# heyblackC/DFMIR

Hardware: AMD Instinct MI355X
Metric: train-step image-pairs/sec (fwd+bwd): 2D 256x256 bs=16 and 3D 160^3 bs=1 (higher is better)
Workload: dtype f32 (fp16x2-split MFMA, fp32 accumulate)

## Files before the change

dfmir_amd/_lib.py:

```python
import ctypes
import os
from ctypes import c_double, c_float, c_int, c_longlong, c_void_p, POINTER, Structure

_HERE = os.path.dirname(os.path.abspath(__file__))
LIB_PATH = os.environ.get("DFMIR_HIP_LIB") or os.path.join(_HERE, "libdfmir_hip.so")


class DfConvGeom(Structure):
    _fields_ = [(n, c_int) for n in (
        "N", "Cin", "Cout", "Di", "Hi", "Wi", "Do", "Ho", "Wo", "KD", "KH", "KW",
        "stride", "dil", "pd", "ph", "pw", "pad_mode", "act")] + [("slope", c_float)]


P = c_void_p
_GP = POINTER(DfConvGeom)
_SIGS = {
    "dfmir_abi_version": [],
    "dfmir_set_option": [ctypes.c_char_p, ctypes.c_char_p],
    "dfmir_get_option": [ctypes.c_char_p, ctypes.c_char_p, c_int],
    "dfmir_conv_fwd": [_GP, P, P, P, P, P],
    "dfmir_conv_wgrad": [_GP, P, P, P, P],
    "dfmir_bias_grad": [P, P, c_int, c_int, c_longlong, P],
    "dfmir_weight_pack": [P, P, c_int, c_int, c_int, c_int, P],
    "dfmir_weight_pack_floats": [c_int, c_int, c_int],
    "dfmir_weight_pack_batch": [P, c_int, P, c_int, P],
    "dfmir_conv3x3_res_ok": [_GP],
    "dfmir_conv3x3_fwd_scaled_res": [_GP, P, P, c_int, P, P, P, P, c_int, P, P],
    "dfmir_conv3x3_reflect_ring_ok": [_GP],
    "dfmir_conv3x3_reflect_ring_len": [_GP],
    "dfmir_conv3x3_reflect_ring": [_GP, P, P, P, c_int, P, P, P],
    "dfmir_conv3x3_bwd_pair_ok": [_GP, _GP],
    "dfmir_conv3x3_bwd_pair": [_GP, _GP, P, P, c_int, P, P, P, P, c_int, P, P, P, c_int, P, P, POINTER(c_int), P],
    "dfmir_conv_fwd_scaled": [_GP, P, P, c_int, P, P, P, P],
    "dfmir_conv_wgrad_scaled": [_GP, P, P, c_int, P, P, c_int, P, P, P],
    "dfmir_conv_wgrad_scaled_ch": [_GP, P, P, c_int, P, P, c_int, P, P, P, P],
    "dfmir_instnorm_bwd_pmax_ok": [c_longlong],
    "dfmir_instnorm_bwd_pmax": [P, P, P, P, P, c_int, c_longlong, c_int, P, P, c_int, P, P],
    "dfmir_patch_gather_bwd_gp": [P, P, P, c_int, c_int, c_longlong, c_int, c_int, P, P, P],
    "dfmir_patch_gather_bwd_any": [P, P, P, c_int, c_int, c_longlong, c_int, c_int, P, P, P],
    "dfmir_absmax": [P, c_longlong, P, P],
    "dfmir_conv3d_split_ok": [_GP],
    "dfmir_conv3d_split_ws_floats": [c_int, c_int],
    "dfmir_conv3d_split_fwd": [_GP, P, P, c_int, P, P, P, P, P, P],
    "dfmir_conv3d_split_fwd_sub": [_GP, P, P, c_int, P, P, P, P, P, c_int, P],
    "dfmir_conv3d_split_fwd_actgrad": [_GP, P, P, c_int, P, P, P, P, P, c_int, P, c_float, P],
    "dfmir_conv3d_up_ok": [c_int] * 6,
    "dfmir_conv3d_wsplit_batch": [P, c_int, P],
    "dfmir_conv3d_split_is_pair": [c_int],
    "dfmir_conv3d_march_ok": [_GP],
    "dfmir_conv3d_march_fwd": [_GP, P, P, c_int, P, P, P, P, P, c_float, P],
    "dfmir_conv3d_tiny_ok": [_GP],
    "dfmir_conv3d_tiny_fwd": [_GP, P, P, P, P, P, P, c_float, P],
    "dfmir_conv3d_s2c2_ok": [_GP],
    "dfmir_conv3d_s2c2_fwd": [_GP, P, P, P, P, P, P],
    "dfmir_conv3d_s2c2_wgrad": [_GP, P, P, P, P],
    "dfmir_conv3d_s2_ok": [_GP],
    "dfmir_conv3d_s2_fwd": [_GP, P, P, P, P, P, P],
    "dfmir_conv3d_s2_wgrad": [_GP, P, P, P, P, P],
    "dfmir_conv3d_s2_dgrad_ok": [_GP],
    "dfmir_conv3d_s2_dgrad": [_GP, P, P, P, P],
    "dfmir_conv3d_up_ws_floats": [c_int, c_int],
    "dfmir_conv3d_up_fwd": [P, P, c_int, P, c_int, P, P] + [c_int] * 6 + [P],
    "dfmir_conv3d_up_skip2_fwd": [P, P, c_int, P, P, c_int, c_int, P, P, P, P, P] + [c_int] * 7 + [c_float, P],
    "dfmir_conv3d_up_dgrad_ws_floats": [c_int, c_int],
    "dfmir_conv3d_up_dgrad": [P, P, c_int, P, c_int, P, P, P, P, c_float] + [c_int] * 6 + [P],
    "dfmir_conv3d_split_fwd_add": [_GP, P, P, c_int, P, c_int, c_int, P, P, P, P, P],
    "dfmir_conv3d_split_wgrad_ok": [_GP],
    "dfmir_conv3d_split_wgrad": [_GP, P, P, c_int, P, P, c_int, P, P],
    "dfmir_conv3d_split_wgrad_upcat": [_GP, P, P, c_int, P, c_int, P, P, c_int, P, P, P],
    "dfmir_conv3d_upwgrad_ok": [_GP, c_int],
    "dfmir_conv3d_wgrad_is_march": [_GP],
    "dfmir_conv3d_wgrad_is_march_at": [_GP, P, P],
    "dfmir_conv3d_upwgrad_ws_floats": [],
    "dfmir_conv3d_upwgrad": [_GP, P, P, c_int, P, c_int, P, P, c_int, P, P, P, P],
    "dfmir_conv3d_split_wgrad_db": [_GP, P, P, c_int, P, P, c_int, P, P, P],
    "dfmir_probe_merge": [P, P, P, P],
    "dfmir_act_bwd_amax": [P, P, P, c_longlong, c_int, c_float, P, P],
    "dfmir_weight_unpack": [P, P, c_int, c_int, c_int, P],
    "dfmir_weight_unpack_add_batch": [P, c_int, c_longlong, P],
    "dfmir_conv7x7_c1_fwd": [P, P, P, P, c_int, c_int, c_int, c_int, c_int, P],
    "dfmir_conv7x7_c1_wgrad": [P, P, P, P, c_int, c_int, c_int, c_int, c_int, P],
    "dfmir_tapstack_fwd": [P, P] + [c_int] * 7 + [P],
    "dfmir_tapstack_bwd": [P, P] + [c_int] * 7 + [P],
    "dfmir_tapsum_fwd": [P, P, P] + [c_int] * 10 + [c_float, P],
    "dfmir_tapsum_bwd": [P, P] + [c_int] * 9 + [P],
    "dfmir_instnorm_fwd": [P, P, P, P, P, c_int, c_longlong, c_float, c_int, P, P],
    "dfmir_instnorm_stats_ok": [c_longlong],
    "dfmir_instnorm_stats": [P, P, P, c_int, c_longlong, c_float, c_int, P, P],
    "dfmir_instnorm_bwd": [P, P, P, P, P, c_int, c_longlong, c_int, P, P],
    "dfmir_instnorm_bwd_cols_ok": [c_longlong, c_int],
    "dfmir_instnorm_bwd_cols": [P, P, P, P, P, c_int, c_longlong, c_int, P, P, c_int, P],
    "dfmir_in_relu_blurdown_ok": [c_int, c_int],
    "dfmir_in_relu_blurdown_fwd": [P, P, P, P, c_int, c_int, c_int, c_float, P, P],
    "dfmir_in_relu_blurdown_bwd": [P, P, P, P, P, c_int, c_int, c_int, P, P, P],
    "dfmir_act_bwd": [P, P, P, c_longlong, c_int, c_float, P],
    "dfmir_blur_down_fwd": [P, P, c_int, c_int, c_int, P],
    "dfmir_blur_down_bwd": [P, P, c_int, c_int, c_int, P],
    "dfmir_blur_up_fwd": [P, P, c_int, c_int, c_int, P],
    "dfmir_blur_up_bwd": [P, P, c_int, c_int, c_int, P],
    "dfmir_reflect_pad2d_fwd": [P, P, c_int, c_int, c_int, c_int, P],
    "dfmir_reflect_pad2d_bwd": [P, P, c_int, c_int, c_int, c_int, P],
    "dfmir_reflect_pad2d_bwd_add": [P, P, P, c_int, c_int, c_int, c_int, P],
    "dfmir_upcat_fwd": [P, P, P] + [c_int] * 7 + [P],
    "dfmir_upcat_bwd": [P, P, P] + [c_int] * 7 + [P],
    "dfmir_cat_channels_fwd": [P, P, P, c_longlong, c_longlong, c_longlong, P],
    "dfmir_cat_channels_bwd": [P, P, P, c_longlong, c_longlong, c_longlong, P],
    "dfmir_scale": [P, P, c_longlong, c_float, P],
    "dfmir_warp2d_fwd": [P, P, P] + [c_int] * 6 + [P],
    "dfmir_warp2d_bwd": [P, P, P, P, P] + [c_int] * 6 + [P],
    "dfmir_warp3d_fwd": [P, P, P] + [c_int] * 7 + [P],
    "dfmir_warp3d_bwd": [P, P, P, P, P] + [c_int] * 7 + [P],
    "dfmir_warp_bwd_own_ws_floats": [c_int] * 6,
    "dfmir_warp_bwd_own": [c_int, P, P, P, P, P] + [c_int] * 7 + [P, P],
    "dfmir_resize_fwd": [P, P] + [c_int] * 7 + [c_float, P],
    "dfmir_resize_bwd": [P, P] + [c_int] * 7 + [c_float, P],
    "dfmir_resize_bwd_ws_floats": [c_int] * 7,
    "dfmir_resize_bwd_sep": [P, P] + [c_int] * 7 + [c_float, P, P],
    "dfmir_bspline_fwd": [c_int, P, P] + [c_int] * 7 + [P],
    "dfmir_bspline_bwd_ws_floats": [c_int] * 8,
    "dfmir_bspline_bwd": [c_int, P, P] + [c_int] * 7 + [P, P],
    "dfmir_patch_gather_fwd": [P, P, P, c_int, c_int, c_longlong, c_int, P],
    "dfmir_patch_gather_bwd": [P, P, P, c_int, c_int, c_longlong, c_int, P],
    "dfmir_patch_gather_bwd_amax": [P, P, P, c_int, c_int, c_longlong, c_int, P, P],
    "dfmir_patch_gather_fwd_g": [P, P, P, c_int, c_int, c_longlong, c_int, c_int, P],
    "dfmir_patch_gather_bwd_g": [P, P, P, c_int, c_int, c_longlong, c_int, c_int, P, P],
    "dfmir_l2norm_fwd": [P, P, P, c_int, c_longlong, c_float, P],
    "dfmir_l2norm_bwd": [P, P, P, P, c_int, c_longlong, c_float, P],
    "dfmir_patchnce_fwd": [P, P, P, P, c_longlong, c_int, c_int, c_float, P],
    "dfmir_patchnce_bwd": [P, P, P, P, c_longlong, c_int, c_int, c_float, P],
    "dfmir_masked_l1_fwd": [P, P, P, c_float, P, P, c_longlong, P],
    "dfmir_masked_l1_bwd": [P, P, P, c_float, P, P, P, P, c_longlong, P],
    "dfmir_flow_smooth_ws_floats": [],
    "dfmir_flow_smooth_fwd": [P, P, P] + [c_int] * 5 + [P],
    "dfmir_flow_smooth_bwd": [P, P, P] + [c_int] * 5 + [P],
    "dfmir_flow_smooth_fwd_p": [P, P, P] + [c_int] * 6 + [P],
    "dfmir_flow_smooth_bwd_p": [P, P, P] + [c_int] * 6 + [P],
    "dfmir_mul": [P, P, P, c_longlong, P],
    "dfmir_bend_ws_floats": [c_int] * 5,
    "dfmir_bend_fwd": [P, P, P] + [c_int] * 5 + [c_float] * 3 + [P],
    "dfmir_bend_bwd": [P, P, P] + [c_int] * 5 + [c_float] * 3 + [P],
    "dfmir_jacdet_ws_floats": [c_int] * 5,
    "dfmir_jacdet_fwd": [c_int, P, P, P] + [c_int] * 5 + [c_float, c_int, P],
    "dfmir_jacdet_bwd": [c_int, P, P, P] + [c_int] * 5 + [c_float, c_int, P],
    "dfmir_jacdet_map": [c_int, P, P] + [c_int] * 5 + [P],
    "dfmir_jacdet_stats": [c_int, P, P, P] + [c_int] * 5 + [c_double, c_double, P],
    "dfmir_invcons_ws_floats": [c_int] * 5,
    "dfmir_invcons_fwd": [c_int, P, P, P, P, P, P] + [c_int] * 4 + [P],
    "dfmir_invcons_bwd_ws_floats": [c_int] * 5,
    "dfmir_invcons_bwd": [c_int, P, P, P, P, P, P, P] + [c_int] * 4 + [P],
    "dfmir_compose_fwd": [c_int, P, P, P] + [c_int] * 4 + [P],
    "dfmir_compose_bwd_ws_floats": [c_int] * 5,
    "dfmir_compose_bwd": [c_int, P, P, P, P, P, P] + [c_int] * 4 + [P],
    "dfmir_flow_invert_ws_floats": [c_int] * 7,
    "dfmir_flow_invert": [c_int, P, P, P, P, P] + [c_int] * 5 + [c_float, c_int, P],
    "dfmir_dsearch_pool": [c_int, P, P, P] + [c_int] * 6 + [P],
    "dfmir_dsearch_cost": [c_int, P, P, P] + [c_int] * 6 + [P],
    "dfmir_dsearch_argmin": [c_int, P, P, c_float, P, P] + [c_int] * 5 + [P],
    "dfmir_dsearch_smooth": [c_int, P, P] + [c_int] * 4 + [P],
    "dfmir_warp_ssd_ws_floats": [c_int] * 6,
    "dfmir_warp_ssd_pack": [c_int, P, P] + [c_int] * 5 + [P],
    "dfmir_warp_ssd_fwd": [c_int] + [P] * 9 + [c_int] * 5 + [P],
    "dfmir_warp_ssd_fwd_grad": [c_int] + [P] * 10 + [c_int] * 5 + [P],
    "dfmir_warp_ssd_bwd": [P, P, P, P, c_longlong, P],
    "dfmir_affine_ws_floats": [c_int] * 5,
    "dfmir_affine_flow": [c_int, P, P] + [c_int] * 4 + [P],
    "dfmir_affine_flow_bwd": [c_int, P, P, P] + [c_int] * 4 + [P],
    "dfmir_affine_system": [c_int] + [P] * 6 + [c_int] * 6 + [P],
    "dfmir_affine_lm_step": [c_int] + [P] * 7 + [c_int] * 3 + [c_double] * 2 + [P],
    "dfmir_landmark_ws_floats": [c_int] * 6,
    "dfmir_landmark_fwd": [c_int] + [P] * 10 + [c_int] * 5 + [c_float] * 3 + [c_int, P],
    "dfmir_landmark_bwd": [c_int] + [P] * 8 + [c_int] * 5 + [c_float] * 3 + [c_int, P],
    "dfmir_nmi_ws_floats": [c_longlong, c_int],
    "dfmir_nmi_fwd": [P, P, P, P, c_int, c_float, c_float, c_longlong, P, P, P],
    "dfmir_nmi_bwd": [P, P, P, P, c_int, c_float, c_float, c_longlong, P, P, P, P, P],
    "dfmir_mind_ws_floats": [c_int] * 8,
    "dfmir_mind_desc": [P] + [c_int] * 7 + [P, P, P],
    "dfmir_mind_fwd": [P, P, P] + [c_int] * 7 + [P, P, P],
    "dfmir_mind_bwd": [P, P, P] + [c_int] * 7 + [P, P, P, P, P, P],
    "dfmir_gradfield_ws_floats": [c_int] * 5,
    "dfmir_gradfield_fwd": [P, P, P] + [c_int] * 5 + [c_float] * 3 + [c_int] + [c_double] * 3 + [P, P, P],
    "dfmir_gradfield_bwd": [P] * 7 + [c_int] * 5 + [c_float] * 3 + [P],
    "dfmir_gradfield_field": [P] + [c_int] * 5 + [c_float] * 3 + [c_int] + [c_double] * 2 + [P, P, P],
    "dfmir_warp_dice_ws_floats": [c_int] * 6,
    "dfmir_warp_dice_fwd": [c_int, P, P, P, P] + [c_int] * 6 + [P, P, P, P, P],
    "dfmir_warp_dice_bwd": [c_int, P, P, P, P] + [c_int] * 5 + [P, P, P, P],
    "dfmir_label_hausdorff_ws_bytes": [c_int] * 6,
    "dfmir_label_edt_sq": [c_int, P, c_int, c_int] + [c_int] * 4 + [P, P],
    "dfmir_label_hausdorff": [c_int, P, P, P] + [c_int] * 7 + [P, P, P, P, P, P],
    "dfmir_dice_ws_floats": [c_longlong, c_longlong],
    "dfmir_dice_fwd": [P, P, c_longlong, c_longlong, P, P, P],
    "dfmir_dice_bwd": [P, P, c_longlong, c_longlong, P, P, P, P, P],
    "dfmir_mse_ws_floats": [c_longlong],
    "dfmir_mse_fwd": [P, P, c_longlong, P, P, P],
    "dfmir_mse_bwd": [P, P, c_longlong, P, P, P, P],
    "dfmir_ncc_fwd_m": [P, P, P, c_int, P, P, P, P] + [c_int] * 5 + [c_float, P],
    "dfmir_ncc_bwd_m": [P, P, P, c_int, P, P, P, P, P, P] + [c_int] * 5 + [c_float, P],
    "dfmir_ncc_gauss_fwd": [P, P, P, c_int, P, P, P, P] + [c_int] * 4 + [P, c_int, c_float, c_float, P],
    "dfmir_ncc_gauss_bwd": [P, P, P, c_int, P, P, P, P, P, P] + [c_int] * 4 + [P, c_int, c_float, c_float, P],
    "dfmir_ncc_fwd": [P, P, P, P, P, P] + [c_int] * 5 + [c_float, P],
    "dfmir_ncc_bwd": [P, P, P, P, P, P, P, P] + [c_int] * 5 + [c_float, P],
    "dfmir_patch_gather_fwd_multi": [P, c_int, P, P, c_int, c_int, c_longlong, c_int, P],
    "dfmir_nce_head_fwd": [P, c_int, P, P, P, P, P, P, P, P, P, P, c_int, c_int, c_longlong, c_int, c_float, P],
    "dfmir_patch_ids_draw": [P, P, c_int, c_int, c_int, P, P],
    "dfmir_segment_means_fwd": [P, P, c_int, c_int, c_longlong, c_float, P],
    "dfmir_segment_means_bwd": [P, P, c_int, c_int, c_longlong, c_float, P],
    "dfmir_scalar_combine_fwd": [P, c_int, P, c_int, P, P],
    "dfmir_scalar_combine_bwd": [P, c_int, P, c_int, P, P],
    "dfmir_det_head_floats": [],
    "dfmir_det_begin": [P, c_longlong, P, c_longlong, P, c_int, P, c_longlong, P, c_int, ctypes.c_double, P],
    "dfmir_det_end": [P, P, c_longlong, P, c_longlong, P],
    "dfmir_fill_zero": [P, c_longlong, P],
    "dfmir_sum_scaled": [P, P, c_longlong, c_float, P],
    "dfmir_fill_from_scalar": [P, P, c_longlong, c_float, P],
    "dfmir_adam_step": [P, P, P, P, c_longlong] + [c_float] * 7 + [P],
}

_lib = None


class DfmirHipError(RuntimeError):
    pass


def lib():
    global _lib
    if _lib is None:
        import torch
        if not os.path.exists(LIB_PATH):
            raise DfmirHipError(
                "libdfmir_hip.so not found at %s -- build it with `python -c 'import __graft_entry__ as g; "
                "g.build()'` or `make -C dfmir_amd/csrc` (there is no CPU fallback)" % LIB_PATH)
        h = ctypes.CDLL(LIB_PATH)
        for name, args in _SIGS.items():
            fn = getattr(h, name)
            fn.argtypes = args
            fn.restype = c_int
        h.dfmir_weight_pack_floats.restype = c_longlong
        h.dfmir_conv3d_split_ws_floats.restype = c_longlong
        h.dfmir_conv3d_up_ws_floats.restype = c_longlong
        h.dfmir_conv3d_up_dgrad_ws_floats.restype = c_longlong
        h.dfmir_conv3d_upwgrad_ws_floats.restype = c_longlong
        h.dfmir_flow_smooth_ws_floats.restype = c_longlong
        h.dfmir_bend_ws_floats.restype = c_longlong
        h.dfmir_jacdet_ws_floats.restype = c_longlong
        h.dfmir_invcons_ws_floats.restype = c_longlong
        h.dfmir_invcons_bwd_ws_floats.restype = c_longlong
        h.dfmir_compose_bwd_ws_floats.restype = c_longlong
        h.dfmir_flow_invert_ws_floats.restype = c_longlong
        h.dfmir_warp_ssd_ws_floats.restype = c_longlong
        h.dfmir_affine_ws_floats.restype = c_longlong
        h.dfmir_landmark_ws_floats.restype = c_longlong
        h.dfmir_nmi_ws_floats.restype = c_longlong
        h.dfmir_mind_ws_floats.restype = c_longlong
        h.dfmir_gradfield_ws_floats.restype = c_longlong
        h.dfmir_warp_dice_ws_floats.restype = c_longlong
        h.dfmir_label_hausdorff_ws_bytes.restype = c_longlong
        h.dfmir_dice_ws_floats.restype = c_longlong
        h.dfmir_mse_ws_floats.restype = c_longlong
        h.dfmir_warp_bwd_own_ws_floats.restype = c_longlong
        h.dfmir_resize_bwd_ws_floats.restype = c_longlong
        h.dfmir_bspline_bwd_ws_floats.restype = c_longlong
        h.dfmir_last_error.argtypes = []
        h.dfmir_last_error.restype = ctypes.c_char_p
        _lib = h
    return _lib


def check(rc):
    if rc != 0:
        msg = lib().dfmir_last_error()
        raise DfmirHipError(msg.decode() if msg else "dfmir_hip error %d" % rc)


def set_option(name, value=None):
    check(lib().dfmir_set_option(name.encode(), None if value is None else str(value).encode()))


def get_option(name):
    buf = ctypes.create_string_buffer(256)
    n = lib().dfmir_get_option(name.encode(), buf, 256)
    return None if n < 0 else buf.value.decode()


def exported_symbols():
    return sorted(list(_SIGS.keys()) + ["dfmir_last_error"])
```

dfmir_amd/csrc/conv.hip:

```cpp
#include "conv3x3_common.h"
#include <stdlib.h>
#include <vector>

typedef float f32x16 __attribute__((ext_vector_type(16)));

struct ConvK {
  DfConvGeom g;
  int kc, nchunks;
  int Dm, Hm, Wm, ncx, ncy, ncz;
};

static inline void df_chunking(int Cin, int& kc, int& nchunks) {
  nchunks = (Cin + 15) / 16;
  int per = (Cin + nchunks - 1) / nchunks;
  kc = (per + 1) & ~1;
  if (kc < 2) kc = 2;
}

template <bool DIL2>
__device__ __forceinline__ bool conv_pixel(const ConvK& k, long long pp, long long P, int& n, int& oz, int& oy, int& ox,
                                           int& cls) {
  const DfConvGeom& g = k.g;
  cls = 0;
  if (pp >= P) { n = oz = oy = ox = 0; return false; }
// ... 282 lines not shown
    v += bias ? bias[co] : 0.f;
    if (g.act == 1) v = v > 0.f ? v : v * g.slope;
    else if (g.act == 2) v = tanhf(v);
    y[((long long)n * g.Cout + co) * DHWo + (pp - (long long)n * DHWo)] = v;
  }
}

template <int WJ, int WC, int TJ, int TC, int BP>
__global__ __launch_bounds__(256) void conv_wgrad_mfma_k(const float* __restrict__ x,
                                                         const float* __restrict__ dy,
                                                         float* __restrict__ dwt, DfConvGeom g,
                                                         long long pchunk, const float* __restrict__ fx) {
  constexpr int BJ = WJ * TJ * 32, BC = WC * TC * 32;
  constexpr int RS = 256 / BP;
  constexpr int NA = BJ / RS, NB = (BC + RS - 1) / RS;
  static_assert(WJ * WC == 4, "4 waves");
  __shared__ float As[2][BP][BJ + 1];
  __shared__ float Bs[2][BP][BC + 1];
  __shared__ int jinfo[BJ];

  const int tid = threadIdx.x, lane = tid & 63, wid = tid >> 6;
  const int wj = wid / WC, wc = wid % WC;
  const long long DHWi = (long long)g.Di * g.Hi * g.Wi;
  const long long DHWo = (long long)g.Do * g.Ho * g.Wo;
  const long long P = (long long)g.N * DHWo;
  const int J = g.KD * g.KH * g.KW * g.Cin;
  const int j0 = blockIdx.y * BJ, c0 = blockIdx.z * BC;
  const long long pbeg = (long long)blockIdx.x * pchunk;
  long long pend = pbeg + pchunk;
  if (pend > P) pend = P;

  for (int i = tid; i < BJ; i += 256) {
    const int j = j0 + i;
    int info = -1;
    if (j < J) {
      const int tap = j / g.Cin, ci = j - tap * g.Cin;
      const int kw = tap % g.KW, t2 = tap / g.KW, kh = t2 % g.KH, kd = t2 / g.KH;
      info = (ci << 12) | (kd << 8) | (kh << 4) | kw;
    }
    jinfo[i] = info;
  }
  __syncthreads();

  constexpr unsigned OOB = 0x80000000u;
  const unsigned dhwi4 = (unsigned)DHWi * 4u;
  const __amdgpu_buffer_rsrc_t x_src = __builtin_amdgcn_make_buffer_rsrc(
      const_cast<float*>(x), 0, (unsigned)((long long)g.N * g.Cin * DHWi * 4), 0x00020000);
  const __amdgpu_buffer_rsrc_t d_src = __builtin_amdgcn_make_buffer_rsrc(
      const_cast<float*>(dy), 0, (unsigned)((long long)g.N * g.Cout * DHWo * 4), 0x00020000);
  const int pl = tid % BP, r0 = tid / BP;
  float ra[NA], rb[NB];
  f32x16 acc[TJ][TC];
#pragma unroll
  for (int i = 0; i < TJ; ++i)
#pragma unroll
    for (int j = 0; j < TC; ++j)
#pragma unroll
      for (int r = 0; r < 16; ++r) acc[i][j][r] = 0.f;

#define WG_GLOAD(pb_)                                                                            \
  {                                                                                              \
    const long long pq = (pb_) + pl;                                                             \
    const bool pv = pq < pend;                                                                   \
    int ox = 0, oy = 0, oz = 0, n = 0;                                                           \
    if (pv) {                                                                                    \
      long long t = pq;                                                                          \
      ox = (int)(t % g.Wo); t /= g.Wo;                                                           \
      oy = (int)(t % g.Ho); t /= g.Ho;                                                           \
      oz = (int)(t % g.Do); n = (int)(t / g.Do);                                                 \
    }                                                                                            \
    const unsigned xb = (unsigned)n * (unsigned)g.Cin * dhwi4;                                   \
    _Pragma("unroll") for (int jj = 0; jj < NA; ++jj) {                                          \
      const int info = jinfo[r0 + RS * jj];                                                      \
      const int ci = info >> 12, kd = (info >> 8) & 15, kh = (info >> 4) & 15, kw = info & 15;   \
      int iz, iy, ix;                                                                            \
      bool v = pv && info >= 0;                                                                  \
      v &= df_in_coord(oz, kd, g.stride, g.pd, 1, g.Di, g.pad_mode, iz);                         \
      v &= df_in_coord(oy, kh, g.stride, g.ph, 1, g.Hi, g.pad_mode, iy);                         \
      v &= df_in_coord(ox, kw, g.stride, g.pw, 1, g.Wi, g.pad_mode, ix);                         \
      const unsigned o = v ? xb + (unsigned)ci * dhwi4 +                                         \
                                 (unsigned)(((long long)iz * g.Hi + iy) * g.Wi + ix) * 4u : OOB; \
      ra[jj] = __uint_as_float(__builtin_amdgcn_raw_buffer_load_b32(x_src, o, 0, 0));            \
    }                                                                                            \
    const long long so = pq - (long long)n * DHWo;                                               \
    _Pragma("unroll") for (int jj = 0; jj < NB; ++jj) {                                          \
      const int cr = r0 + RS * jj;                                                               \
      const int co = c0 + cr;                                                                    \
      const unsigned o = (pv && cr < BC && co < g.Cout)                                          \
                             ? (unsigned)(((long long)n * g.Cout + co) * DHWo + so) * 4u : OOB;  \
      rb[jj] = __uint_as_float(__builtin_amdgcn_raw_buffer_load_b32(d_src, o, 0, 0));            \
    }                                                                                            \
  }
#define WG_LSTORE(buf_)                                                                          \
  {                                                                                              \
    _Pragma("unroll") for (int jj = 0; jj < NA; ++jj) As[buf_][pl][r0 + RS * jj] = ra[jj];       \
    _Pragma("unroll") for (int jj = 0; jj < NB; ++jj) {                                          \
      const int cr = r0 + RS * jj;                                                               \
      if (cr < BC) Bs[buf_][pl][cr] = rb[jj];                                                    \
    }                                                                                            \
  }

  if (pbeg < pend) {
    WG_GLOAD(pbeg);
    WG_LSTORE(0);
  }
  __syncthreads();
  const int l31 = lane & 31, lhi = lane >> 5;
  int it = 0;
  for (long long pb = pbeg; pb < pend; pb += BP, ++it) {
    const int buf = it & 1;
    const bool more = (pb + BP) < pend;
    if (more) WG_GLOAD(pb + BP);
#pragma unroll 2
    for (int kk = 0; kk < BP / 2; ++kk) {
      const int kr = 2 * kk + lhi;
      float a[TJ], b[TC];
#pragma unroll
      for (int i = 0; i < TJ; ++i) a[i] = As[buf][kr][(wj * TJ + i) * 32 + l31];
#pragma unroll
      for (int j = 0; j < TC; ++j) b[j] = Bs[buf][kr][(wc * TC + j) * 32 + l31];
#pragma unroll
      for (int i = 0; i < TJ; ++i)
#pragma unroll
        for (int j = 0; j < TC; ++j)
          acc[i][j] = __builtin_amdgcn_mfma_f32_32x32x2f32(a[i], b[j], acc[i][j], 0, 0, 0);
    }
    if (more) WG_LSTORE(buf ^ 1);
    __syncthreads();
  }
#undef WG_GLOAD
#undef WG_LSTORE

#pragma unroll
  for (int j = 0; j < TC; ++j) {
    const int co = c0 + (wc * TC + j) * 32 + l31;
    if (co >= g.Cout) continue;
#pragma unroll
    for (int i = 0; i < TJ; ++i) {
      const int jb = j0 + (wj * TJ + i) * 32 + 4 * lhi;
#pragma unroll
      for (int r = 0; r < 16; ++r) {
        const int jr = jb + (r & 3) + 8 * (r >> 2);
        if (jr < J) df_acc(dwt, (long long)jr * g.Cout + co, acc[i][j][r], fx);
      }
    }
  }
}


__global__ __launch_bounds__(256) void conv1x1_wgrad_k(const float* __restrict__ x, const float* __restrict__ dy,
                                                       float* __restrict__ dwt, int N, int Cin, int Cout, long long S,
                                                       long long chunks_per_img, long long chunks_per_block,
                                                       const float* __restrict__ fx) {
  constexpr int BK = 64, LD = BK + 1;
  __shared__ float Xs[64 * LD];
  __shared__ float Ds[64 * LD];
  const int tid = threadIdx.x, lane = tid & 63, wid = tid >> 6;
  const int l31 = lane & 31, lhi = lane >> 5, wm = wid >> 1, wn = wid & 1;
  const int ci0 = blockIdx.y * 64, co0 = blockIdx.z * 64;
  const long long total = (long long)N * chunks_per_img;
  const long long cbeg = (long long)blockIdx.x * chunks_per_block;
  long long cend = cbeg + chunks_per_block;
  if (cend > total) cend = total;
  const int r = tid >> 2, q16 = (tid & 3) * 16;
  const bool xrow = ci0 + r < Cin, drow = co0 + r < Cout;
  float4 rx[4], rd[4];
  const float4 z4 = make_float4(0.f, 0.f, 0.f, 0.f);
#define G1_GLOAD(c_)                                                                                         \
  {                                                                                                          \
    const long long n_ = (c_) / chunks_per_img, q0_ = ((c_) - n_ * chunks_per_img) * BK + q16;               \
    const float* xp_ = x + ((long long)n_ * Cin + ci0 + r) * S + q0_;                                        \
    const float* dp_ = dy + ((long long)n_ * Cout + co0 + r) * S + q0_;                                      \
    _Pragma("unroll") for (int j = 0; j < 4; ++j) {                                                          \
      const bool in_ = q0_ + 4 * j < S;                                                                      \
      rx[j] = (xrow && in_) ? *reinterpret_cast<const float4*>(xp_ + 4 * j) : z4;                            \
      rd[j] = (drow && in_) ? *reinterpret_cast<const float4*>(dp_ + 4 * j) : z4;                            \
    }                                                                                                        \
  }
#define G1_LSTORE()                                                                                          \
  {                                                                                                          \
    float* xs_ = &Xs[r * LD + q16];                                                                          \
    float* ds_ = &Ds[r * LD + q16];                                                                          \
    _Pragma("unroll") for (int j = 0; j < 4; ++j) {                                                          \
      xs_[4 * j] = rx[j].x; xs_[4 * j + 1] = rx[j].y; xs_[4 * j + 2] = rx[j].z; xs_[4 * j + 3] = rx[j].w;    \
      ds_[4 * j] = rd[j].x; ds_[4 * j + 1] = rd[j].y; ds_[4 * j + 2] = rd[j].z; ds_[4 * j + 3] = rd[j].w;    \
    }                                                                                                        \
  }
  f32x16 acc;
#pragma unroll
  for (int i = 0; i < 16; ++i) acc[i] = 0.f;
  if (cbeg < cend) G1_GLOAD(cbeg)
  for (long long c = cbeg; c < cend; ++c) {
    __syncthreads();
    G1_LSTORE()
    __syncthreads();
    if (c + 1 < cend) G1_GLOAD(c + 1)
    const float* ap = &Xs[(wm * 32 + l31) * LD + lhi];
    const float* bp = &Ds[(wn * 32 + l31) * LD + lhi];
#pragma unroll 8
    for (int ks = 0; ks < BK / 2; ++ks)
      acc = __builtin_amdgcn_mfma_f32_32x32x2f32(ap[2 * ks], bp[2 * ks], acc, 0, 0, 0);
  }
#undef G1_GLOAD
#undef G1_LSTORE
  const int co = co0 + wn * 32 + l31;
  if (co < Cout && cbeg < cend) {
#pragma unroll
    for (int i = 0; i < 16; ++i) {
      const int ci = ci0 + wm * 32 + 4 * lhi + (i & 3) + 8 * (i >> 2);
      if (ci < Cin) df_acc(dwt, (long long)ci * Cout + co, acc[i], fx);
    }
  }
}

__global__ void bias_grad_k(const float* __restrict__ dy, float* __restrict__ db, int N, int C,
                            long long S, int nsplit, const float* __restrict__ fx) {
  __shared__ float sm[17];
  const int c = blockIdx.x, n = blockIdx.y, part = blockIdx.z;
  const long long per = (((S + nsplit - 1) / nsplit) + 3) & ~3LL;
  const long long beg = part * per;
  long long end = beg + per;
  if (end > S) end = S;
  const float* p = dy + ((long long)n * C + c) * S;
  float s = 0.f;
  if ((S & 3) == 0) {
    const float4* p4 = reinterpret_cast<const float4*>(p);
    for (long long i = (beg >> 2) + threadIdx.x; i < (end >> 2); i += blockDim.x) {
      const float4 v = p4[i];
      s += (v.x + v.y) + (v.z + v.w);
    }
  } else {
    for (long long i = beg + threadIdx.x; i < end; i += blockDim.x) s += p[i];
  }
  s = block_sum(s, sm);
  if (threadIdx.x == 0 && beg < S) df_acc(db, c, s, fx);
}

__global__ __launch_bounds__(256) void weight_pack_k(const float* __restrict__ w, float* __restrict__ o, int Cout,
                                                     int Cin, int T, int mode, float* __restrict__ part) {
  __shared__ unsigned smax;
  if (threadIdx.x == 0) smax = 0u;
  __syncthreads();
  float am = 0.f;
  const long long total = (long long)Cout * Cin * T;
  for (long long i = (long long)blockIdx.x * blockDim.x + threadIdx.x; i < total;
       i += (long long)gridDim.x * blockDim.x) {
    if (mode == 0) {
      const int co = (int)(i % Cout);
      long long r = i / Cout;
      const int ci = (int)(r % Cin);
      const int t = (int)(r / Cin);
      o[i] = w[((long long)co * Cin + ci) * T + t];
      am = fmaxf(am, fabsf(o[i]));
    } else {
      const int ci = (int)(i % Cin);
      long long r = i / Cin;
      const int co = (int)(r % Cout);
      const int t = (int)(r / Cout);
      o[i] = w[((long long)co * Cin + ci) * T + (T - 1 - t)];
      am = fmaxf(am, fabsf(o[i]));
    }
  }
  if (part) publish_block_absmax(am, &smax, part + blockIdx.x);
}
__global__ void weight_unpack_k(const float* __restrict__ gt, float* __restrict__ g, int Cout, int Cin,
                                int T) {
  const long long total = (long long)Cout * Cin * T;
  for (long long i = (long long)blockIdx.x * blockDim.x + threadIdx.x; i < total;
       i += (long long)gridDim.x * blockDim.x) {
    const int t = (int)(i % T);
    long long r = i / T;
    const int ci = (int)(r % Cin);
    const int co = (int)(r / Cin);
    g[i] = gt[((long long)t * Cin + ci) * Cout + co];
  }
}

__global__ __launch_bounds__(256) void weight_pack_batch_k(const DfPackJobDev* __restrict__ jobs) {
  const DfPackJobDev jb = jobs[blockIdx.y];
  if ((int)blockIdx.x >= jb.nblk) return;
  __shared__ unsigned smax;
  if (threadIdx.x == 0) smax = 0u;
  __syncthreads();
  float am = 0.f;
  const int Cout = jb.Cout, Cin = jb.Cin, T = jb.T;
  const long long total = (long long)Cout * Cin * T;
  for (long long i = (long long)blockIdx.x * 256 + threadIdx.x; i < total; i += (long long)jb.nblk * 256) {
    float v;
    if (jb.mode == 0) {
      const int co = (int)(i % Cout);
      long long r = i / Cout;
      const int ci = (int)(r % Cin);
      const int t = (int)(r / Cin);
      v = jb.w[((long long)co * Cin + ci) * T + t];
    } else {
      const int ci = (int)(i % Cin);
      long long r = i / Cin;
      const int co = (int)(r % Cout);
      const int t = (int)(r / Cout);
      v = jb.w[((long long)co * Cin + ci) * T + (T - 1 - t)];
    }
    jb.o[i] = v;
    am = fmaxf(am, fabsf(v));
  }
  if (jb.part) publish_block_absmax(am, &smax, jb.part + blockIdx.x);
}

__global__ __launch_bounds__(256) void weight_unpack_add_batch_k(const DfUnpackJob* __restrict__ jobs) {
  const DfUnpackJob jb = jobs[blockIdx.y];
  const int Cout = jb.Cout, Cin = jb.Cin, T = jb.T;
  if (T > 9) {
    const long long total = (long long)Cout * Cin * T;
    for (long long i = (long long)blockIdx.x * blockDim.x + threadIdx.x; i < total;
         i += (long long)gridDim.x * blockDim.x) {
      const int t = (int)(i % T);
      long long r = i / T;
      const int ci = (int)(r % Cin);
      const int co = (int)(r / Cin);
      const long long j = ((long long)t * Cin + ci) * Cout + co;
      jb.dst[i] += jb.src[j];
      jb.src[j] = 0.f;
    }
    return;
  }
  __shared__ float tile[32][32 * 9 + 1];
  const int tco = (Cout + 31) >> 5, tci = (Cin + 31) >> 5;
  const int lx = threadIdx.x & 31, ly = threadIdx.x >> 5;
  for (int tl = blockIdx.x; tl < tco * tci; tl += gridDim.x) {
    const int co0 = (tl % tco) << 5, ci0 = (tl / tco) << 5;
    for (int r = ly; r < T * 32; r += 8) {
      const int t = r >> 5, ci = ci0 + (r & 31), co = co0 + lx;
      float v = 0.f;
      if (ci < Cin && co < Cout) {
        const long long j = ((long long)t * Cin + ci) * Cout + co;
        v = jb.src[j];
        jb.src[j] = 0.f;
      }
      tile[lx][(r & 31) * T + t] = v;
    }
    __syncthreads();
    const int ncol = 32 * T;
    for (int e = threadIdx.x; e < 32 * ncol; e += 256) {
      const int c = e / ncol, q = e - c * ncol;
      const int co = co0 + c, ci = ci0 + q / T;
      if (co < Cout && ci < Cin) jb.dst[((long long)co * Cin + ci0) * T + q] += tile[c][q];
    }
    __syncthreads();
  }
}

bool df_conv3x3_fwd_try(const DfConvGeom* g, const float* x, const float* w_tcc, const float* bias,
                        float* y, hipStream_t st, int* rc);
bool df_conv3x3_wgrad_try(const DfConvGeom* g, const float* x, const float* dy, float* dw_tcc,
                          hipStream_t st, int* rc);
bool df_conv3x3_small_wgrad_try(const DfConvGeom* g, const float* x, const float* dy, float* dw_tcc, hipStream_t st,
                                int* rc);
bool df_conv3x3_split_fwd_try(const DfConvGeom* g, const float* x, const float* x_amax, int x_n, const float* w_packed,
                              const float* bias, const float* res, const float* ring, int ring_rl, float* y,
                              hipStream_t st, int* rc);
int df_conv3x3_split_res_ok(const DfConvGeom* g);
bool df_conv3x3_split_wgrad_try(const DfConvGeom* g, const float* x, const float* x_amax, int x_n, const float* dy,
                                const float* dy_amax, int dy_n, float* dw_tcc, float* db, hipStream_t st, int* rc,
                                const float* dy_pmax);
int df_weight_split_launch(const float* w_tcc, float* packed, int K, int M, int npart, hipStream_t st);
float* df_weight_probe_slots(float* packed, int K, int M);
int df_absmax_launch(const float* x, long long n, float* out, hipStream_t st, bool zero_first);
bool df_conv3d_fwd_try(const DfConvGeom* g, const float* x, const float* w_tcc, const float* bias, float* y,
                       hipStream_t st, int* rc);
bool df_conv3d_wgrad_try(const DfConvGeom* g, const float* x, const float* dy, float* dw_tcc, hipStream_t st,
                         int* rc);
static bool use_generic_only() {
  static DfOptInt o{"DFMIR_CONV_GENERIC", 0};
  return o.get() == 1;
}

static int check_geom(const DfConvGeom* g) {
  if (!g) return -1;
  if (g->N <= 0 || g->Cin <= 0 || g->Cout <= 0) return -1;
  if (g->Di <= 0 || g->Hi <= 0 || g->Wi <= 0 || g->Do <= 0 || g->Ho <= 0 || g->Wo <= 0) return -1;
  if (g->KD <= 0 || g->KH <= 0 || g->KW <= 0 || g->KD > 15 || g->KH > 15 || g->KW > 15) return -1;
  if (g->stride < 1 || g->dil < 1) return -1;
  if (g->pad_mode != 0 && g->pad_mode != 1) return -1;
  if (g->pad_mode == 1 && g->dil != 1) return -1;
  return 0;
}

static int conv_fwd_impl(const DfConvGeom* g, const float* x, const float* x_amax, int x_n, const float* w_tcc,
                         const float* bias, float* y, void* stream);
extern "C" int dfmir_conv_fwd(const DfConvGeom* g, const float* x, const float* w_tcc,
                              const float* bias, float* y, void* stream) {
  return conv_fwd_impl(g, x, nullptr, 0, w_tcc, bias, y, stream);
}
extern "C" int dfmir_conv_fwd_scaled(const DfConvGeom* g, const float* x, const float* x_amax, int x_amax_n,
                                     const float* w_tcc, const float* bias, float* y, void* stream) {
  return conv_fwd_impl(g, x, x_amax, x_amax_n, w_tcc, bias, y, stream);
}
extern "C" int dfmir_conv3x3_res_ok(const DfConvGeom* g) {
  return (g && check_geom(g) == 0 && !use_generic_only()) ? df_conv3x3_split_res_ok(g) : 0;
}
extern "C" int dfmir_conv3x3_fwd_scaled_res(const DfConvGeom* g, const float* x, const float* x_amax, int x_amax_n,
                                            const float* w_tcc, const float* bias, const float* res,
                                            const float* ring, int ring_len, float* y, void* stream) {
  DF_ARG_CHECK(g && check_geom(g) == 0 && x && x_amax && x_amax_n > 0 && w_tcc && (res || ring) && y);
  DF_ARG_CHECK(!use_generic_only() && df_conv3x3_split_res_ok(g));
  DF_ARG_CHECK(!ring || (ring_len >= (g->Ho > g->Wo ? g->Ho : g->Wo) + 2 && g->Ho >= 4 && g->Wo >= 4));
  int rc = 0;
  if (!df_conv3x3_split_fwd_try(g, x, x_amax, x_amax_n, w_tcc, bias, res, ring, ring_len, y, (hipStream_t)stream, &rc))
    return df_set_error((int)hipErrorInvalidValue, __FILE__, __LINE__);
  return rc;
}
extern "C" int dfmir_absmax(const float* x, long long n, float* out, void* stream) {
  DF_ARG_CHECK(x && out && n > 0);
  const int rc = df_absmax_launch(x, n, out, (hipStream_t)stream, false);
  if (rc) return df_set_error(rc, __FILE__, __LINE__);
  return 0;
}
static int conv_fwd_impl(const DfConvGeom* g, const float* x, const float* x_amax, int x_n, const float* w_tcc,
                         const float* bias, float* y, void* stream) {
  DF_ARG_CHECK(check_geom(g) == 0 && x && w_tcc && y);
  hipStream_t st = (hipStream_t)stream;
  const long long P = (long long)g->N * g->Do * g->Ho * g->Wo;
  static DfOptFlag tinyvol_o{"DFMIR_NO_TINYVOL"};
  const bool tinyvol = !use_generic_only() && g->Do > 1 && (long long)g->Do * g->Ho * g->Wo <= 512 && P <= 8192 && g->Cout <= 64 &&
                       g->Cout > 4 && !tinyvol_o.get();
  if (!use_generic_only()) {
    int rc = 0;
    if (df_conv3x3_split_fwd_try(g, x, x_amax, x_n, w_tcc, bias, nullptr, nullptr, 0, y, st, &rc)) return rc;
    if (df_conv3x3_fwd_try(g, x, w_tcc, bias, y, st, &rc)) return rc;
    if (!tinyvol && df_conv3d_fwd_try(g, x, w_tcc, bias, y, st, &rc)) return rc;
  }
  if (g->Cout <= 4) {
    const unsigned grid = (unsigned)((P + 255) / 256);
    if (g->Cout == 1) conv_small_k<1><<<grid, 256, 0, st>>>(x, w_tcc, bias, y, *g);
    else if (g->Cout == 2) conv_small_k<2><<<grid, 256, 0, st>>>(x, w_tcc, bias, y, *g);
    else conv_small_k<4><<<grid, 256, 0, st>>>(x, w_tcc, bias, y, *g);
    DF_LAUNCH_CHECK();
    return 0;
  }
  if (tinyvol) {
    if (g->Cout <= 8) conv_tinyvol_k<8><<<(unsigned)P, 256, 0, st>>>(x, w_tcc, bias, y, *g);
    else if (g->Cout <= 16) conv_tinyvol_k<16><<<(unsigned)P, 256, 0, st>>>(x, w_tcc, bias, y, *g);
    else if (g->Cout <= 32) conv_tinyvol_k<32><<<(unsigned)P, 256, 0, st>>>(x, w_tcc, bias, y, *g);
    else conv_tinyvol_k<64><<<(unsigned)P, 256, 0, st>>>(x, w_tcc, bias, y, *g);
    DF_LAUNCH_CHECK();
    return 0;
  }
  const long long in_img = (long long)g->Cin * g->Di * g->Hi * g->Wi * 4;
  const long long out_img = (long long)g->Cout * g->Do * g->Ho * g->Wo * 4;
  DF_ARG_CHECK(in_img < 0x7FFFFFFFLL && out_img < 0x7FFFFFFFLL);
  DF_ARG_CHECK((long long)g->KD * g->KH * g->KW * g->Cin * g->Cout * 4 < 0x7FFFFFFFLL);
  long long nb = 0x7FFFFFFFLL / (in_img > out_img ? in_img : out_img);
  if (nb > g->N) nb = g->N;
  for (int n0 = 0; n0 < g->N; n0 += (int)nb) {
    ConvK k;
    k.g = *g;
    k.g.N = (g->N - n0 < nb) ? g->N - n0 : (int)nb;
    df_chunking(g->Cin, k.kc, k.nchunks);
    const float* xs = x + (long long)n0 * (in_img / 4);
    float* ys = y + (long long)n0 * (out_img / 4);
    long long Ps = (long long)k.g.N * g->Do * g->Ho * g->Wo;
    const bool dil2 = g->dil == 2 && g->stride == 1 && g->pad_mode == 0 && g->KD * g->KH * g->KW <= 128 && g->Cout <= 64;
    k.ncx = k.ncy = k.ncz = 1;
    k.Dm = g->Do; k.Hm = g->Ho; k.Wm = g->Wo;
    if (dil2) {
      if (g->Wi > 1 || g->KW > 1) { k.ncx = 2; k.Wm = (g->Wo + 1) / 2; }
      if (g->Hi > 1 || g->KH > 1) { k.ncy = 2; k.Hm = (g->Ho + 1) / 2; }
      if (g->Di > 1 || g->KD > 1) { k.ncz = 2; k.Dm = (g->Do + 1) / 2; }
      Ps = (long long)k.ncx * k.ncy * k.ncz * k.g.N * k.Dm * k.Hm * k.Wm;
    }
    const bool small_p = (Ps + 255) / 256 < 192 && g->Cout > 8;
    if (dil2) {
      if (small_p) {
        dim3 grid((unsigned)((Ps + 63) / 64), (unsigned)((g->Cout + 63) / 64));
        conv_mfma_k<2, 2, 1, 1, true><<<grid, 256, 0, st>>>(xs, w_tcc, bias, ys, k);
      } else {
        dim3 grid((unsigned)((Ps + 255) / 256), 1);
        if (g->Cout > 32) conv_mfma_k<1, 4, 2, 2, true><<<grid, 256, 0, st>>>(xs, w_tcc, bias, ys, k);
        else conv_mfma_k<1, 4, 1, 2, true><<<grid, 256, 0, st>>>(xs, w_tcc, bias, ys, k);
      }
    } else if (small_p && g->Cout <= 64) {
      dim3 grid((unsigned)((Ps + 63) / 64), (unsigned)((g->Cout + 63) / 64));
      conv_mfma_k<2, 2, 1, 1><<<grid, 256, 0, st>>>(xs, w_tcc, bias, ys, k);
    } else if (g->Cout > 64) {
      const long long big = ((Ps + 127) / 128) * ((g->Cout + 127) / 128);
      constexpr int big_min = 256;
      if (big < big_min) {
        dim3 grid((unsigned)((Ps + 63) / 64), (unsigned)((g->Cout + 63) / 64));
        conv_mfma_k<2, 2, 1, 1><<<grid, 256, 0, st>>>(xs, w_tcc, bias, ys, k);
      } else {
        dim3 grid((unsigned)((Ps + 127) / 128), (unsigned)((g->Cout + 127) / 128));
        conv_mfma_k<2, 2, 2, 2><<<grid, 256, 0, st>>>(xs, w_tcc, bias, ys, k);
      }
    } else if (g->Cout > 32) {
      dim3 grid((unsigned)((Ps + 255) / 256), 1);
      conv_mfma_k<1, 4, 2, 2><<<grid, 256, 0, st>>>(xs, w_tcc, bias, ys, k);
    } else {
      dim3 grid((unsigned)((Ps + 255) / 256), 1);
      conv_mfma_k<1, 4, 1, 2><<<grid, 256, 0, st>>>(xs, w_tcc, bias, ys, k);
    }
    DF_LAUNCH_CHECK();
  }
  return 0;
}

static int conv_wgrad_impl(const DfConvGeom* g, const float* x, const float* x_amax, int x_n, const float* dy,
                           const float* dy_amax, int dy_n, float* dw_tcc, float* db, void* stream,
                           const float* dy_pmax = nullptr);
extern "C" int dfmir_conv_wgrad_scaled_ch(const DfConvGeom* g, const float* x, const float* x_amax, int x_amax_n,
                                          const float* dy, const float* dy_amax, int dy_amax_n, const float* dy_pmax,
                                          float* dw_tcc, float* db, void* stream) {
  return conv_wgrad_impl(g, x, x_amax, x_amax_n, dy, dy_amax, dy_amax_n, dw_tcc, db, stream, dy_pmax);
}
extern "C" int dfmir_conv_wgrad(const DfConvGeom* g, const float* x, const float* dy, float* dw_tcc,
                                void* stream) {
  return conv_wgrad_impl(g, x, nullptr, 0, dy, nullptr, 0, dw_tcc, nullptr, stream);
}
extern "C" int dfmir_conv_wgrad_scaled(const DfConvGeom* g, const float* x, const float* x_amax, int x_amax_n,
                                       const float* dy, const float* dy_amax, int dy_amax_n, float* dw_tcc,
                                       float* db, void* stream) {
  return conv_wgrad_impl(g, x, x_amax, x_amax_n, dy, dy_amax, dy_amax_n, dw_tcc, db, stream);
}
static int bias_grad_launch(const float* dy, float* db, int N, int C, long long S, hipStream_t st);
static int conv_wgrad_impl(const DfConvGeom* g, const float* x, const float* x_amax, int x_n, const float* dy,
                           const float* dy_amax, int dy_n, float* dw_tcc, float* db, void* stream, const float* dy_pmax) {
  DF_ARG_CHECK(check_geom(g) == 0 && x && dy && dw_tcc);
  DF_ARG_CHECK(g->dil == 1 && g->Cin < (1 << 19));
  hipStream_t st = (hipStream_t)stream;
  if (!use_generic_only()) {
    int rc = 0;
    if (df_conv3x3_split_wgrad_try(g, x, x_amax, x_n, dy, dy_amax, dy_n, dw_tcc, db, st, &rc, dy_pmax)) return rc;
  }
  if (db) {
    const int rcb = bias_grad_launch(dy, db, g->N, g->Cout, (long long)g->Do * g->Ho * g->Wo, st);
    if (rcb) return rcb;
  }
  if (!use_generic_only()) {
    int rc = 0;
    if (df_conv3x3_wgrad_try(g, x, dy, dw_tcc, st, &rc)) return rc;
    if (df_conv3x3_small_wgrad_try(g, x, dy, dw_tcc, st, &rc)) return rc;
    if (df_conv3d_wgrad_try(g, x, dy, dw_tcc, st, &rc)) return rc;
  }
  {
    static DfOptFlag no1x1_o{"DFMIR_NO_1X1_WGRAD"};
    const long long S1 = (long long)g->Di * g->Hi * g->Wi;
    if (!use_generic_only() && !no1x1_o.get() && g->KD == 1 && g->KH == 1 && g->KW == 1 && g->stride == 1 && g->pd == 0 &&
        g->ph == 0 && g->pw == 0 && g->Do == g->Di && g->Ho == g->Hi && g->Wo == g->Wi && (S1 & 3) == 0 && S1 >= 64 &&
        ((reinterpret_cast<uintptr_t>(x) | reinterpret_cast<uintptr_t>(dy)) & 15) == 0 && g->Cin >= 8 && g->Cout >= 8) {
      const long long cpi = (S1 + 63) / 64, total = (long long)g->N * cpi;
      const unsigned ny = (unsigned)((g->Cin + 63) / 64), nz = (unsigned)((g->Cout + 63) / 64);
      long long want = 1024 / ((long long)ny * nz);
      if (want < 1) want = 1;
      long long maxs = (total + 7) / 8;
      if (maxs < 1) maxs = 1;
      if (want > maxs) want = maxs;
      const long long cpb = (total + want - 1) / want;
      const unsigned nx = (unsigned)((total + cpb - 1) / cpb);
      conv1x1_wgrad_k<<<dim3(nx, ny, nz), 256, 0, st>>>(x, dy, dw_tcc, g->N, g->Cin, g->Cout, S1, cpi, cpb, df_det_fx());
      DF_LAUNCH_CHECK();
      return 0;
    }
  }
  long long P = (long long)g->N * g->Do * g->Ho * g->Wo;
  const int J = g->KD * g->KH * g->KW * g->Cin;
  auto plan = [&](int BJ, int BC, int BP, unsigned& nP, long long& pchunk, dim3& grid) {
    const unsigned nJ = (J + BJ - 1) / BJ, nC = (g->Cout + BC - 1) / BC;
    long long want = 2048 / ((long long)nJ * nC);
    if (want < 1) want = 1;
    long long maxp = (P + (long long)BP * 8 - 1) / ((long long)BP * 8);
    if (maxp < 1) maxp = 1;
    if (want > maxp) want = maxp;
    pchunk = (P + want - 1) / want;
    pchunk = ((pchunk + BP - 1) / BP) * BP;
    nP = (unsigned)((P + pchunk - 1) / pchunk);
    grid = dim3(nP, nJ, nC);
  };
  const long long in_img = (long long)g->Cin * g->Di * g->Hi * g->Wi * 4;
  const long long out_img = (long long)g->Cout * g->Do * g->Ho * g->Wo * 4;
  DF_ARG_CHECK(in_img < 0x7FFFFFFFLL && out_img < 0x7FFFFFFFLL);
  long long nb = 0x7FFFFFFFLL / (in_img > out_img ? in_img : out_img);
  if (nb > g->N) nb = g->N;
  const int Nfull = g->N;
  for (int n0 = 0; n0 < Nfull; n0 += (int)nb) {
    DfConvGeom gs = *g;
    gs.N = (Nfull - n0 < nb) ? Nfull - n0 : (int)nb;
    const float* xs = x + (long long)n0 * (in_img / 4);
    const float* ds = dy + (long long)n0 * (out_img / 4);
    P = (long long)gs.N * g->Do * g->Ho * g->Wo;
    unsigned nP;
    long long pchunk;
    dim3 grid;
    if (g->Cout > 64) {
      plan(128, 128, 16, nP, pchunk, grid);
      conv_wgrad_mfma_k<2, 2, 2, 2, 16><<<grid, 256, 0, st>>>(xs, ds, dw_tcc, gs, pchunk, df_det_fx());
    } else if (g->Cout > 32) {
      plan(128, 64, 16, nP, pchunk, grid);
      conv_wgrad_mfma_k<4, 1, 1, 2, 16><<<grid, 256, 0, st>>>(xs, ds, dw_tcc, gs, pchunk, df_det_fx());
    } else {
      plan(128, 32, 32, nP, pchunk, grid);
      conv_wgrad_mfma_k<4, 1, 1, 1, 32><<<grid, 256, 0, st>>>(xs, ds, dw_tcc, gs, pchunk, df_det_fx());
    }
    DF_LAUNCH_CHECK();
  }
  return 0;
}

static int bias_grad_launch(const float* dy, float* db, int N, int C, long long S, hipStream_t st) {
  int nsplit = (int)((S + 65535) / 65536);
  if (nsplit > 64) nsplit = 64;
  if (nsplit < 1) nsplit = 1;
  DF_ARG_CHECK(N <= 65535);
  bias_grad_k<<<dim3(C, N, nsplit), S >= 4096 ? 256 : 64, 0, st>>>(dy, db, N, C, S, nsplit, df_det_fx());
  DF_LAUNCH_CHECK();
  return 0;
}
extern "C" int dfmir_bias_grad(const float* dy, float* db, int N, int C, long long S, void* stream) {
  DF_ARG_CHECK(dy && db && N > 0 && C > 0 && S > 0);
  return bias_grad_launch(dy, db, N, C, S, (hipStream_t)stream);
}

extern "C" int dfmir_weight_pack(const float* w, float* w_tcc, int Cout, int Cin, int T, int mode,
                                 void* stream) {
  DF_ARG_CHECK(w && w_tcc && Cout > 0 && Cin > 0 && T > 0 && (mode == 0 || mode == 1));
  const long long total = (long long)Cout * Cin * T;
  const unsigned nblk = df_grid(total, 256, 2048);
  const int K = mode ? Cout : Cin, M = mode ? Cin : Cout;
  float* part = (T == 9) ? df_weight_probe_slots(w_tcc, K, M) : nullptr;
  weight_pack_k<<<nblk, 256, 0, (hipStream_t)stream>>>(w, w_tcc, Cout, Cin, T, mode, part);
  DF_LAUNCH_CHECK();
  if (T == 9) {
    const int rc = df_weight_split_launch(w_tcc, w_tcc, K, M, (int)nblk, (hipStream_t)stream);
    if (rc) return df_set_error(rc, __FILE__, __LINE__);
  }
  return 0;
}
int df_conv3x3_reflect_ring_ok(const DfConvGeom* g);
int df_conv3x3_reflect_ring_launch(const DfConvGeom* g, const float* dy, const float* dy_cols, const float* dy_amax,
                                   int dy_n, const float* wd_packed, float* ring, hipStream_t st);
int df_conv3x3_reflect_ring_len(const DfConvGeom* g);
extern "C" int dfmir_conv3x3_reflect_ring_ok(const DfConvGeom* g) {
  return (g && check_geom(g) == 0) ? df_conv3x3_reflect_ring_ok(g) : 0;
}
extern "C" int dfmir_conv3x3_reflect_ring_len(const DfConvGeom* g) {
  return (g && check_geom(g) == 0 && df_conv3x3_reflect_ring_ok(g)) ? df_conv3x3_reflect_ring_len(g) : 0;
}
extern "C" int dfmir_conv3x3_reflect_ring(const DfConvGeom* g, const float* dy, const float* dy_cols,
                                          const float* dy_amax, int dy_amax_n, const float* wd_packed, float* ring,
                                          void* stream) {
  DF_ARG_CHECK(g && check_geom(g) == 0 && dy && dy_amax && dy_amax_n > 0 && wd_packed && ring);
  DF_ARG_CHECK(df_conv3x3_reflect_ring_ok(g));
  const int rc = df_conv3x3_reflect_ring_launch(g, dy, dy_cols, dy_amax, dy_amax_n, wd_packed, ring, (hipStream_t)stream);
  if (rc) return df_set_error(rc, __FILE__, __LINE__);
  return 0;
}
int df_conv3x3_bwd_pair_ok(const DfConvGeom* gd, const DfConvGeom* gw);
bool df_conv3x3_bwd_pair_try(const DfConvGeom* gd, const DfConvGeom* gw, const float* dy, const float* dy_amax, int dy_n,
                             const float* dy_pmax, const float* wd_packed, const float* res, const float* ring, int ring_rl,
                             float* dx, const float* x, const float* x_amax, int x_n, float* dw_tcc, float* db,
                             hipStream_t st, int* rc);
extern "C" int dfmir_conv3x3_bwd_pair_ok(const DfConvGeom* gd, const DfConvGeom* gw) {
  return (gd && gw && check_geom(gd) == 0 && check_geom(gw) == 0 && !use_generic_only()) ? df_conv3x3_bwd_pair_ok(gd, gw) : 0;
}
extern "C" int dfmir_conv3x3_bwd_pair(const DfConvGeom* gd, const DfConvGeom* gw, const float* dy, const float* dy_amax,
                                      int dy_amax_n, const float* dy_pmax, const float* wd_packed, const float* res,
                                      const float* ring, int ring_len, float* dx, const float* x, const float* x_amax,
                                      int x_amax_n, float* dw_tcc, float* db, int* paired, void* stream) {
  DF_ARG_CHECK(gd && gw && check_geom(gd) == 0 && check_geom(gw) == 0 && dy && wd_packed && dx && x && dw_tcc && paired);
  DF_ARG_CHECK(gd->N == gw->N && gd->Cin == gw->Cout && gd->Cout == gw->Cin && gw->dil == 1 && gw->Cin < (1 << 19));
  DF_ARG_CHECK(!ring || (ring_len >= (gd->Ho > gd->Wo ? gd->Ho : gd->Wo) + 2 && gd->Ho >= 4 && gd->Wo >= 4));
  *paired = 0;
  int rc = 0;
  if (!use_generic_only() && df_conv3x3_bwd_pair_try(gd, gw, dy, dy_amax, dy_amax_n, dy_pmax, wd_packed, res, ring, ring_len,
                                                     dx, x, x_amax, x_amax_n, dw_tcc, db, (hipStream_t)stream, &rc)) {
    *paired = rc == 0 ? 1 : 0;
    return rc;
  }
  rc = (res || ring) ? dfmir_conv3x3_fwd_scaled_res(gd, dy, dy_amax, dy_amax_n, wd_packed, nullptr, res, ring, ring_len, dx, stream)
                     : conv_fwd_impl(gd, dy, dy_amax, dy_amax_n, wd_packed, nullptr, dx, stream);
  if (rc) return rc;
  return conv_wgrad_impl(gw, x, x_amax, x_amax_n, dy, dy_amax, dy_amax_n, dw_tcc, db, stream, dy_pmax);
}
extern "C" int dfmir_weight_pack_batch(const DfPackJob* jobs_host, int njobs, void* table_dev, int upload,
                                       void* stream) {
  DF_ARG_CHECK(jobs_host && table_dev && njobs > 0 && njobs <= 65535);
  static_assert(sizeof(DfPackJobDev) == 64, "job table stride");
  hipStream_t st = (hipStream_t)stream;
  int max_nblk = 0, max_nsplit = 0;
  std::vector<DfPackJobDev> tab((size_t)njobs);
  for (int i = 0; i < njobs; ++i) {
    const DfPackJob& h = jobs_host[i];
    DF_ARG_CHECK(h.w && h.packed && h.Cout > 0 && h.Cin > 0 && h.T > 0 && (h.mode == 0 || h.mode == 1));
    DfPackJobDev& d = tab[(size_t)i];
    d.w = h.w; d.o = h.packed; d.Cout = h.Cout; d.Cin = h.Cin; d.T = h.T; d.mode = h.mode;
    d.nblk = (int)df_grid((long long)h.Cout * h.Cin * h.T, 256, 2048);
    df_weight_split_fill(&d);
    max_nblk = d.nblk > max_nblk ? d.nblk : max_nblk;
    max_nsplit = d.nsplit > max_nsplit ? d.nsplit : max_nsplit;
  }
  if (upload) {
    hipError_t e = hipMemcpyAsync(table_dev, tab.data(), sizeof(DfPackJobDev) * (size_t)njobs, hipMemcpyHostToDevice, st);
    if (e != hipSuccess) return df_set_error((int)e, __FILE__, __LINE__);
  }
  weight_pack_batch_k<<<dim3((unsigned)max_nblk, (unsigned)njobs), 256, 0, st>>>(
      reinterpret_cast<const DfPackJobDev*>(table_dev));
  DF_LAUNCH_CHECK();
  const int rc = df_weight_split_batch_launch(reinterpret_cast<const DfPackJobDev*>(table_dev), njobs, max_nsplit, st);
  if (rc) return df_set_error(rc, __FILE__, __LINE__);
  return 0;
}
extern "C" long long dfmir_weight_pack_floats(int Cout, int Cin, int T) {
  if (Cout <= 0 || Cin <= 0 || T <= 0) return -1;
  const long long s0 = df_pack_split_floats(Cin, Cout, T), s1 = df_pack_split_floats(Cout, Cin, T);
  return df_pack_tcc_floats(Cin, Cout, T) + (s0 > s1 ? s0 : s1) + (T == 9 ? 4 + 2048 : 0);
}
extern "C" int dfmir_weight_unpack_add_batch(const DfUnpackJob* jobs_dev, int njobs, long long max_total,
                                             void* stream) {
  DF_ARG_CHECK(jobs_dev && njobs > 0 && njobs <= 65535 && max_total > 0);
  long long bx = (max_total + 255) / 256;
  if (bx > 64) bx = 64;
  weight_unpack_add_batch_k<<<dim3((unsigned)bx, (unsigned)njobs), 256, 0, (hipStream_t)stream>>>(jobs_dev);
  DF_LAUNCH_CHECK();
  return 0;
}
extern "C" int dfmir_weight_unpack(const float* g_tcc, float* g, int Cout, int Cin, int T,
                                   void* stream) {
  DF_ARG_CHECK(g_tcc && g && Cout > 0 && Cin > 0 && T > 0);
  const long long total = (long long)Cout * Cin * T;
  weight_unpack_k<<<df_grid(total, 256, 2048), 256, 0, (hipStream_t)stream>>>(g_tcc, g, Cout, Cin, T);
  DF_LAUNCH_CHECK();
  return 0;
}
```

dfmir_amd/csrc/nce_head.hip:

```cpp
#include "common.h"

#define DF_IDS_MAXP 1024
#define DF_IDS_MAXPERM 4096
struct DfIdSizes {
  long long S[8];
};

__device__ __forceinline__ unsigned long long df_mix64(unsigned long long z) {
  z += 0x9E3779B97F4A7C15ull;
  z = (z ^ (z >> 30)) * 0xBF58476D1CE4E5B9ull;
  z = (z ^ (z >> 27)) * 0x94D049BB133111EBull;
  return z ^ (z >> 31);
}

__global__ __launch_bounds__(256) void patch_ids_draw_k(unsigned long long* __restrict__ state, DfIdSizes sizes,
                                                        int n_layers, int n_sets, int P, int Ppad,
                                                        long long* __restrict__ out) {
  __shared__ unsigned long long el[DF_IDS_MAXPERM];
  __shared__ unsigned char lost[DF_IDS_MAXP];
  __shared__ int pending;
  const int layer = blockIdx.x / n_sets, set = blockIdx.x - layer * n_sets;
  const unsigned long long S = (unsigned long long)sizes.S[layer];
  const unsigned long long seed = state[0], counter = state[1];
  const unsigned long long stream = df_mix64(seed ^ df_mix64(counter * 0x100000001B3ull + (unsigned long long)blockIdx.x));
// ... 5 lines not shown
      el[i] = i < (int)S ? ((df_mix64(stream ^ ((unsigned long long)i * 0xD6E8FEB86659FD93ull)) >> 12) << 12) | (unsigned long long)i
                         : ~0ull;
    __syncthreads();
    for (int k = 2; k <= Spad; k <<= 1)
      for (int j = k >> 1; j > 0; j >>= 1) {
        for (int i = threadIdx.x; i < Spad; i += 256) {
          const int ixj = i ^ j;
          if (ixj > i) {
            const unsigned long long a = el[i], b = el[ixj];
            const bool up = (i & k) == 0;
            if ((a > b) == up) { el[i] = b; el[ixj] = a; }
          }
        }
        __syncthreads();
      }
    for (int i = threadIdx.x; i < P; i += 256) o[i] = (long long)(el[i] & 0xFFFull);
  } else {
  long long mine[DF_IDS_MAXP / 256];
  bool fresh[DF_IDS_MAXP / 256];
#pragma unroll
  for (int j = 0; j < DF_IDS_MAXP / 256; ++j) { mine[j] = -1; fresh[j] = true; }
  for (int round = 0; round < 64; ++round) {
#pragma unroll
    for (int j = 0; j < DF_IDS_MAXP / 256; ++j) {
      const int slot = threadIdx.x + j * 256;
      if (slot < Ppad) {
        unsigned long long e = ~0ull;
        if (slot < P) {
          if (fresh[j]) {
            const unsigned long long r = df_mix64(stream ^ ((unsigned long long)slot * 0xD6E8FEB86659FD93ull +
                                                            (unsigned long long)round * 0xA0761D6478BD642Full));
            mine[j] = (long long)(((r >> 32) * S) >> 32);
          }
          e = ((unsigned long long)mine[j] << 12) | ((unsigned long long)(fresh[j] ? 1 : 0) << 11) | (unsigned long long)slot;
        }
        el[slot] = e;
      }
    }
    if (threadIdx.x == 0) pending = 0;
    __syncthreads();
    for (int k = 2; k <= Ppad; k <<= 1)
      for (int j = k >> 1; j > 0; j >>= 1) {
        for (int i = threadIdx.x; i < Ppad; i += 256) {
          const int ixj = i ^ j;
          if (ixj > i) {
            const unsigned long long a = el[i], b = el[ixj];
            const bool up = (i & k) == 0;
            if ((a > b) == up) { el[i] = b; el[ixj] = a; }
          }
        }
        __syncthreads();
      }
    for (int i = threadIdx.x; i < Ppad; i += 256) lost[i] = 0;
    __syncthreads();
    for (int i = threadIdx.x + 1; i < Ppad; i += 256) {
      const unsigned long long e = el[i];
      if (e != ~0ull && (el[i - 1] >> 12) == (e >> 12)) lost[(int)(e & 0x7FFull)] = 1;
    }
    __syncthreads();
    bool any = false;
#pragma unroll
    for (int j = 0; j < DF_IDS_MAXP / 256; ++j) {
      const int slot = threadIdx.x + j * 256;
      if (slot < P) {
        fresh[j] = lost[slot] != 0;
        any = any || fresh[j];
      }
    }
    if (any) atomicOr(&pending, 1);
    __syncthreads();
    const int more = pending;
    __syncthreads();
    if (!more) break;
  }
#pragma unroll
  for (int j = 0; j < DF_IDS_MAXP / 256; ++j) {
    const int slot = threadIdx.x + j * 256;
    if (slot < P) o[slot] = mine[j];
  }
  }
  __syncthreads();
  if (threadIdx.x == 0) {
    __threadfence();
    const unsigned long long done = atomicAdd(&state[2], 1ull);
    if (done == (unsigned long long)gridDim.x - 1) {
      state[2] = 0ull;
      state[1] = counter + 1ull;
      __threadfence();
    }
  }
}

extern "C" int dfmir_patch_ids_draw(unsigned long long* state, const long long* sizes, int n_layers, int n_sets,
                                    int P, long long* out, void* stream) {
  DF_ARG_CHECK(state && sizes && out && n_layers > 0 && n_layers <= 8 && n_sets > 0 && P > 0 && P <= DF_IDS_MAXP);
  DfIdSizes sz{};
  for (int l = 0; l < n_layers; ++l) {
    DF_ARG_CHECK(sizes[l] >= P && sizes[l] < (1LL << 32));
    DF_ARG_CHECK(sizes[l] >= 2LL * P || sizes[l] <= DF_IDS_MAXPERM);
    sz.S[l] = sizes[l];
  }
  int Ppad = 1;
  while (Ppad < P) Ppad <<= 1;
  patch_ids_draw_k<<<(unsigned)(n_layers * n_sets), 256, 0, (hipStream_t)stream>>>(state, sz, n_layers, n_sets, P, Ppad,
                                                                               out);
  DF_LAUNCH_CHECK();
  return 0;
}

struct DfGatherSrcs {
  const float* p[8];
};
__global__ void patch_gather_multi_k(DfGatherSrcs srcs, const long long* __restrict__ ids, float* __restrict__ out,
                                     int G, int Bper, int C, long long S, int P) {
  const long long total = (long long)G * Bper * C * P;
  const long long rows = (long long)G * Bper * P;
  for (long long i = (long long)blockIdx.x * blockDim.x + threadIdx.x; i < total;
       i += (long long)gridDim.x * blockDim.x) {
    const int p = (int)(i % P);
    long long t = i / P;
    const int c = (int)(t % C);
    t /= C;
    const int b = (int)(t % Bper), g = (int)(t / Bper);
    out[(long long)c * rows + ((long long)g * Bper + b) * P + p] =
        srcs.p[g][((long long)b * C + c) * S + ids[(long long)g * P + p]];
  }
}
extern "C" int dfmir_patch_gather_fwd_multi(const float* const* srcs, int G, const long long* ids, float* out, int Bper,
                                            int C, long long S, int P, void* stream) {
  DF_ARG_CHECK(srcs && ids && out && G > 0 && G <= 8 && Bper > 0 && C > 0 && S > 0 && P > 0);
  DfGatherSrcs s{};
  for (int g = 0; g < G; ++g) {
    DF_ARG_CHECK(srcs[g] != nullptr);
    s.p[g] = srcs[g];
  }
  patch_gather_multi_k<<<df_grid((long long)G * Bper * C * P, 256, 4096), 256, 0, (hipStream_t)stream>>>(
      s, ids, out, G, Bper, C, S, P);
  DF_LAUNCH_CHECK();
  return 0;
}

typedef float nh_f32x16 __attribute__((ext_vector_type(16)));
struct NceHeadP {
  DfGatherSrcs srcs;
  const long long* ids;
  const float *w1, *b1, *w2, *b2;
  float *out, *nrm, *xs, *hs, *ypre;
  int G, Bper, C, P;
  long long S, rows;
  float eps;
};
constexpr int NH_R = 32, NH_M = 256, NH_CMAX = 256, NH_KB = 8;
__global__ __launch_bounds__(256, 2) void nce_head_fwd_k(NceHeadP k) {
  __shared__ float Xs[NH_CMAX * NH_R];
  __shared__ float Hs[NH_M * NH_R];
  __shared__ float red[4][NH_R];
  const int tid = threadIdx.x, lane = tid & 63, wid = tid >> 6;
  const int l31 = lane & 31, hi = lane >> 5;
  const long long r0 = (long long)blockIdx.x * NH_R;
  {
    const int r = tid & 31;
    const long long rr = r0 + r;
    const bool rok = rr < k.rows;
    const long long gb = rok ? rr / k.P : 0;
    const int pp = rok ? (int)(rr - gb * k.P) : 0;
    const int g = (int)(gb / k.Bper), b = (int)(gb - (long long)g * k.Bper);
    const long long id = rok ? k.ids[(long long)g * k.P + pp] : 0;
    const float* src = k.srcs.p[g] + (long long)b * k.C * k.S + id;
    const int Cp = (k.C + 2 * NH_KB - 1) / (2 * NH_KB) * (2 * NH_KB);
    for (int cb = tid >> 5; cb < Cp; cb += 64) {
      float v[8];
#pragma unroll
      for (int u = 0; u < 8; ++u) {
        const int c = cb + 8 * u;
        v[u] = (rok && c < k.C) ? src[(long long)c * k.S] : 0.f;
      }
#pragma unroll
      for (int u = 0; u < 8; ++u) {
        const int c = cb + 8 * u;
        if (c < Cp) {
          Xs[c * NH_R + r] = v[u];
          if (k.xs && rok && c < k.C) k.xs[(long long)c * k.rows + rr] = v[u];
        }
      }
    }
  }
  __syncthreads();
  const int m0 = 64 * wid;
  nh_f32x16 acc[2];
#pragma unroll
  for (int i = 0; i < 2; ++i)
#pragma unroll
    for (int e = 0; e < 16; ++e) acc[i][e] = 0.f;
#define NH_GEMM(W_, KTOT_, SRC_)                                                                  \
  {                                                                                               \
    const float* wp = (W_) + m0 + l31;                                                            \
    const int K2 = ((KTOT_) + 1) >> 1, nb = (K2 + NH_KB - 1) / NH_KB;                             \
    float ca0[NH_KB], ca1[NH_KB], na0[NH_KB], na1[NH_KB];                                         \
    _Pragma("unroll") for (int u = 0; u < NH_KB; ++u) {                                           \
      const int kr = 2 * u + hi;                                                                  \
      const bool ok = kr < (KTOT_);                                                               \
      ca0[u] = ok ? wp[(long long)kr * NH_M] : 0.f;                                               \
      ca1[u] = ok ? wp[(long long)kr * NH_M + 32] : 0.f;                                          \
    }                                                                                             \
    for (int j = 0; j < nb; ++j) {                                                                \
      if (j + 1 < nb) {                                                                           \
        _Pragma("unroll") for (int u = 0; u < NH_KB; ++u) {                                       \
          const int kr = 2 * ((j + 1) * NH_KB + u) + hi;                                          \
          const bool ok = kr < (KTOT_);                                                           \
          na0[u] = ok ? wp[(long long)kr * NH_M] : 0.f;                                           \
          na1[u] = ok ? wp[(long long)kr * NH_M + 32] : 0.f;                                      \
        }                                                                                         \
      }                                                                                           \
      _Pragma("unroll") for (int u = 0; u < NH_KB; ++u) {                                         \
        const int kr = 2 * (j * NH_KB + u) + hi;                                                  \
        const float bv = (SRC_)[kr * NH_R + l31];                                                 \
        acc[0] = __builtin_amdgcn_mfma_f32_32x32x2f32(ca0[u], bv, acc[0], 0, 0, 0);               \
        acc[1] = __builtin_amdgcn_mfma_f32_32x32x2f32(ca1[u], bv, acc[1], 0, 0, 0);               \
      }                                                                                           \
      _Pragma("unroll") for (int u = 0; u < NH_KB; ++u) { ca0[u] = na0[u]; ca1[u] = na1[u]; }     \
    }                                                                                             \
  }
  NH_GEMM(k.w1, k.C, Xs)
#pragma unroll
  for (int i = 0; i < 2; ++i)
#pragma unroll
    for (int e = 0; e < 16; ++e) {
      const int m = m0 + 32 * i + (e >> 2) * 8 + hi * 4 + (e & 3);
      float v = acc[i][e] + k.b1[m];
      v = v > 0.f ? v : 0.f;
      Hs[m * NH_R + l31] = v;
      if (k.hs && r0 + l31 < k.rows) k.hs[(long long)m * k.rows + r0 + l31] = v;
      acc[i][e] = 0.f;
    }
  __syncthreads();
  NH_GEMM(k.w2, NH_M, Hs)
#undef NH_GEMM
  float ss = 0.f;
#pragma unroll
  for (int i = 0; i < 2; ++i)
#pragma unroll
    for (int e = 0; e < 16; ++e) {
      const int m = m0 + 32 * i + (e >> 2) * 8 + hi * 4 + (e & 3);
      acc[i][e] += k.b2[m];
      ss += acc[i][e] * acc[i][e];
    }
  ss += __shfl_xor(ss, 32);
  if (hi == 0) red[wid][l31] = ss;
  __syncthreads();
  const float nr = sqrtf((red[0][l31] + red[1][l31]) + (red[2][l31] + red[3][l31]));
  const float inv = 1.f / (nr + k.eps);
  const long long rr = r0 + l31;
  if (rr < k.rows) {
    if (k.nrm && wid == 0 && hi == 0) k.nrm[rr] = nr;
#pragma unroll
    for (int i = 0; i < 2; ++i)
#pragma unroll
      for (int e = 0; e < 16; ++e) {
        const int m = m0 + 32 * i + (e >> 2) * 8 + hi * 4 + (e & 3);
        k.out[(long long)m * k.rows + rr] = acc[i][e] * inv;
        if (k.ypre) k.ypre[(long long)m * k.rows + rr] = acc[i][e];
      }
  }
}
extern "C" int dfmir_nce_head_fwd(const float* const* srcs, int G, const long long* ids, const float* w1, const float* b1,
                                  const float* w2, const float* b2, float* out, float* nrm, float* xs, float* hs,
                                  float* ypre, int Bper, int C, long long S, int P, float eps, void* stream) {
  DF_ARG_CHECK(srcs && ids && w1 && b1 && w2 && b2 && out && G > 0 && G <= 8 && Bper > 0 && C > 0 && C <= NH_CMAX && S > 0 && P > 0);
  NceHeadP k{};
  for (int g = 0; g < G; ++g) {
    DF_ARG_CHECK(srcs[g] != nullptr);
    k.srcs.p[g] = srcs[g];
  }
  k.ids = ids; k.w1 = w1; k.b1 = b1; k.w2 = w2; k.b2 = b2;
  k.out = out; k.nrm = nrm; k.xs = xs; k.hs = hs; k.ypre = ypre;
  k.G = G; k.Bper = Bper; k.C = C; k.P = P; k.S = S; k.rows = (long long)G * Bper * P; k.eps = eps;
  nce_head_fwd_k<<<(unsigned)((k.rows + NH_R - 1) / NH_R), 256, 0, (hipStream_t)stream>>>(k);
  DF_LAUNCH_CHECK();
  return 0;
}

__global__ __launch_bounds__(256) void segment_means_k(const float* __restrict__ rows, float* __restrict__ out, int L,
                                                       int T, long long seg, float scale) {
  __shared__ float sm[17];
  const int t = blockIdx.x;
  float s = 0.f;
  for (int l = 0; l < L; ++l) {
    const float* r = rows + ((long long)l * T + t) * seg;
    for (long long i = threadIdx.x; i < seg; i += 256) s += r[i];
  }
  s = block_sum(s, sm);
  if (threadIdx.x == 0) out[t] = s * (scale / (float)seg);
}
__global__ void segment_means_bwd_k(const float* __restrict__ g, float* __restrict__ drows, int L, int T, long long seg,
                                    float scale) {
  const long long total = (long long)L * T * seg;
  for (long long i = (long long)blockIdx.x * blockDim.x + threadIdx.x; i < total;
       i += (long long)gridDim.x * blockDim.x) {
    const int t = (int)((i / seg) % T);
    drows[i] = g[t] * (scale / (float)seg);
  }
}
extern "C" int dfmir_segment_means_fwd(const float* rows, float* out, int L, int T, long long seg, float scale,
                                       void* stream) {
  DF_ARG_CHECK(rows && out && L > 0 && T > 0 && seg > 0);
  segment_means_k<<<(unsigned)T, 256, 0, (hipStream_t)stream>>>(rows, out, L, T, seg, scale);
  DF_LAUNCH_CHECK();
  return 0;
}
extern "C" int dfmir_segment_means_bwd(const float* gout, float* drows, int L, int T, long long seg, float scale,
                                       void* stream) {
  DF_ARG_CHECK(gout && drows && L > 0 && T > 0 && seg > 0);
  segment_means_bwd_k<<<df_grid((long long)L * T * seg, 256, 1024), 256, 0, (hipStream_t)stream>>>(gout, drows, L, T, seg,
                                                                                                scale);
  DF_LAUNCH_CHECK();
  return 0;
}

struct DfCombine {
  const float* in[8];
  float M[8][8];
};
__global__ void scalar_combine_k(DfCombine c, int n_in, int n_out, float* __restrict__ out) {
  const int j = threadIdx.x;
  if (j < n_out) {
    float s = 0.f;
    for (int i = 0; i < n_in; ++i) s += c.M[j][i] * c.in[i][0];
    out[j] = s;
  }
}
__global__ void scalar_combine_bwd_k(DfCombine c, const float* __restrict__ g, int n_in, int n_out,
                                     float* __restrict__ din) {
  const int i = threadIdx.x;
  if (i < n_in) {
    float s = 0.f;
    for (int j = 0; j < n_out; ++j) s += c.M[j][i] * g[j];
    din[i] = s;
  }
}
extern "C" int dfmir_scalar_combine_fwd(const float* const* in, int n_in, const float* M, int n_out, float* out,
                                        void* stream) {
  DF_ARG_CHECK(in && M && out && n_in > 0 && n_in <= 8 && n_out > 0 && n_out <= 8);
  DfCombine c{};
  for (int i = 0; i < n_in; ++i) {
    DF_ARG_CHECK(in[i] != nullptr);
    c.in[i] = in[i];
  }
  for (int j = 0; j < n_out; ++j)
    for (int i = 0; i < n_in; ++i) c.M[j][i] = M[j * n_in + i];
  scalar_combine_k<<<1, 64, 0, (hipStream_t)stream>>>(c, n_in, n_out, out);
  DF_LAUNCH_CHECK();
  return 0;
}
extern "C" int dfmir_scalar_combine_bwd(const float* gout, int n_in, const float* M, int n_out, float* din,
                                        void* stream) {
  DF_ARG_CHECK(gout && M && din && n_in > 0 && n_in <= 8 && n_out > 0 && n_out <= 8);
  DfCombine c{};
  for (int j = 0; j < n_out; ++j)
    for (int i = 0; i < n_in; ++i) c.M[j][i] = M[j * n_in + i];
  scalar_combine_bwd_k<<<1, 64, 0, (hipStream_t)stream>>>(c, gout, n_in, n_out, din);
  DF_LAUNCH_CHECK();
  return 0;
}

__global__ void probe_merge_k(const float* __restrict__ a, const float* __restrict__ b, float* __restrict__ out) {
  out[threadIdx.x] = fmaxf(a[threadIdx.x], b[threadIdx.x]);
}
extern "C" int dfmir_probe_merge(const float* a, const float* b, float* out, void* stream) {
  DF_ARG_CHECK(a && b && out);
  probe_merge_k<<<1, DF_PROBE_SLOTS, 0, (hipStream_t)stream>>>(a, b, out);
  DF_LAUNCH_CHECK();
  return 0;
}
```

dfmir_amd/networks.py:

```python
import functools
import os
import math

import numpy as np
import torch
import torch.nn as nn
from torch.nn import init
from torch.optim import lr_scheduler

from . import ops


class _ConvNd(nn.Module):

    def __init__(self, nd, in_channels, out_channels, kernel_size, stride=1, padding=0, bias=True):
        super().__init__()
        self.nd = nd
        self.in_channels, self.out_channels = in_channels, out_channels
        self.kernel_size, self.stride, self.padding = kernel_size, stride, padding
        self.weight = nn.Parameter(torch.empty((out_channels, in_channels) + (kernel_size,) * nd))
        self.bias = nn.Parameter(torch.empty(out_channels)) if bias else None
        self._packs = {}
        self.reset_parameters()

# ... 239 lines not shown
            stop = encode_only and idx == last
            if idx in want:
                if shared and not stop and t is feat:
                    feat, t = ops.fork_tap(t)
                feats.append(t)
            return stop

        while i < n:
            m = mods[i]
            gb = getattr(self, 'grad_boundary', None)
            if gb is not None and i == gb[0] and feat.requires_grad and torch.is_grad_enabled():
                feat.register_hook(lambda g_, cb=gb[1]: (cb(), None)[1])
            if isinstance(m, ReflectionPad2d) and i + 1 < n and isinstance(mods[i + 1], Conv2d):
                if i in want:
                    if emit(i, m(feat), shared=False):
                        return feat, feats, True
                conv = mods[i + 1]
                tanh = i + 2 < n and isinstance(mods[i + 2], Tanh) and (i + 1) not in want
                feat = _reflect_conv(m, conv, feat, act=2 if tanh else 0)
                if emit(i + 1, feat):
                    return feat, feats, True
                i += 2
                if tanh:
                    if emit(i, feat):
                        return feat, feats, True
                    i += 1
                continue
            if isinstance(m, Conv2d):
                tanh = i + 1 < n and isinstance(mods[i + 1], Tanh) and i not in want
                feat = m(feat, act=2 if tanh else 0)
                if emit(i, feat):
                    return feat, feats, True
                i += 1
                if tanh:
                    if emit(i, feat):
                        return feat, feats, True
                    i += 1
                continue
            if (isinstance(m, InstanceNorm2d) and i + 2 < n and isinstance(mods[i + 1], ReLU)
                    and isinstance(mods[i + 2], Downsample) and not ({i, i + 1, i + 2} & want)
                    and ops.in_relu_blurdown_ok(feat)):
                feat = ops.instance_norm_relu_blur_down(feat, m.eps)
                i += 3
                continue
            if isinstance(m, InstanceNorm2d):
                relu = i + 1 < n and isinstance(mods[i + 1], ReLU)
                feat = m(feat, relu=relu)
                if emit(i, feat):
                    return feat, feats, True
                i += 1
                if relu:
                    if emit(i, feat):
                        return feat, feats, True
                    i += 1
                continue
            feat = m(feat)
            if emit(i, feat):
                return feat, feats, True
            i += 1
        return feat, feats, False

    def forward(self, input, layers=[], encode_only=False):
        if -1 in layers:
            layers.append(len(self.model))
        if len(layers) > 0:
            feat, feats, stopped = self._run(input, list(layers), encode_only)
            if stopped:
                return feats
            return feat, feats
        feat, _, _ = self._run(input, [], False)
        return feat


def define_G(input_nc, output_nc, ngf, netG, norm='batch', use_dropout=False, init_type='normal',
             init_gain=0.02, no_antialias=False, no_antialias_up=False, gpu_ids=[], opt=None):
    norm_layer = get_norm_layer(norm_type=norm)
    blocks = {'resnet_9blocks': 9, 'resnet_6blocks': 6, 'resnet_4blocks': 4}
    if netG not in blocks:
        raise NotImplementedError('Generator model name [%s] is not recognized' % netG)
    net = ResnetGenerator(input_nc, output_nc, ngf, norm_layer=norm_layer, use_dropout=use_dropout,
                          no_antialias=no_antialias, no_antialias_up=no_antialias_up, n_blocks=blocks[netG], opt=opt)
    return init_net(net, init_type, init_gain, gpu_ids, initialize_weights=True)


class Normalize(nn.Module):

    def __init__(self, power=2):
        super().__init__()
        if power != 2:
            raise NotImplementedError("only the L2 Normalize is on the path")
        self.power = power

    def forward(self, x_rows_c):
        return ops.l2norm_rows(_as_channel_major(x_rows_c)).t()


def _as_channel_major(x_rows_c):
    t = x_rows_c.t()
    return t if t.is_contiguous() else t.contiguous()


class PatchSampleF(nn.Module):

    def __init__(self, use_mlp=False, init_type='normal', init_gain=0.02, nc=256, gpu_ids=[]):
        super().__init__()
        self.l2norm = Normalize(2)
        self.use_mlp = use_mlp
        self.nc = nc
        self.mlp_init = False
        self.init_type = init_type
        self.init_gain = init_gain
        self.gpu_ids = gpu_ids

    def create_mlp(self, feats):
        for mlp_id, feat in enumerate(feats):
            input_nc = feat.shape[1]
            mlp = nn.Sequential(Linear(input_nc, self.nc), ReLU(), Linear(self.nc, self.nc))
            mlp.to(feat.device)
            setattr(self, 'mlp_%d' % mlp_id, mlp)
        init_net(self, self.init_type, self.init_gain, self.gpu_ids)
        self.mlp_init = True

    def forward(self, feats, num_patches=64, patch_ids=None):
        return_ids, return_feats = [], []
        if self.use_mlp and not self.mlp_init:
            self.create_mlp(feats)
        for feat_id, feat in enumerate(feats):
            if num_patches <= 0:
                raise NotImplementedError("num_patches=0 (dense features) is not on the path")
            S = feat.shape[2] * feat.shape[3]
            if patch_ids is not None:
                patch_id = patch_ids[feat_id]
            else:
                patch_id = torch.randperm(S, device=feats[0].device)
                patch_id = ops.mark_distinct(patch_id[:int(min(num_patches, patch_id.shape[0]))])
            groups = patch_id.shape[0] if patch_id.dim() == 2 else 1
            x = ops.patch_gather(feat, patch_id, groups)
            return_ids.append(patch_id)
            return_feats.append(self.project(feat_id, x).t())
        return return_feats, return_ids

    def sample_project(self, feat_id, feat, ids, groups=1):
        if ops.nce_head_ok(feat.shape[1], self.nc, self.use_mlp):
            mlp = getattr(self, 'mlp_%d' % feat_id)
            return ops.nce_head(feat, ids, mlp[0], mlp[2])
        return self.project(feat_id, ops.patch_gather(feat, ids, groups))

    def sample_project_multi(self, feat_id, srcs, ids):
        if ops.nce_head_ok(srcs[0].shape[1], self.nc, self.use_mlp):
            mlp = getattr(self, 'mlp_%d' % feat_id)
            return ops.nce_head_multi(srcs, ids, mlp[0], mlp[2])
        return self.project(feat_id, ops.patch_gather_multi(srcs, ids))

    def project(self, feat_id, x_cm):
        if self.use_mlp:
            mlp = getattr(self, 'mlp_%d' % feat_id)
            x_cm = mlp[2](mlp[0](x_cm, relu=True))
        return ops.l2norm_rows(x_cm)


def define_F(input_nc, netF, norm='batch', use_dropout=False, init_type='normal', init_gain=0.02,
             no_antialias=False, gpu_ids=[], opt=None):
    if netF == 'sample':
        net = PatchSampleF(use_mlp=False, init_type=init_type, init_gain=init_gain, gpu_ids=gpu_ids, nc=opt.netF_nc)
    elif netF == 'mlp_sample':
        net = PatchSampleF(use_mlp=True, init_type=init_type, init_gain=init_gain, gpu_ids=gpu_ids, nc=opt.netF_nc)
    else:
        raise NotImplementedError('projection model name [%s] is not recognized' % netF)
    return init_net(net, init_type, init_gain, gpu_ids)


class GANLoss(nn.Module):

    def __init__(self, gan_mode, target_real_label=1.0, target_fake_label=0.0):
        super().__init__()
        self.gan_mode = gan_mode

    def forward(self, *a, **k):
        raise NotImplementedError("the registration model is discriminator-free (lambda_GAN = 0)")
```

dfmir_amd/ops.py:

```python
import collections
import ctypes
import functools
import os

import numpy as np
import torch
from torch.autograd import Function
from torch.autograd.function import once_differentiable

from ._lib import DfConvGeom, DfmirHipError, check, lib

_VP = ctypes.c_void_p


def _p(t):
    return None if t is None else _VP(t.data_ptr())


def _st():
    return _VP(torch.cuda.current_stream().cuda_stream)


def _need(*ts):
    for t in ts:
# ... 1781 lines not shown

    @staticmethod
    @once_differentiable
    def backward(ctx, dout):
        (ids,) = ctx.saved_tensors
        shape, B, C, S, Pn, G, distinct = ctx.meta
        dout = _c(dout)
        if ctx.stash is not None:
            ctx.stash.append((dout, ids, ctx.meta))
            return None, None, None, None
        dfeat = zeros(shape, dout.device)
        if distinct:
            check(lib().dfmir_patch_gather_bwd_g(_p(dout), _p(ids), _p(dfeat), B, C, S, Pn, G, None, _st()))
        else:
            check(lib().dfmir_patch_gather_bwd_any(_p(dout), _p(ids), _p(dfeat), B, C, S, Pn, G, None, None, _st()))
        return dfeat, None, None, None


def mark_distinct(ids):
    ids._df_distinct = (ids._version, ids.data_ptr())
    return ids


def ids_distinct(ids, groups=1):
    tag = getattr(ids, "_df_distinct", None)
    if tag is not None and tag == (ids._version, ids.data_ptr()):
        return True
    key = (ids._version, ids.data_ptr(), int(groups))
    seen = getattr(ids, "_df_distinct_checked", None)
    if seen is not None and seen[0] == key:
        return seen[1]
    if torch.cuda.is_current_stream_capturing():
        return False
    srt = torch.sort(ids.reshape(int(groups), -1), dim=1).values
    hit = bool((srt[:, 1:] != srt[:, :-1]).all()) if srt.shape[1] > 1 else True
    ids._df_distinct_checked = (key, hit)
    return hit


def patch_gather(feat, ids, groups=1):
    distinct = ids_distinct(ids, groups) if (torch.is_grad_enabled() and feat.requires_grad) else True
    return PatchGatherFn.apply(feat, ids, groups, distinct)


class L2NormFn(Function):

    @staticmethod
    def forward(ctx, x, eps):
        _need(x)
        x = _c(x)
        C, rows = x.shape
        y = torch.empty_like(x)
        nrm = torch.empty(rows, device=x.device, dtype=torch.float32)
        check(lib().dfmir_l2norm_fwd(_p(x), _p(y), _p(nrm), C, rows, float(eps), _st()))
        ctx.save_for_backward(x, nrm)
        ctx.eps = float(eps)
        return y

    @staticmethod
    @once_differentiable
    def backward(ctx, dy):
        x, nrm = ctx.saved_tensors
        dy = _c(dy)
        dx = torch.empty_like(x)
        check(lib().dfmir_l2norm_bwd(_p(dy), _p(x), _p(nrm), _p(dx), x.shape[0], x.shape[1], ctx.eps, _st()))
        return dx, None


def l2norm_rows(x, eps=1e-7):
    return L2NormFn.apply(x, eps)


class PatchNCEFn(Function):

    @staticmethod
    def forward(ctx, q, k, groups, T):
        _need(q, k)
        q, k = _c(q), _c(k)
        C, rows = q.shape
        if rows % groups != 0:
            raise DfmirHipError("patchnce: rows %d not divisible by groups %d" % (rows, groups))
        R = rows // groups
        loss = torch.empty(rows, device=q.device, dtype=torch.float32)
        probs = torch.empty((rows, R + 1), device=q.device, dtype=torch.float32)
        check(lib().dfmir_patchnce_fwd(_p(q), _p(k), _p(loss), _p(probs), rows, C, groups, float(T), _st()))
        ctx.save_for_backward(probs, k)
        ctx.meta = (rows, C, groups, float(T))
        return loss

    @staticmethod
    @once_differentiable
    def backward(ctx, dloss):
        probs, k = ctx.saved_tensors
        rows, C, groups, T = ctx.meta
        dloss = _c(dloss)
        dq = torch.empty_like(k)
        check(lib().dfmir_patchnce_bwd(_p(dloss), _p(probs), _p(k), _p(dq), rows, C, groups, T, _st()))
        return dq, None, None, None


def patchnce_rows(q, k, groups, T):
    return PatchNCEFn.apply(q, k, groups, T)


class NCETermsFn(Function):

    @staticmethod
    def forward(ctx, groups, temp, scale, n_terms, *qk):
        L = len(qk) // 2
        qs = [_c(t) for t in qk[:L]]
        ks = [_c(t) for t in qk[L:]]
        _need(*qs)
        _need(*ks)
        rows = qs[0].shape[1]
        if rows % n_terms or rows % groups:
            raise DfmirHipError("nce_terms: %d rows, %d terms, %d groups" % (rows, n_terms, groups))
        seg = rows // n_terms
        R = rows // groups
        dev = qs[0].device
        buf = torch.empty((L, rows), device=dev, dtype=torch.float32)
        probs = []
        for l in range(L):
            C = qs[l].shape[0]
            pr = torch.empty((rows, R + 1), device=dev, dtype=torch.float32)
            check(lib().dfmir_patchnce_fwd(_p(qs[l]), _p(ks[l]), _VP(buf.data_ptr() + 4 * l * rows), _p(pr), rows, C,
                                           groups, float(temp), _st()))
            probs.append(pr)
        out = torch.empty(n_terms, device=dev, dtype=torch.float32)
        check(lib().dfmir_segment_means_fwd(_p(buf), _p(out), L, n_terms, seg, float(scale), _st()))
        ctx.save_for_backward(*(probs + ks))
        ctx.meta = (L, rows, seg, groups, float(temp), float(scale), n_terms, [q.shape[0] for q in qs])
        ctx.rows_buf = buf
        return out

    @staticmethod
    @once_differentiable
    def backward(ctx, g):
        L, rows, seg, groups, temp, scale, n_terms, Cs = ctx.meta
        saved = ctx.saved_tensors
        probs, ks = saved[:L], saved[L:]
        g = _c(g)
        drows = torch.empty((L, rows), device=g.device, dtype=torch.float32)
        check(lib().dfmir_segment_means_bwd(_p(g), _p(drows), L, n_terms, seg, scale, _st()))
        dqs = []
        for l in range(L):
            dq = torch.empty_like(ks[l])
            check(lib().dfmir_patchnce_bwd(_VP(drows.data_ptr() + 4 * l * rows), _p(probs[l]), _p(ks[l]), _p(dq), rows,
                                           Cs[l], groups, temp, _st()))
            dqs.append(dq)
        return (None, None, None, None) + tuple(dqs) + (None,) * L


def nce_terms(qs, ks, groups, temp, scale, n_terms):
    return NCETermsFn.apply(int(groups), temp, scale, int(n_terms), *(list(qs) + [k.detach() for k in ks]))


class ScalarCombineFn(Function):

    @staticmethod
    def forward(ctx, M, *ins):
        import numpy as np
        _need(*ins)
        n_in, n_out = len(ins), len(M)
        Mh = np.ascontiguousarray(np.asarray(M, dtype=np.float32).reshape(n_out, n_in))
        ptrs = (ctypes.c_void_p * n_in)(*[t.data_ptr() for t in ins])
        out = torch.empty(n_out, device=ins[0].device, dtype=torch.float32)
        check(lib().dfmir_scalar_combine_fwd(ptrs, n_in, Mh.ctypes.data, n_out, _p(out), _st()))
        ctx.M = Mh
        ctx.shapes = [tuple(t.shape) for t in ins]
        return out

    @staticmethod
    @once_differentiable
    def backward(ctx, g):
        g = _c(g)
        n_out, n_in = ctx.M.shape
        din = torch.empty(n_in, device=g.device, dtype=torch.float32)
        check(lib().dfmir_scalar_combine_bwd(_p(g), n_in, ctx.M.ctypes.data, n_out, _p(din), _st()))
        return (None,) + tuple(din[i].view(ctx.shapes[i]) for i in range(n_in))


def scalar_combine(M, ins):
    return ScalarCombineFn.apply(M, *ins)


_IDS_STATE = {}


def _cuda_device(device):
    device = torch.device("cuda" if device is None else device)
    if device.type != "cuda":
        raise DfmirHipError("patch ids are drawn on the HIP device, not on %s" % device)
    return torch.device("cuda", torch.cuda.current_device() if device.index is None else device.index)


def seed_patch_ids(seed, device=None):
    device = _cuda_device(device)
    new = torch.tensor([int(seed) & 0x7FFFFFFFFFFFFFFF, 0, 0], dtype=torch.int64)
    st = _IDS_STATE.get(device)
    if st is None:
        st = _IDS_STATE[device] = new.to(device)
    else:
        st.copy_(new)
    return st


def draw_patch_ids(sizes, n_sets, P, device):
    device = _cuda_device(device)
    st = _IDS_STATE.get(device)
    if st is None:
        st = seed_patch_ids(torch.initial_seed(), device)
    L = len(sizes)
    out = torch.empty((L, n_sets, P), device=device, dtype=torch.int64)
    sz = (ctypes.c_longlong * L)(*[int(s) for s in sizes])
    check(lib().dfmir_patch_ids_draw(_p(st), sz, L, int(n_sets), int(P), _p(out), _st()))
    return mark_distinct(out)


def patch_gather_multi(srcs, ids):
    _need(*srcs)
    _need(ids)
    G = len(srcs)
    srcs = [_c(s) for s in srcs]
    Bper, C = srcs[0].shape[0], srcs[0].shape[1]
    S = srcs[0].numel() // (Bper * C)
    for s_ in srcs:
        if tuple(s_.shape) != tuple(srcs[0].shape):
            raise DfmirHipError("patch_gather_multi: sources differ in shape")
    ids = _c(ids.to(torch.int64))
    if ids.dim() != 2 or ids.shape[0] != G:
        raise DfmirHipError("patch_gather_multi: ids must be [G, P]")
    Pn = ids.shape[1]
    out = torch.empty((C, G * Bper * Pn), device=srcs[0].device, dtype=torch.float32)
    ptrs = (ctypes.c_void_p * G)(*[s_.data_ptr() for s_ in srcs])
    check(lib().dfmir_patch_gather_fwd_multi(ptrs, G, _p(ids), _p(out), Bper, C, S, Pn, _st()))
    return out


def nce_head_ok(C, nc, use_mlp):
    return use_mlp and nc == 256 and 1 <= C <= 256


def _nce_head_launch(ptrs, G, ids, mlp0, mlp2, Bper, C, S, Pn, eps, device, save):
    rows = G * Bper * Pn
    out = torch.empty((256, rows), device=device, dtype=torch.float32)
    nrm = xs = hs = ypre = None
    if save:
        nrm = torch.empty(rows, device=device, dtype=torch.float32)
        xs = torch.empty((C, rows), device=device, dtype=torch.float32)
        hs = torch.empty((256, rows), device=device, dtype=torch.float32)
        ypre = torch.empty((256, rows), device=device, dtype=torch.float32)
    arr = (ctypes.c_void_p * G)(*ptrs)
    check(lib().dfmir_nce_head_fwd(arr, G, _p(ids), _p(mlp0.packed(0)), _p(mlp0.bias), _p(mlp2.packed(0)), _p(mlp2.bias),
                                   _p(out), _p(nrm), _p(xs), _p(hs), _p(ypre), Bper, C, S, Pn, float(eps), _st()))
    return out, nrm, xs, hs, ypre


def nce_head_multi(srcs, ids, mlp0, mlp2, eps=1e-7):
    _need(*srcs)
    srcs = [_c(s_) for s_ in srcs]
    Bper, C = srcs[0].shape[0], srcs[0].shape[1]
    S = srcs[0].numel() // (Bper * C)
    ids = _c(ids.to(torch.int64))
    out, _, _, _, _ = _nce_head_launch([s_.data_ptr() for s_ in srcs], len(srcs), ids, mlp0, mlp2, Bper, C, S, ids.shape[1], eps,
                                       srcs[0].device, False)
    return out


class NceHeadFn(Function):

    @staticmethod
    def forward(ctx, feat, ids, w1, b1, w2, b2, mlp0, mlp2, eps, distinct):
        _need(feat, ids)
        ctx.stash = getattr(feat, "_df_tap_stash", None) if feat.is_contiguous() else None
        feat = _c(feat)
        ids = _c(ids.to(torch.int64))
        G, Pn = ids.shape
        B, C = feat.shape[0], feat.shape[1]
        if B % G:
            raise DfmirHipError("nce_head: ids [G,P] with G dividing the batch")
        Bper = B // G
        S = feat.numel() // (B * C)
        base = feat.data_ptr()
        ptrs = [base + 4 * g * Bper * C * S for g in range(G)]
        out, nrm, xs, hs, ypre = _nce_head_launch(ptrs, G, ids, mlp0, mlp2, Bper, C, S, Pn, eps, feat.device, True)
        ctx.save_for_backward(ids, nrm, xs, hs, ypre, w1, w2)
        ctx.meta = (tuple(feat.shape), B, C, S, Pn, G, bool(distinct), float(eps))
        ctx.mods = (mlp0, mlp2)
        return out

    @staticmethod
    @once_differentiable
    def backward(ctx, dout):
        ids, nrm, xs, hs, ypre, w1, w2 = ctx.saved_tensors
        shape, B, C, S, Pn, G, distinct, eps = ctx.meta
        mlp0, mlp2 = ctx.mods
        rows = B * Pn
        dout = _c(dout)
        dy = torch.empty_like(ypre)
        check(lib().dfmir_l2norm_bwd(_p(dout), _p(ypre), _p(nrm), _p(dy), 256, rows, eps, _st()))
        c2 = _Ctx()
        c2.cfg, c2.x_amax, c2.dead_tail, c2.in_act, c2.has_bias = (2, (1, 1, 1), 1, (0, 0, 0), 0, 0, 0.0, mlp2), None, 0, None, True
        c2.needs_input_grad = (True, ctx.needs_input_grad[4], ctx.needs_input_grad[5])
        dh, dw2, db2 = _conv_backward_impl(c2, dy.view(1, 256, 1, rows), None, hs.view(1, 256, 1, 1, rows),
                                           w2.view(256, 256, 1, 1), None)
        c1 = _Ctx()
        c1.cfg, c1.x_amax, c1.dead_tail, c1.in_act, c1.has_bias = (2, (1, 1, 1), 1, (0, 0, 0), 0, 1, 0.0, mlp0), None, 0, None, True
        c1.needs_input_grad = (ctx.needs_input_grad[0], ctx.needs_input_grad[2], ctx.needs_input_grad[3])
        dx, dw1, db1 = _conv_backward_impl(c1, dh, None, xs.view(1, C, 1, 1, rows), w1.view(256, C, 1, 1),
                                           hs.view(1, 256, 1, 1, rows))
        dfeat = None
        if dx is not None:
            dxr = _c(dx).view(C, rows)
            meta = (shape, B, C, S, Pn, G, distinct)
            if ctx.stash is not None:
                ctx.stash.append((dxr, ids, meta))
            else:
                dfeat = zeros(shape, dxr.device)
                if distinct:
                    check(lib().dfmir_patch_gather_bwd_g(_p(dxr), _p(ids), _p(dfeat), B, C, S, Pn, G, None, _st()))
                else:
                    check(lib().dfmir_patch_gather_bwd_any(_p(dxr), _p(ids), _p(dfeat), B, C, S, Pn, G, None, None, _st()))
        dw1 = dw1.view(256, C) if dw1 is not None else None
        dw2 = dw2.view(256, 256) if dw2 is not None else None
        return dfeat, None, dw1, db1, dw2, db2, None, None, None, None


def nce_head(feat, ids, mlp0, mlp2, eps=1e-7):
    groups = ids.shape[0] if ids.dim() == 2 else 1
    ids2 = ids if ids.dim() == 2 else ids.view(1, -1)
    distinct = ids_distinct(ids, groups) if (torch.is_grad_enabled() and feat.requires_grad) else True
    return NceHeadFn.apply(feat, ids2, mlp0.weight, mlp0.bias, mlp2.weight, mlp2.bias, mlp0, mlp2, eps, distinct)


_LAST_L1_WS = [None]


class MaskedL1Fn(Function):
    @staticmethod
    def forward(ctx, a, b, mask, thr):
        _need(a, b, mask)
        a, b = _c(a), _c(b)
        m = None
        if mask is not None:
            m = _c(mask.to(torch.bool))
            if m.shape != a.shape:
                m = _c(m.expand_as(a))
        ws = torch.empty(8, device=a.device, dtype=torch.float32)
        out = torch.empty((), device=a.device, dtype=torch.float32)
        check(lib().dfmir_masked_l1_fwd(_p(a), _p(b), _p(m), float(thr), _p(ws), _p(out), a.numel(), _st()))
        _LAST_L1_WS[0] = ws
        ctx.save_for_backward(a, b, m, ws)
        ctx.thr = float(thr)
        return out

    @staticmethod
    @once_differentiable
    def backward(ctx, g):
        a, b, m, ws = ctx.saved_tensors
        g = _c(g)
        da = torch.empty_like(a) if ctx.needs_input_grad[0] else None
        db = torch.empty_like(b) if ctx.needs_input_grad[1] else None
        if da is not None or db is not None:
            check(lib().dfmir_masked_l1_bwd(_p(a), _p(b), _p(m), ctx.thr, _p(ws), _p(g), _p(da), _p(db),
                                            a.numel(), _st()))
        return da, db, None, None


def masked_l1(a, b, mask=None, thr=-0.95):
    out = MaskedL1Fn.apply(a, b, mask, thr)
    out._df_mask_sum = _LAST_L1_WS[0][1]
    return out


class FlowSmoothFn(Function):
    @staticmethod
    def forward(ctx, flow, penalty=2):
        _need(flow)
        flow = _c(flow)
        nd = flow.dim() - 2
        B, C = flow.shape[0], flow.shape[1]
        D, H, W = flow.shape[2:] if nd == 3 else (1,) + tuple(flow.shape[2:])
        ws = torch.empty(int(lib().dfmir_flow_smooth_ws_floats()), device=flow.device, dtype=torch.float32)
        out = torch.empty((), device=flow.device, dtype=torch.float32)
        if penalty == 2:
            check(lib().dfmir_flow_smooth_fwd(_p(flow), _p(ws), _p(out), B, C, D, H, W, _st()))
        else:
            check(lib().dfmir_flow_smooth_fwd_p(_p(flow), _p(ws), _p(out), B, C, D, H, W, int(penalty), _st()))
        ctx.save_for_backward(flow)
        ctx.meta = (B, C, D, H, W, int(penalty))
        return out

    @staticmethod
    @once_differentiable
    def backward(ctx, g):
        (flow,) = ctx.saved_tensors
        B, C, D, H, W, penalty = ctx.meta
        g = _c(g)
        df = torch.empty_like(flow)
        if penalty == 2:
            check(lib().dfmir_flow_smooth_bwd(_p(flow), _p(g), _p(df), B, C, D, H, W, _st()))
        else:
            check(lib().dfmir_flow_smooth_bwd_p(_p(flow), _p(g), _p(df), B, C, D, H, W, penalty, _st()))
        return df, None


def flow_smoothness(flow, penalty='l2'):
    if penalty not in ('l1', 'l2'):
        raise DfmirHipError("gradient penalty must be 'l1' or 'l2', got %r" % (penalty,))
    return FlowSmoothFn.apply(flow, 2 if penalty == 'l2' else 1)


def bending_spacing(spacing, lengths, what):
    if spacing is None:
        return (1.0,) * lengths[0]
    try:
        vals = tuple(spacing)
    except TypeError:
        vals = None
    if vals is None or isinstance(spacing, str) or len(vals) not in lengths:
        raise ValueError("%s: spacing must be a sequence of %s numbers, got %r"
                         % (what, " or ".join(str(n) for n in lengths), spacing))
    for v in vals:
        if isinstance(v, bool) or not isinstance(v, (int, float, np.integer, np.floating)) \
                or not np.isfinite(v) or not 0.0 < float(np.float32(v)) < float('inf'):
            raise ValueError("%s: spacing must hold positive finite numbers, got %r" % (what, spacing))
    return tuple(float(v) for v in vals)


def bending_geom(flow, spacing, what):
    if flow.dim() not in (4, 5):
        raise ValueError("%s: expects a [B,C,H,W] or [B,C,D,H,W] field, got %d dims" % (what, flow.dim()))
    nd = flow.dim() - 2
    B, C = int(flow.shape[0]), int(flow.shape[1])
    D, H, W = (int(v) for v in (flow.shape[2:] if nd == 3 else (1,) + tuple(flow.shape[2:])))
    if B < 1 or C < 1:
        raise ValueError("%s: empty tensor %s" % (what, tuple(flow.shape)))
    short = [n for n in ((H, W) if D == 1 else (D, H, W)) if n < 3]
    if short:
        raise ValueError("%s: every axis needs an extent of at least 3 (a voxel with its whole 3^nd neighbourhood inside "
                         "the volume), got %s" % (what, tuple(flow.shape[2:])))
    if B * C * D * H * W >= 2 ** 31:
        raise ValueError("%s: fields of 2^31 and more elements are not supported, got %s" % (what, tuple(flow.shape)))
    sp = bending_spacing(spacing, (2,) if nd == 2 else ((2, 3) if D == 1 else (3,)), what)
    hz, hy, hx = sp if len(sp) == 3 else (1.0,) + sp
    return B, C, D, H, W, hz, hy, hx


class BendingEnergyFn(Function):

    @staticmethod
    def forward(ctx, flow, geom):
        flow = _c(flow)
        B, C, D, H, W, hz, hy, hx = geom
        ws = torch.empty(int(lib().dfmir_bend_ws_floats(B, C, D, H, W)), device=flow.device, dtype=torch.float32)
        out = torch.empty((), device=flow.device, dtype=torch.float32)
        check(lib().dfmir_bend_fwd(_p(flow), _p(ws), _p(out), B, C, D, H, W, hz, hy, hx, _st()))
        ctx.save_for_backward(flow)
        ctx.meta = geom
        return out

    @staticmethod
    @once_differentiable
    def backward(ctx, g):
        (flow,) = ctx.saved_tensors
        B, C, D, H, W, hz, hy, hx = ctx.meta
        g = _c(g)
        df = torch.empty_like(flow)
        check(lib().dfmir_bend_bwd(_p(flow), _p(g), _p(df), B, C, D, H, W, hz, hy, hx, _st()))
        return df, None


def bending_energy(flow, spacing=None):
    geom = bending_geom(flow, spacing, "bending_energy")
    _need(flow)
    if flow.dtype != torch.float32:
        raise DfmirHipError("bending_energy: fp32 tensors only (got %s)" % flow.dtype)
    return BendingEnergyFn.apply(flow, geom)


def _jacobian_geom(flow, border, what):
    if not torch.is_tensor(flow) or flow.dim() not in (4, 5):
        raise ValueError("%s: expects a [B,2,H,W] or [B,3,D,H,W] displacement field, got %s"
                         % (what, "%d dims" % flow.dim() if torch.is_tensor(flow) else type(flow).__name__))
    nd = flow.dim() - 2
    if int(flow.shape[1]) != nd:
        raise ValueError("%s: a %d-D field needs %d channels, one displacement per axis, got %s"
# ... 1386 lines not shown
```

dfmir_amd/registration_model.py:

```python
import os

import numpy as np
import torch

from . import networks, ops
from . import voxelmorph as vxm
from .base_model import BaseModel
from .losses import NCC_Loss, smooothing_loss
from .optim import FlatAdam
from .patchnce import PatchNCELoss
from .voxelmorph import SpatialTransformer


def str2bool(v):
    if isinstance(v, bool):
        return v
    if v.lower() in ('yes', 'true', 't', 'y', '1'):
        return True
    if v.lower() in ('no', 'false', 'f', 'n', '0'):
        return False
    import argparse
    raise argparse.ArgumentTypeError('Boolean value expected.')


# ... 468 lines not shown
        streams = {'g': cur, 'r': rs}
        done = {}
        ops.begin_deferred()
        try:
            for name, sk, fn, after in self._step_pieces():
                for dep in after:
                    streams[sk].wait_event(done[dep])
                with torch.cuda.stream(streams[sk]):
                    fn()
                done[name] = torch.cuda.Event()
                done[name].record(streams[sk])
        except BaseException:
            cur.wait_stream(rs)
            ops.end_deferred(failed=True)
            raise

    def _capture_staged(self, side, mode):
        rs = self._r_stream()
        streams = {'g': side, 'r': rs}
        pools = {'g': torch.cuda.graph_pool_handle(), 'r': torch.cuda.graph_pool_handle()}
        graphs = []
        ops.begin_deferred()
        try:
            for name, sk, fn, after in self._step_pieces():
                g = torch.cuda.CUDAGraph()
                with torch.cuda.graph(g, pool=pools[sk], stream=streams[sk], capture_error_mode=mode):
                    fn()
                graphs.append((name, sk, g, after))
        except BaseException:
            ops._DEFER["on"] = False
            ops._DEFER["pending"] = {}
            raise
        return graphs

    def _replay_staged(self, graphs):
        cur, rs = torch.cuda.current_stream(), self._r_stream()
        streams = {'g': cur, 'r': rs}
        evs = self._graph_state().setdefault('events', {})
        for name, sk, g, after in graphs:
            s = streams[sk]
            for dep in after:
                s.wait_event(evs[dep])
            if s is cur:
                g.replay()
            else:
                with torch.cuda.stream(s):
                    g.replay()
            if name not in evs:
                evs[name] = torch.cuda.Event()
            evs[name].record(s)

    def _global_mask_norm(self, *terms):
        import torch.distributed as dist
        from . import distributed as dfdist
        m = torch.stack([t._df_mask_sum for t in terms])
        tot = m.clone()
        if dfdist._staged(tot):
            h = tot.cpu()
            dist.all_reduce(h)
            tot = h.to(m.device)
        else:
            dist.all_reduce(tot)
        f = torch.where(tot > 0, m * float(dfdist.world_size()) / tot.clamp_min(1e-30), torch.ones_like(m))
        return tuple(t * f[i] for i, t in enumerate(terms))

    def set_input(self, input):
        AtoB = self.opt.direction == 'AtoB'
        self.real_A = input['A' if AtoB else 'B'].to(self.device, non_blocking=True)
        self.real_B = input['B' if AtoB else 'A'].to(self.device, non_blocking=True)
        self.image_paths = input['A_paths' if AtoB else 'B_paths']

    def forward(self):
        self.real = ops.cat_batch(self.real_A, self.real_B)
        self.flipped_for_equivariance = False
        if self.opt.flip_equivariance:
            draw = getattr(self, 'flip_draw', None)
            self.flipped_for_equivariance = self.isTrain and bool(draw() if draw is not None else np.random.random() < 0.5)
            if self.flipped_for_equivariance:
                self.real = torch.flip(self.real, [3])
        nb = self.real_A.size(0)
        self._key_feats = None
        if (self.isTrain and self.opt.lambda_NCE > 0.0 and getattr(self.opt, 'reuse_key_features', True)
                and not self.flipped_for_equivariance):
            self.fake, feats = self.netG(self.real, self.nce_layers, encode_only=False)
            self._key_feats = ((self.real_A, [f[:nb].detach() for f in feats]),
                               (self.real_B, [f[nb:].detach() for f in feats]))
        else:
            self.fake = self.netG(self.real)
        self.fake_B = self.fake[:nb]
        self.idt_B = self.fake[nb:]

    def _encode_keys(self, src):
        for owner, feats in (self._key_feats or ()):
            if owner is src:
                return feats
        return self.netG(src, self.nce_layers, encode_only=True)

    def compute_G_loss(self):
        if self.opt.lambda_GAN > 0.0:
            raise NotImplementedError("the registration model is discriminator-free (lambda_GAN must be 0)")
        self.loss_G_GAN = 0.0
        if self.opt.lambda_NCE > 0.0:
            self.loss_NCE = self.calculate_NCE_loss(self.real_A, self.fake_B)
        else:
            self.loss_NCE, self.loss_NCE_bd = 0.0, 0.0
        if self.opt.nce_idt and self.opt.lambda_NCE > 0.0:
            self.loss_NCE_Y = self.calculate_NCE_loss(self.real_B, self.idt_B)
            loss_NCE_both = (self.loss_NCE + self.loss_NCE_Y) * 0.5
        else:
            loss_NCE_both = self.loss_NCE
        self.loss_G = self.loss_G_GAN + loss_NCE_both
        return self.loss_G

    def calculate_NCE_loss(self, src, tgt):
        n_layers = len(self.nce_layers)
        feat_q = self.netG(tgt, self.nce_layers, encode_only=True)
        if self.opt.flip_equivariance and self.flipped_for_equivariance:
            feat_q = [torch.flip(fq, [3]) for fq in feat_q]
        with torch.no_grad():
            feat_k = self._encode_keys(src)
            pinned = None
            if getattr(self, 'patch_id_source', None) is not None:
                sets = self._patch_id_sets([f.shape[2] * f.shape[3] for f in feat_k], 1, self.opt.num_patches, feat_k[0].device)
                pinned = [sets[l][0] for l in range(len(feat_k))]
            feat_k_pool, sample_ids = self.netF(feat_k, self.opt.num_patches, pinned)
        feat_q_pool, _ = self.netF(feat_q, self.opt.num_patches, sample_ids)
        total_nce_loss = 0.0
        for f_q, f_k, crit, nce_layer in zip(feat_q_pool, feat_k_pool, self.criterionNCE, self.nce_layers):
            loss = crit(f_q, f_k)
            total_nce_loss += ops.mean(loss) * self.opt.lambda_NCE
        return total_nce_loss / n_layers

    def calculate_NCE_losses_stacked(self, terms, tgt=None):
        T = len(terms)
        n_layers = len(self.nce_layers)
        if tgt is None:
            tgt = ops.cat_batch(self.fake, terms[2][1]) if T == 3 else ops.cat_batch(terms[0][1], terms[1][1])
        feat_q = self.netG(tgt, self.nce_layers, encode_only=True)
        if self.opt.flip_equivariance and self.flipped_for_equivariance:
            feat_q = [torch.flip(fq, [3]) for fq in feat_q]
        sizes = [f.shape[2] * f.shape[3] for f in feat_q]
        P = self.opt.num_patches
        per_term_groups = 1 if self.opt.nce_includes_all_negatives_from_minibatch else self.opt.batch_size
        sequential = getattr(self.opt, 'nce_sequential_keys', False) or 'forward' in vars(self.netF)
        if not sequential and self.opt.netF == 'mlp_sample' and all(S >= 2 * P or P <= S <= 4096 for S in sizes):
            id_src = getattr(self, 'patch_id_source', None)
            self._nce_on_device = id_src is None or bool(getattr(id_src, 'graph_safe', False))
            ids = self._patch_id_sets(sizes, T, P, feat_q[0].device)
            with torch.no_grad():
                keys = {}
                for src, _ in terms:
                    if id(src) not in keys:
                        keys[id(src)] = self._encode_keys(src)
                k_cm = [self.netF.sample_project_multi(l, [keys[id(src)][l] for src, _ in terms], ids[l])
                        for l in range(n_layers)]
            q_cm = [self.netF.sample_project(l, feat_q[l], ids[l], T) for l in range(n_layers)]
            losses = ops.nce_terms(q_cm, k_cm, T * per_term_groups, self.opt.nce_T,
                                   self.opt.lambda_NCE / n_layers, T)
            return list(losses.unbind(0))
        self._nce_on_device = False
        pools_k, ids_t = [], []
        with torch.no_grad():
            for src, _ in terms:
                pool, ids = self.netF(self._encode_keys(src), self.opt.num_patches, None)
                pools_k.append(pool)
                ids_t.append(ids)
        ids_stacked = [torch.stack([ids_t[t][l] for t in range(T)]) for l in range(n_layers)]
        for l in range(n_layers):
            if all(getattr(ids_t[t][l], "_df_distinct", None) is not None for t in range(T)):
                ops.mark_distinct(ids_stacked[l])
        fq_pool, _ = self.netF(feat_q, self.opt.num_patches, ids_stacked)
        losses = []
        for t in range(T):
            total = 0.0
            for l, crit in enumerate(self.criterionNCE):
                f_q = fq_pool[l]
                rows = f_q.shape[0] // T
                total += ops.mean(crit(f_q[t * rows:(t + 1) * rows], pools_k[t][l])) * self.opt.lambda_NCE
            losses.append(total / n_layers)
        return losses

    def _patch_id_sets(self, sizes, n_sets, P, device):
        src = getattr(self, 'patch_id_source', None)
        if src is None:
            ids = ops.draw_patch_ids(sizes, n_sets, P, device)
            return [ops.mark_distinct(ids[l]) for l in range(len(sizes))]
        ids = src(sizes, n_sets, P)
        out = [ids[l].to(device) for l in range(len(sizes))]
        if getattr(src, 'distinct', False):
            out = [ops.mark_distinct(t) for t in out]
        return out

    def calculate_L1_loss(self, src, tgt, mask):
        if mask is None:
            return ops.masked_l1(src, tgt, torch.ones_like(src, dtype=torch.bool))
        if isinstance(mask, str):
            return ops.masked_l1(src, tgt, None, -0.95)
        return ops.masked_l1(src, tgt, mask)
```

include/dfmir_hip.h:

```cpp
#ifndef DFMIR_HIP_H
#define DFMIR_HIP_H

#ifdef __cplusplus
extern "C" {
#endif

#define DFMIR_ABI_VERSION 14

int dfmir_abi_version(void);
const char* dfmir_last_error(void);

int dfmir_set_option(const char* name, const char* value);
int dfmir_get_option(const char* name, char* buf, int buf_len);

typedef struct DfConvGeom {
  int N, Cin, Cout;
  int Di, Hi, Wi;
  int Do, Ho, Wo;
  int KD, KH, KW;
  int stride, dil;
  int pd, ph, pw;
  int pad_mode;
  int act;
  float slope;
// ... 70 lines not shown
                            void* stream);
int dfmir_conv_wgrad_scaled_ch(const DfConvGeom* g, const float* x, const float* x_amax, int x_amax_n, const float* dy,
                               const float* dy_amax, int dy_amax_n, const float* dy_pmax, float* dw_tcc, float* db,
                               void* stream);
int dfmir_bias_grad(const float* dy, float* db, int N, int C, long long S, void* stream);
long long dfmir_weight_pack_floats(int Cout, int Cin, int T);
int dfmir_weight_pack(const float* w, float* w_tcc, int Cout, int Cin, int T, int mode, void* stream);
int dfmir_weight_unpack(const float* g_tcc, float* g, int Cout, int Cin, int T, void* stream);
int dfmir_conv3x3_res_ok(const DfConvGeom* g);
int dfmir_conv3x3_fwd_scaled_res(const DfConvGeom* g, const float* x, const float* x_amax, int x_amax_n,
                                 const float* w_tcc, const float* bias, const float* res, const float* ring,
                                 int ring_len, float* y, void* stream);

int dfmir_conv3x3_reflect_ring_ok(const DfConvGeom* g);
int dfmir_conv3x3_reflect_ring_len(const DfConvGeom* g);
int dfmir_conv3x3_reflect_ring(const DfConvGeom* g, const float* dy, const float* dy_cols, const float* dy_amax,
                               int dy_amax_n, const float* wd_packed, float* ring, void* stream);

int dfmir_conv3x3_bwd_pair_ok(const DfConvGeom* gd, const DfConvGeom* gw);
int dfmir_conv3x3_bwd_pair(const DfConvGeom* gd, const DfConvGeom* gw, const float* dy, const float* dy_amax,
                           int dy_amax_n, const float* dy_pmax, const float* wd_packed, const float* res,
                           const float* ring, int ring_len, float* dx, const float* x, const float* x_amax,
                           int x_amax_n, float* dw_tcc, float* db, int* paired, void* stream);

typedef struct DfPackJob {
  const float* w;
  float* packed;
  int Cout, Cin, T, mode;
} DfPackJob;
int dfmir_weight_pack_batch(const DfPackJob* jobs, int njobs, void* table_dev, int upload, void* stream);

typedef struct DfUnpackJob {
  float* src;
  float* dst;
  int Cout, Cin, T, reserved;
} DfUnpackJob;
int dfmir_weight_unpack_add_batch(const DfUnpackJob* jobs, int njobs, long long max_total, void* stream);

int dfmir_conv7x7_c1_fwd(const float* x, const float* w, const float* bias, float* y, int N, int H, int W, int Cout,
                         int pad_mode, void* stream);
int dfmir_conv7x7_c1_wgrad(const float* x, const float* dy, float* dw, float* db, int N, int H, int W, int Cout,
                           int pad_mode, void* stream);

int dfmir_tapstack_fwd(const float* x, float* s, int N, int C, int H, int W, int K, int pad,
                       int pad_mode, void* stream);
int dfmir_tapstack_bwd(const float* ds, float* dx, int N, int C, int H, int W, int K, int pad,
                       int pad_mode, void* stream);
int dfmir_tapsum_fwd(const float* z, const float* bias, float* y, int N, int C, int Hz, int Wz, int Ho,
                     int Wo, int K, int opad, int pad_mode, int act, float slope, void* stream);
int dfmir_tapsum_bwd(const float* dy, float* dz, int N, int C, int Hz, int Wz, int Ho, int Wo, int K,
                     int opad, int pad_mode, void* stream);

int dfmir_instnorm_stats_ok(long long S);
int dfmir_instnorm_stats(const float* x, float* mean, float* rstd, int planes, long long S, float eps, int relu,
                         float* y_amax, void* stream);
int dfmir_instnorm_fwd(const float* x, const float* res, float* y, float* mean, float* rstd,
                       int planes, long long S, float eps, int relu, float* y_amax, void* stream);
int dfmir_instnorm_bwd(const float* dy, const float* x, const float* mean, const float* rstd,
                       float* dx, int planes, long long S, int relu, float* dx_amax, void* stream);
int dfmir_instnorm_bwd_cols_ok(long long S, int W);
int dfmir_instnorm_bwd_cols(const float* dy, const float* x, const float* mean, const float* rstd, float* dx, int planes,
                            long long S, int relu, float* dx_amax, float* dx_cols, int W, void* stream);
int dfmir_instnorm_bwd_pmax_ok(long long S);
int dfmir_instnorm_bwd_pmax(const float* dy, const float* x, const float* mean, const float* rstd, float* dx, int planes,
                            long long S, int relu, float* dx_amax, float* dx_cols, int W, float* dx_pmax, void* stream);

int dfmir_in_relu_blurdown_ok(int H, int W);
int dfmir_in_relu_blurdown_fwd(const float* x, float* z, float* mean, float* rstd, int planes, int H, int W, float eps,
                               float* z_amax, void* stream);
int dfmir_in_relu_blurdown_bwd(const float* dz, const float* x, const float* mean, const float* rstd, float* dx,
                               int planes, int H, int W, float* dx_amax, float* dx_pmax, void* stream);

int dfmir_act_bwd(const float* dy, const float* y, float* dx, long long n, int act, float slope,
                  void* stream);
int dfmir_act_bwd_amax(const float* dy, const float* y, float* dx, long long n, int act, float slope,
                       float* dx_amax, void* stream);

int dfmir_blur_down_fwd(const float* x, float* y, int planes, int H, int W, void* stream);
int dfmir_blur_down_bwd(const float* dy, float* dx, int planes, int H, int W, void* stream);
int dfmir_blur_up_fwd(const float* x, float* y, int planes, int H, int W, void* stream);
int dfmir_blur_up_bwd(const float* dy, float* dx, int planes, int H, int W, void* stream);
int dfmir_reflect_pad2d_fwd(const float* x, float* y, int planes, int H, int W, int p, void* stream);
int dfmir_reflect_pad2d_bwd(const float* dy, float* dx, int planes, int H, int W, int p, void* stream);
int dfmir_reflect_pad2d_bwd_add(const float* dy, const float* add, float* dx, int planes, int H, int W, int p,
                                void* stream);

int dfmir_upcat_fwd(const float* a, const float* b, float* y, int N, int Ca, int Cb, int Da, int Ha,
                    int Wa, int sd, void* stream);
int dfmir_upcat_bwd(const float* dy, float* da, float* db, int N, int Ca, int Cb, int Da, int Ha,
                    int Wa, int sd, void* stream);

int dfmir_cat_channels_fwd(const float* a, const float* b, float* y, long long N, long long SA,
                           long long SB, void* stream);
int dfmir_cat_channels_bwd(const float* dy, float* da, float* db, long long N, long long SA,
                           long long SB, void* stream);
int dfmir_scale(const float* x, float* y, long long n, float mult, void* stream);

int dfmir_warp2d_fwd(const float* src, const float* flow, float* out, int B, int C, int H, int W,
                     int mode, int add_identity, void* stream);
int dfmir_warp2d_bwd(const float* dout, const float* src, const float* flow, float* dsrc,
                     float* dflow, int B, int C, int H, int W, int add_identity, int flow_into_src,
                     void* stream);
int dfmir_warp3d_fwd(const float* src, const float* flow, float* out, int B, int C, int D, int H,
                     int W, int mode, int add_identity, void* stream);
int dfmir_warp3d_bwd(const float* dout, const float* src, const float* flow, float* dsrc,
                     float* dflow, int B, int C, int D, int H, int W, int add_identity,
                     int flow_into_src, void* stream);
long long dfmir_warp_bwd_own_ws_floats(int nd, int B, int C, int D, int H, int W);
int dfmir_warp_bwd_own(int nd, const float* dout, const float* src, const float* flow, float* dsrc, float* dflow, int B,
                       int C, int D, int H, int W, int add_identity, int flow_into_src, float* ws, void* stream);

int dfmir_resize_fwd(const float* x, float* y, int planes, int Di, int Hi, int Wi, int Do, int Ho,
                     int Wo, float mult, void* stream);
int dfmir_resize_bwd(const float* dy, float* dx, int planes, int Di, int Hi, int Wi, int Do, int Ho,
                     int Wo, float mult, void* stream);
long long dfmir_resize_bwd_ws_floats(int planes, int Di, int Hi, int Wi, int Do, int Ho, int Wo);
int dfmir_resize_bwd_sep(const float* dy, float* dx, int planes, int Di, int Hi, int Wi, int Do, int Ho, int Wo,
                         float mult, float* ws, void* stream);

int dfmir_bspline_fwd(int nd, const float* ctrl, float* y, int planes, int D, int H, int W, int sz, int sy, int sx,
                      void* stream);
long long dfmir_bspline_bwd_ws_floats(int nd, int planes, int D, int H, int W, int sz, int sy, int sx);
int dfmir_bspline_bwd(int nd, const float* dy, float* dctrl, int planes, int D, int H, int W, int sz, int sy, int sx,
                      float* ws, void* stream);

int dfmir_patch_gather_fwd(const float* feat, const long long* ids, float* out, int B, int C,
                           long long S, int P, void* stream);
int dfmir_patch_gather_bwd(const float* dout, const long long* ids, float* dfeat, int B, int C,
                           long long S, int P, void* stream);
int dfmir_patch_gather_bwd_amax(const float* dout, const long long* ids, float* dfeat, int B, int C, long long S,
                                int P, float* dfeat_amax, void* stream);
int dfmir_patch_gather_fwd_g(const float* feat, const long long* ids, float* out, int B, int C, long long S, int P,
                             int G, void* stream);
int dfmir_patch_gather_bwd_g(const float* dout, const long long* ids, float* dfeat, int B, int C, long long S, int P,
                             int G, float* dfeat_amax, void* stream);
int dfmir_patch_gather_bwd_gp(const float* dout, const long long* ids, float* dfeat, int B, int C, long long S, int P,
                              int G, float* dfeat_amax, float* dfeat_pmax, void* stream);
int dfmir_patch_gather_bwd_any(const float* dout, const long long* ids, float* dfeat, int B, int C, long long S, int P,
                               int G, float* dfeat_amax, float* dfeat_pmax, void* stream);
int dfmir_patch_gather_fwd_multi(const float* const* srcs, int G, const long long* ids, float* out, int Bper, int C,
                                 long long S, int P, void* stream);
int dfmir_nce_head_fwd(const float* const* srcs, int G, const long long* ids, const float* w1, const float* b1,
                       const float* w2, const float* b2, float* out, float* nrm, float* xs, float* hs, float* ypre,
                       int Bper, int C, long long S, int P, float eps, void* stream);
int dfmir_patch_ids_draw(unsigned long long* state, const long long* sizes, int n_layers, int n_sets, int P,
                         long long* out, void* stream);
int dfmir_l2norm_fwd(const float* x, float* y, float* norm, int C, long long rows, float eps, void* stream);
int dfmir_l2norm_bwd(const float* dy, const float* x, const float* norm, float* dx, int C,
                     long long rows, float eps, void* stream);
int dfmir_patchnce_fwd(const float* q, const float* k, float* loss, float* probs, long long rows,
                       int C, int G, float T, void* stream);
int dfmir_patchnce_bwd(const float* dloss, const float* probs, const float* k, float* dq,
                       long long rows, int C, int G, float T, void* stream);

int dfmir_masked_l1_fwd(const float* a, const float* b, const unsigned char* mask, float thr,
                        float* ws, float* out, long long n, void* stream);
int dfmir_masked_l1_bwd(const float* a, const float* b, const unsigned char* mask, float thr,
                        const float* ws, const float* gout, float* da, float* db, long long n,
                        void* stream);
long long dfmir_flow_smooth_ws_floats(void);
int dfmir_flow_smooth_fwd(const float* flow, float* ws, float* out, int B, int C, int D, int H,
                          int W, void* stream);
int dfmir_flow_smooth_bwd(const float* flow, const float* gout, float* dflow, int B, int C, int D,
                          int H, int W, void* stream);
int dfmir_flow_smooth_fwd_p(const float* flow, float* ws, float* out, int B, int C, int D, int H,
                            int W, int penalty, void* stream);
int dfmir_flow_smooth_bwd_p(const float* flow, const float* gout, float* dflow, int B, int C, int D,
                            int H, int W, int penalty, void* stream);
long long dfmir_bend_ws_floats(int B, int C, int D, int H, int W);
int dfmir_bend_fwd(const float* flow, float* ws, float* out, int B, int C, int D, int H, int W, float hz, float hy,
                   float hx, void* stream);
int dfmir_bend_bwd(const float* flow, const float* gout, float* dflow, int B, int C, int D, int H, int W, float hz,
                   float hy, float hx, void* stream);
long long dfmir_jacdet_ws_floats(int nd, int B, int D, int H, int W);
int dfmir_jacdet_fwd(int nd, const float* flow, float* ws, float* out, int B, int D, int H, int W, int border, float eps,
                     int power, void* stream);
int dfmir_jacdet_bwd(int nd, const float* flow, const float* gout, float* dflow, int B, int D, int H, int W, int border,
                     float eps, int power, void* stream);
int dfmir_jacdet_map(int nd, const float* flow, float* detmap, int B, int D, int H, int W, int border, void* stream);
int dfmir_jacdet_stats(int nd, const float* flow, float* ws, double* stats, int B, int D, int H, int W, int border,
                       double log_offset, double log_floor, void* stream);
long long dfmir_invcons_ws_floats(int nd, int B, int D, int H, int W);
int dfmir_invcons_fwd(int nd, const float* u, const float* v, float* ws, float* per_sample, float* loss, float* rmax, int B,
                      int D, int H, int W, void* stream);
long long dfmir_invcons_bwd_ws_floats(int nd, int B, int D, int H, int W);
int dfmir_invcons_bwd(int nd, const float* u, const float* v, const float* gout, const float* rmax, float* du, float* dv,
                      float* ws, int B, int D, int H, int W, void* stream);
int dfmir_compose_fwd(int nd, const float* u, const float* v, float* out, int B, int D, int H, int W, void* stream);
long long dfmir_compose_bwd_ws_floats(int nd, int B, int D, int H, int W);
int dfmir_compose_bwd(int nd, const float* u, const float* v, const float* g, float* du, float* dv, float* ws, int B, int D,
                      int H, int W, void* stream);
long long dfmir_flow_invert_ws_floats(int nd, int B, int D, int H, int W, int iters, int history);
int dfmir_flow_invert(int nd, const float* u, const float* init, float* w, float* stats, float* ws, int B, int D, int H,
                      int W, int iters, float tol, int history, void* stream);
int dfmir_dsearch_pool(int nd, const float* in, float* out, float* packed, int B, int C, int D, int H, int W, int g,
                       void* stream);
int dfmir_dsearch_cost(int nd, const float* fixp, const float* movp, float* cost, int B, int C, int D, int H, int W, int r,
                       void* stream);
int dfmir_dsearch_argmin(int nd, const float* cost, const float* soft, float coeff, int* idx, float* disp, int B, int D, int H,
                         int W, int r, void* stream);
int dfmir_dsearch_smooth(int nd, const float* disp, float* out, int B, int D, int H, int W, void* stream);
long long dfmir_warp_ssd_ws_floats(int nd, int B, int C, int D, int H, int W);
int dfmir_warp_ssd_pack(int nd, const float* M, float* Mp, int B, int C, int D, int H, int W, void* stream);
int dfmir_warp_ssd_fwd(int nd, const float* Mp, const float* M, const float* F, const float* phi, const float* mask,
                       float* ws, float* per_sample, float* loss, float* scale, int B, int C, int D, int H, int W,
                       void* stream);
int dfmir_warp_ssd_fwd_grad(int nd, const float* Mp, const float* M, const float* F, const float* phi, const float* mask,
                            float* ws, float* per_sample, float* loss, float* scale, float* unit, int B, int C, int D, int H,
                            int W, void* stream);
int dfmir_warp_ssd_bwd(const float* unit, const float* gout, const float* scale, float* dflow, long long n, void* stream);
long long dfmir_affine_ws_floats(int nd, int B, int D, int H, int W);
int dfmir_affine_flow(int nd, const float* theta, float* flow, int B, int D, int H, int W, void* stream);
int dfmir_affine_flow_bwd(int nd, const float* dflow, float* ws, float* dtheta, int B, int D, int H, int W, void* stream);
int dfmir_affine_system(int nd, const float* Mp, const float* F, const float* theta, const float* mask, float* ws, double* out,
                        int full, int B, int C, int D, int H, int W, void* stream);
int dfmir_affine_lm_step(int nd, const double* Lb, const double* g, const double* H, float* theta_acc, float* trial,
                         double* state, double* hist, int B, int k, int translation, double mu_up, double mu_down,
                         void* stream);
long long dfmir_landmark_ws_floats(int nd, int B, int K, int D, int H, int W);
int dfmir_landmark_fwd(int nd, const float* flow, const float* fixed_pts, const float* moving_pts, const float* weight,
                       float* ws, float* mapped, float* d, float* per_sample, float* loss, float* wsum, int B, int K, int D,
                       int H, int W, float hz, float hy, float hx, int penalty, void* stream);
int dfmir_landmark_bwd(int nd, const float* flow, const float* fixed_pts, const float* moving_pts, const float* weight,
                       const float* gout, const float* wsum, float* dflow, float* ws, int B, int K, int D, int H, int W,
                       float hz, float hy, float hx, int penalty, void* stream);
long long dfmir_nmi_ws_floats(long long n, int nb);
int dfmir_nmi_fwd(const float* y_true, const float* y_pred, const float* mask, const float* centers, int nb,
                  float preterm, float max_clip, long long n, float* ws, float* out, void* stream);
int dfmir_nmi_bwd(const float* y_true, const float* y_pred, const float* mask, const float* centers, int nb,
                  float preterm, float max_clip, long long n, const float* ws, const float* gout, float* d_true,
                  float* d_pred, void* stream);
long long dfmir_mind_ws_floats(int nd, int B, int D, int H, int W, int radius, int dilation, int which);
int dfmir_mind_desc(const float* I, int nd, int B, int D, int H, int W, int radius, int dilation, float* ws, float* out,
                    void* stream);
int dfmir_mind_fwd(const float* a, const float* b, const float* mask, int nd, int B, int D, int H, int W, int radius,
                   int dilation, float* ws, float* out, void* stream);
int dfmir_mind_bwd(const float* a, const float* b, const float* mask, int nd, int B, int D, int H, int W, int radius,
                   int dilation, const float* ws, float* tmp, const float* gout, float* da, float* db, void* stream);
long long dfmir_gradfield_ws_floats(int nd, int B, int D, int H, int W);
int dfmir_gradfield_fwd(const float* a, const float* b, const float* mask, int nd, int B, int D, int H, int W, float hz,
                        float hy, float hx, int auto_eps, double eta, double eps_a, double eps_b, float* ws, float* out,
                        void* stream);
int dfmir_gradfield_bwd(const float* a, const float* b, const float* mask, const float* gout, const float* ws, float* da,
                        float* db, int nd, int B, int D, int H, int W, float hz, float hy, float hx, void* stream);
int dfmir_gradfield_field(const float* I, int nd, int B, int D, int H, int W, float hz, float hy, float hx, int auto_eps,
                          double eta, double eps, float* ws, float* out, void* stream);
long long dfmir_warp_dice_ws_floats(int nd, int B, int K, int D, int H, int W);
int dfmir_warp_dice_fwd(int nd, const unsigned char* mov, const unsigned char* fix, const float* flow,
                        const unsigned char* slot_of, int K, int B, int D, int H, int W, int mode, float* ws,
                        float* loss, float* dice, float* seeds, void* stream);
int dfmir_warp_dice_bwd(int nd, const unsigned char* mov, const unsigned char* fix, const float* flow,
                        const unsigned char* slot_of, int K, int B, int D, int H, int W, const float* seeds,
                        const float* gout, float* dflow, void* stream);
#define DFMIR_EDT_SQ_INF (1 << 29)
#define DFMIR_HD_SURFACE 1
long long dfmir_label_hausdorff_ws_bytes(int nd, int B, int K, int D, int H, int W);
int dfmir_label_edt_sq(int nd, const unsigned char* map, int value, int surface, int B, int D, int H, int W, int* out,
                       void* stream);
int dfmir_label_hausdorff(int nd, const unsigned char* a, const unsigned char* b, const unsigned char* labels, int K, int B,
                          int D, int H, int W, int qm, int flags, void* ws, float* hd, float* directed, float* mean,
                          int* d2, void* stream);
long long dfmir_dice_ws_floats(long long planes, long long S);
int dfmir_dice_fwd(const float* y_true, const float* y_pred, long long planes, long long S, float* ws, float* out,
                   void* stream);
int dfmir_dice_bwd(const float* y_true, const float* y_pred, long long planes, long long S, const float* ws,
                   const float* gout, float* d_true, float* d_pred, void* stream);
long long dfmir_mse_ws_floats(long long n);
int dfmir_mse_fwd(const float* y_true, const float* y_pred, long long n, float* ws, float* out, void* stream);
int dfmir_mse_bwd(const float* y_true, const float* y_pred, long long n, const float* gout, float* d_true, float* d_pred,
                  void* stream);
int dfmir_mul(const float* a, const float* b, float* out, long long n, void* stream);
int dfmir_ncc_fwd(const float* I, const float* J, float* tmp, float* tmp2, float* ws, float* out,
                  int B, int D, int H, int W, int win, float eps, void* stream);
int dfmir_ncc_bwd(const float* I, const float* J, const float* sums, float* tmp, float* tmp2,
                  const float* ws, const float* gout, float* dI, int B, int D, int H, int W,
                  int win, float eps, void* stream);
#define DFMIR_NCC_VOLUME 4
int dfmir_ncc_fwd_m(const float* I, const float* J, const float* mask, int mode, float* tmp, float* tmp2,
                    float* ws, float* out, int B, int D, int H, int W, int win, float eps, void* stream);
int dfmir_ncc_bwd_m(const float* I, const float* J, const float* mask, int mode, const float* sums,
                    float* tmp, float* tmp2, const float* ws, const float* gout, float* dI, int B, int D,
                    int H, int W, int win, float eps, void* stream);
int dfmir_ncc_gauss_fwd(const float* I, const float* J, const float* mask, int mode, float* tmp, float* tmp2,
                        float* ws, float* out, int B, int D, int H, int W, const float* taps, int K, float c,
                        float eps, void* stream);
int dfmir_ncc_gauss_bwd(const float* I, const float* J, const float* mask, int mode, const float* sums,
                        float* tmp, float* tmp2, const float* ws, const float* gout, float* dI, int B, int D,
                        int H, int W, const float* taps, int K, float c, float eps, void* stream);
int dfmir_segment_means_fwd(const float* rows, float* out, int L, int T, long long seg, float scale, void* stream);
int dfmir_segment_means_bwd(const float* gout, float* drows, int L, int T, long long seg, float scale, void* stream);
int dfmir_scalar_combine_fwd(const float* const* in, int n_in, const float* M, int n_out, float* out, void* stream);
int dfmir_scalar_combine_bwd(const float* gout, int n_in, const float* M, int n_out, float* din, void* stream);
int dfmir_fill_zero(float* p, long long n, void* stream);
int dfmir_sum_scaled(const float* x, float* out, long long n, float scale, void* stream);
int dfmir_fill_from_scalar(const float* gout, float* dx, long long n, float scale, void* stream);

int dfmir_det_head_floats(void);
int dfmir_det_begin(float* scratch, long long slots, const float* x, long long nx, const float* x_amax, int x_amax_n,
                    const float* dy, long long ndy, const float* dy_amax, int dy_amax_n, double count, void* stream);
int dfmir_det_end(const float* scratch, float* dw_out, long long n_dw, float* db_out, long long n_db, void* stream);

int dfmir_adam_step(float* p, const float* g, float* m, float* v, long long n, float lr, float beta1,
                    float beta2, float eps, float bc1, float bc2, float grad_scale, void* stream);

#ifdef __cplusplus
}
// ... 3 lines not shown
```

Measured before the change: 220.8.

## Group PatchNCE head forward and 1x1 wgrad across layers into single launches

Adds grouped kernels that batch the per-layer PatchNCE MLP head forward and the 1x1 conv weight and bias gradients of all layers into one launch each, with a device-side job table. The NCE loss path gains an autograd function covering all layers, replacing many small per-layer launches and Python dispatches. The wgrad and bias-grad kernel bodies move into shared include files so the single and grouped kernels reuse them. This adds a linear job lookup per block and a more complex fallback path.

```diff
diff --git a/dfmir_amd/_lib.py b/dfmir_amd/_lib.py
--- a/dfmir_amd/_lib.py
+++ b/dfmir_amd/_lib.py
@@ -10,6 +10,19 @@
     _fields_ = [(n, c_int) for n in (
         "N", "Cin", "Cout", "Di", "Hi", "Wi", "Do", "Ho", "Wo", "KD", "KH", "KW",
         "stride", "dil", "pd", "ph", "pw", "pad_mode", "act")] + [("slope", c_float)]
+
+
+NCE_GROUP_MAX = 16
+
+
+class DfNceHeadJob(Structure):
+    _fields_ = ([("srcs", c_void_p * 8), ("ids", c_void_p)]
+                + [(n, c_void_p) for n in ("w1", "b1", "w2", "b2", "out", "nrm", "xs", "hs", "ypre")]
+                + [(n, c_int) for n in ("G", "Bper", "C", "P")] + [("S", c_longlong)])
+
+
+class DfWgradJob(Structure):
+    _fields_ = [(n, c_void_p) for n in ("x", "dy", "dw_tcc", "db")] + [("Cin", c_int), ("Cout", c_int)]
 
 
 P = c_void_p
@@ -201,6 +214,9 @@
     "dfmir_ncc_bwd": [P, P, P, P, P, P, P, P] + [c_int] * 5 + [c_float, P],
     "dfmir_patch_gather_fwd_multi": [P, c_int, P, P, c_int, c_int, c_longlong, c_int, P],
     "dfmir_nce_head_fwd": [P, c_int, P, P, P, P, P, P, P, P, P, P, c_int, c_int, c_longlong, c_int, c_float, P],
+    "dfmir_nce_head_fwd_group": [P, c_int, c_float, P],
+    "dfmir_conv1x1_wgrad_group_ok": [c_int, c_int, c_longlong, P, P],
+    "dfmir_conv1x1_wgrad_group": [P, c_int, c_longlong, P],
     "dfmir_patch_ids_draw": [P, P, c_int, c_int, c_int, P, P],
     "dfmir_segment_means_fwd": [P, P, c_int, c_int, c_longlong, c_float, P],
     "dfmir_segment_means_bwd": [P, P, c_int, c_int, c_longlong, c_float, P],
diff --git a/dfmir_amd/csrc/bias_grad_body.inc b/dfmir_amd/csrc/bias_grad_body.inc
--- /dev/null
+++ b/dfmir_amd/csrc/bias_grad_body.inc
@@ -0,0 +1,19 @@
+  __shared__ float sm[17];
+  const int c = BG_C, n = BG_N, part = BG_PART;
+  const long long per = (((S + nsplit - 1) / nsplit) + 3) & ~3LL;
+  const long long beg = part * per;
+  long long end = beg + per;
+  if (end > S) end = S;
+  const float* p = dy + ((long long)n * C + c) * S;
+  float s = 0.f;
+  if ((S & 3) == 0) {
+    const float4* p4 = reinterpret_cast<const float4*>(p);
+    for (long long i = (beg >> 2) + threadIdx.x; i < (end >> 2); i += blockDim.x) {
+      const float4 v = p4[i];
+      s += (v.x + v.y) + (v.z + v.w);
+    }
+  } else {
+    for (long long i = beg + threadIdx.x; i < end; i += blockDim.x) s += p[i];
+  }
+  s = block_sum(s, sm);
+  if (threadIdx.x == 0 && beg < S) df_acc(db, c, s, fx);
diff --git a/dfmir_amd/csrc/conv.hip b/dfmir_amd/csrc/conv.hip
--- a/dfmir_amd/csrc/conv.hip
+++ b/dfmir_amd/csrc/conv.hip
@@ -458,88 +458,24 @@
                                                        float* __restrict__ dwt, int N, int Cin, int Cout, long long S,
                                                        long long chunks_per_img, long long chunks_per_block,
                                                        const float* __restrict__ fx) {
-  constexpr int BK = 64, LD = BK + 1;
-  __shared__ float Xs[64 * LD];
-  __shared__ float Ds[64 * LD];
-  const int tid = threadIdx.x, lane = tid & 63, wid = tid >> 6;
-  const int l31 = lane & 31, lhi = lane >> 5, wm = wid >> 1, wn = wid & 1;
-  const int ci0 = blockIdx.y * 64, co0 = blockIdx.z * 64;
-  const long long total = (long long)N * chunks_per_img;
-  const long long cbeg = (long long)blockIdx.x * chunks_per_block;
-  long long cend = cbeg + chunks_per_block;
-  if (cend > total) cend = total;
-  const int r = tid >> 2, q16 = (tid & 3) * 16;
-  const bool xrow = ci0 + r < Cin, drow = co0 + r < Cout;
-  float4 rx[4], rd[4];
-  const float4 z4 = make_float4(0.f, 0.f, 0.f, 0.f);
-#define G1_GLOAD(c_)                                                                                         \
-  {                                                                                                          \
-    const long long n_ = (c_) / chunks_per_img, q0_ = ((c_) - n_ * chunks_per_img) * BK + q16;               \
-    const float* xp_ = x + ((long long)n_ * Cin + ci0 + r) * S + q0_;                                        \
-    const float* dp_ = dy + ((long long)n_ * Cout + co0 + r) * S + q0_;                                      \
-    _Pragma("unroll") for (int j = 0; j < 4; ++j) {                                                          \
-      const bool in_ = q0_ + 4 * j < S;                                                                      \
-      rx[j] = (xrow && in_) ? *reinterpret_cast<const float4*>(xp_ + 4 * j) : z4;                            \
-      rd[j] = (drow && in_) ? *reinterpret_cast<const float4*>(dp_ + 4 * j) : z4;                            \
-    }                                                                                                        \
-  }
-#define G1_LSTORE()                                                                                          \
-  {                                                                                                          \
-    float* xs_ = &Xs[r * LD + q16];                                                                          \
-    float* ds_ = &Ds[r * LD + q16];                                                                          \
-    _Pragma("unroll") for (int j = 0; j < 4; ++j) {                                                          \
-      xs_[4 * j] = rx[j].x; xs_[4 * j + 1] = rx[j].y; xs_[4 * j + 2] = rx[j].z; xs_[4 * j + 3] = rx[j].w;    \
-      ds_[4 * j] = rd[j].x; ds_[4 * j + 1] = rd[j].y; ds_[4 * j + 2] = rd[j].z; ds_[4 * j + 3] = rd[j].w;    \
-    }                                                                                                        \
-  }
-  f32x16 acc;
-#pragma unroll
-  for (int i = 0; i < 16; ++i) acc[i] = 0.f;
-  if (cbeg < cend) G1_GLOAD(cbeg)
-  for (long long c = cbeg; c < cend; ++c) {
-    __syncthreads();
-    G1_LSTORE()
-    __syncthreads();
-    if (c + 1 < cend) G1_GLOAD(c + 1)
-    const float* ap = &Xs[(wm * 32 + l31) * LD + lhi];
-    const float* bp = &Ds[(wn * 32 + l31) * LD + lhi];
-#pragma unroll 8
-    for (int ks = 0; ks < BK / 2; ++ks)
-      acc = __builtin_amdgcn_mfma_f32_32x32x2f32(ap[2 * ks], bp[2 * ks], acc, 0, 0, 0);
-  }
-#undef G1_GLOAD
-#undef G1_LSTORE
-  const int co = co0 + wn * 32 + l31;
-  if (co < Cout && cbeg < cend) {
-#pragma unroll
-    for (int i = 0; i < 16; ++i) {
-      const int ci = ci0 + wm * 32 + 4 * lhi + (i & 3) + 8 * (i >> 2);
-      if (ci < Cin) df_acc(dwt, (long long)ci * Cout + co, acc[i], fx);
-    }
-  }
+#define G1_BX blockIdx.x
+#define G1_BY blockIdx.y
+#define G1_BZ blockIdx.z
+#include "conv1x1_wgrad_body.inc"
+#undef G1_BX
+#undef G1_BY
+#undef G1_BZ
 }
 
 __global__ void bias_grad_k(const float* __restrict__ dy, float* __restrict__ db, int N, int C,
                             long long S, int nsplit, const float* __restrict__ fx) {
-  __shared__ float sm[17];
-  const int c = blockIdx.x, n = blockIdx.y, part = blockIdx.z;
-  const long long per = (((S + nsplit - 1) / nsplit) + 3) & ~3LL;
-  const long long beg = part * per;
-  long long end = beg + per;
-  if (end > S) end = S;
-  const float* p = dy + ((long long)n * C + c) * S;
-  float s = 0.f;
-  if ((S & 3) == 0) {
-    const float4* p4 = reinterpret_cast<const float4*>(p);
-    for (long long i = (beg >> 2) + threadIdx.x; i < (end >> 2); i += blockDim.x) {
-      const float4 v = p4[i];
-      s += (v.x + v.y) + (v.z + v.w);
-    }
-  } else {
-    for (long long i = beg + threadIdx.x; i < end; i += blockDim.x) s += p[i];
-  }
-  s = block_sum(s, sm);
-  if (threadIdx.x == 0 && beg < S) df_acc(db, c, s, fx);
+#define BG_C blockIdx.x
+#define BG_N blockIdx.y
+#define BG_PART blockIdx.z
+#include "bias_grad_body.inc"
+#undef BG_C
+#undef BG_N
+#undef BG_PART
 }
 
 __global__ __launch_bounds__(256) void weight_pack_k(const float* __restrict__ w, float* __restrict__ o, int Cout,
@@ -827,6 +763,25 @@
   return conv_wgrad_impl(g, x, x_amax, x_amax_n, dy, dy_amax, dy_amax_n, dw_tcc, db, stream);
 }
 static int bias_grad_launch(const float* dy, float* db, int N, int C, long long S, hipStream_t st);
+static bool conv1x1_wgrad_takes(int Cin, int Cout, long long S1, const float* x, const float* dy) {
+  static DfOptFlag no1x1_o{"DFMIR_NO_1X1_WGRAD"};
+  return !use_generic_only() && !no1x1_o.get() && (S1 & 3) == 0 && S1 >= 64 &&
+         ((reinterpret_cast<uintptr_t>(x) | reinterpret_cast<uintptr_t>(dy)) & 15) == 0 && Cin >= 8 && Cout >= 8;
+}
+static void conv1x1_wgrad_plan(int N, int Cin, int Cout, long long S1, long long& cpi, long long& cpb, unsigned& nx,
+                               unsigned& ny, unsigned& nz) {
+  cpi = (S1 + 63) / 64;
+  const long long total = (long long)N * cpi;
+  ny = (unsigned)((Cin + 63) / 64);
+  nz = (unsigned)((Cout + 63) / 64);
+  long long want = 1024 / ((long long)ny * nz);
+  if (want < 1) want = 1;
+  long long maxs = (total + 7) / 8;
+  if (maxs < 1) maxs = 1;
+  if (want > maxs) want = maxs;
+  cpb = (total + want - 1) / want;
+  nx = (unsigned)((total + cpb - 1) / cpb);
+}
 static int conv_wgrad_impl(const DfConvGeom* g, const float* x, const float* x_amax, int x_n, const float* dy,
                            const float* dy_amax, int dy_n, float* dw_tcc, float* db, void* stream, const float* dy_pmax) {
   DF_ARG_CHECK(check_geom(g) == 0 && x && dy && dw_tcc);
@@ -847,20 +802,12 @@
     if (df_conv3d_wgrad_try(g, x, dy, dw_tcc, st, &rc)) return rc;
   }
   {
-    static DfOptFlag no1x1_o{"DFMIR_NO_1X1_WGRAD"};
     const long long S1 = (long long)g->Di * g->Hi * g->Wi;
-    if (!use_generic_only() && !no1x1_o.get() && g->KD == 1 && g->KH == 1 && g->KW == 1 && g->stride == 1 && g->pd == 0 &&
-        g->ph == 0 && g->pw == 0 && g->Do == g->Di && g->Ho == g->Hi && g->Wo == g->Wi && (S1 & 3) == 0 && S1 >= 64 &&
-        ((reinterpret_cast<uintptr_t>(x) | reinterpret_cast<uintptr_t>(dy)) & 15) == 0 && g->Cin >= 8 && g->Cout >= 8) {
-      const long long cpi = (S1 + 63) / 64, total = (long long)g->N * cpi;
-      const unsigned ny = (unsigned)((g->Cin + 63) / 64), nz = (unsigned)((g->Cout + 63) / 64);
-      long long want = 1024 / ((long long)ny * nz);
-      if (want < 1) want = 1;
-      long long maxs = (total + 7) / 8;
-      if (maxs < 1) maxs = 1;
-      if (want > maxs) want = maxs;
-      const long long cpb = (total + want - 1) / want;
-      const unsigned nx = (unsigned)((total + cpb - 1) / cpb);
+    if (g->KD == 1 && g->KH == 1 && g->KW == 1 && g->stride == 1 && g->pd == 0 && g->ph == 0 && g->pw == 0 &&
+        g->Do == g->Di && g->Ho == g->Hi && g->Wo == g->Wi && conv1x1_wgrad_takes(g->Cin, g->Cout, S1, x, dy)) {
+      long long cpi, cpb;
+      unsigned nx, ny, nz;
+      conv1x1_wgrad_plan(g->N, g->Cin, g->Cout, S1, cpi, cpb, nx, ny, nz);
       conv1x1_wgrad_k<<<dim3(nx, ny, nz), 256, 0, st>>>(x, dy, dw_tcc, g->N, g->Cin, g->Cout, S1, cpi, cpb, df_det_fx());
       DF_LAUNCH_CHECK();
       return 0;
@@ -924,6 +871,79 @@
   return bias_grad_launch(dy, db, N, C, S, (hipStream_t)stream);
 }
 
+struct G1GroupTab {
+  const float* x[DF_NCE_GROUP_MAX];
+  const float* dy[DF_NCE_GROUP_MAX];
+  float* dw[DF_NCE_GROUP_MAX];
+  float* db[DF_NCE_GROUP_MAX];
+  long long cpb[DF_NCE_GROUP_MAX];
+  int Cin[DF_NCE_GROUP_MAX], Cout[DF_NCE_GROUP_MAX];
+  unsigned nx[DF_NCE_GROUP_MAX], ny[DF_NCE_GROUP_MAX];
+  unsigned first[DF_NCE_GROUP_MAX + 1];
+};
+__global__ __launch_bounds__(256) void conv1x1_wgrad_group_k(G1GroupTab t, int njobs, long long S, long long chunks_per_img,
+                                                             const float* __restrict__ fx) {
+  int job = 0;
+  while (job + 1 < njobs && blockIdx.x >= t.first[job + 1]) ++job;
+  const unsigned local = blockIdx.x - t.first[job];
+  const unsigned G1_BX = local % t.nx[job], rest = local / t.nx[job];
+  const unsigned G1_BY = rest % t.ny[job], G1_BZ = rest / t.ny[job];
+  const float* __restrict__ x = t.x[job];
+  const float* __restrict__ dy = t.dy[job];
+  float* __restrict__ dwt = t.dw[job];
+  const int N = 1, Cin = t.Cin[job], Cout = t.Cout[job];
+  const long long chunks_per_block = t.cpb[job];
+#include "conv1x1_wgrad_body.inc"
+}
+__global__ void bias_grad_group_k(G1GroupTab t, long long S, int nsplit, const float* __restrict__ fx) {
+  const int C = t.Cout[blockIdx.y];
+  const float* __restrict__ dy = t.dy[blockIdx.y];
+  float* __restrict__ db = t.db[blockIdx.y];
+  if ((int)blockIdx.x >= C || db == nullptr) return;
+#define BG_C blockIdx.x
+#define BG_N 0
+#define BG_PART blockIdx.z
+#include "bias_grad_body.inc"
+#undef BG_C
+#undef BG_N
+#undef BG_PART
+}
+extern "C" int dfmir_conv1x1_wgrad_group_ok(int Cin, int Cout, long long rows, const float* x, const float* dy) {
+  return (Cin > 0 && Cout > 0 && rows > 0 && x && dy && df_det_fx() == nullptr &&
+          conv1x1_wgrad_takes(Cin, Cout, rows, x, dy)) ? 1 : 0;
+}
+extern "C" int dfmir_conv1x1_wgrad_group(const DfWgradJob* jobs, int njobs, long long rows, void* stream) {
+  DF_ARG_CHECK(jobs && njobs > 0 && njobs <= DF_NCE_GROUP_MAX && rows > 0);
+  hipStream_t st = (hipStream_t)stream;
+  G1GroupTab t{};
+  unsigned nwg = 0;
+  int cmax = 0;
+  bool any_db = false;
+  long long cpi = 0;
+  for (int j = 0; j < njobs; ++j) {
+    const DfWgradJob& a = jobs[j];
+    DF_ARG_CHECK(a.x && a.dy && a.dw_tcc && dfmir_conv1x1_wgrad_group_ok(a.Cin, a.Cout, rows, a.x, a.dy));
+    unsigned nx, ny, nz;
+    conv1x1_wgrad_plan(1, a.Cin, a.Cout, rows, cpi, t.cpb[j], nx, ny, nz);
+    t.x[j] = a.x; t.dy[j] = a.dy; t.dw[j] = a.dw_tcc; t.db[j] = a.db;
+    t.Cin[j] = a.Cin; t.Cout[j] = a.Cout; t.nx[j] = nx; t.ny[j] = ny;
+    t.first[j] = nwg;
+    nwg += nx * ny * nz;
+    if (a.db) { any_db = true; if (a.Cout > cmax) cmax = a.Cout; }
+  }
+  t.first[njobs] = nwg;
+  if (any_db) {
+    int nsplit = (int)((rows + 65535) / 65536);
+    if (nsplit > 64) nsplit = 64;
+    bias_grad_group_k<<<dim3((unsigned)cmax, (unsigned)njobs, (unsigned)nsplit), rows >= 4096 ? 256 : 64, 0, st>>>(
+        t, rows, nsplit, df_det_fx());
+    DF_LAUNCH_CHECK();
+  }
+  conv1x1_wgrad_group_k<<<nwg, 256, 0, st>>>(t, njobs, rows, cpi, df_det_fx());
+  DF_LAUNCH_CHECK();
+  return 0;
+}
+
 extern "C" int dfmir_weight_pack(const float* w, float* w_tcc, int Cout, int Cin, int T, int mode,
                                  void* stream) {
   DF_ARG_CHECK(w && w_tcc && Cout > 0 && Cin > 0 && T > 0 && (mode == 0 || mode == 1));
diff --git a/dfmir_amd/csrc/conv1x1_wgrad_body.inc b/dfmir_amd/csrc/conv1x1_wgrad_body.inc
--- /dev/null
+++ b/dfmir_amd/csrc/conv1x1_wgrad_body.inc
@@ -0,0 +1,59 @@
+  constexpr int BK = 64, LD = BK + 1;
+  __shared__ float Xs[64 * LD];
+  __shared__ float Ds[64 * LD];
+  const int tid = threadIdx.x, lane = tid & 63, wid = tid >> 6;
+  const int l31 = lane & 31, lhi = lane >> 5, wm = wid >> 1, wn = wid & 1;
+  const int ci0 = G1_BY * 64, co0 = G1_BZ * 64;
+  const long long total = (long long)N * chunks_per_img;
+  const long long cbeg = (long long)G1_BX * chunks_per_block;
+  long long cend = cbeg + chunks_per_block;
+  if (cend > total) cend = total;
+  const int r = tid >> 2, q16 = (tid & 3) * 16;
+  const bool xrow = ci0 + r < Cin, drow = co0 + r < Cout;
+  float4 rx[4], rd[4];
+  const float4 z4 = make_float4(0.f, 0.f, 0.f, 0.f);
+#define G1_GLOAD(c_)                                                                                         \
+  {                                                                                                          \
+    const long long n_ = (c_) / chunks_per_img, q0_ = ((c_) - n_ * chunks_per_img) * BK + q16;               \
+    const float* xp_ = x + ((long long)n_ * Cin + ci0 + r) * S + q0_;                                        \
+    const float* dp_ = dy + ((long long)n_ * Cout + co0 + r) * S + q0_;                                      \
+    _Pragma("unroll") for (int j = 0; j < 4; ++j) {                                                          \
+      const bool in_ = q0_ + 4 * j < S;                                                                      \
+      rx[j] = (xrow && in_) ? *reinterpret_cast<const float4*>(xp_ + 4 * j) : z4;                            \
+      rd[j] = (drow && in_) ? *reinterpret_cast<const float4*>(dp_ + 4 * j) : z4;                            \
+    }                                                                                                        \
+  }
+#define G1_LSTORE()                                                                                          \
+  {                                                                                                          \
+    float* xs_ = &Xs[r * LD + q16];                                                                          \
+    float* ds_ = &Ds[r * LD + q16];                                                                          \
+    _Pragma("unroll") for (int j = 0; j < 4; ++j) {                                                          \
+      xs_[4 * j] = rx[j].x; xs_[4 * j + 1] = rx[j].y; xs_[4 * j + 2] = rx[j].z; xs_[4 * j + 3] = rx[j].w;    \
+      ds_[4 * j] = rd[j].x; ds_[4 * j + 1] = rd[j].y; ds_[4 * j + 2] = rd[j].z; ds_[4 * j + 3] = rd[j].w;    \
+    }                                                                                                        \
+  }
+  f32x16 acc;
+#pragma unroll
+  for (int i = 0; i < 16; ++i) acc[i] = 0.f;
+  if (cbeg < cend) G1_GLOAD(cbeg)
+  for (long long c = cbeg; c < cend; ++c) {
+    __syncthreads();
+    G1_LSTORE()
+    __syncthreads();
+    if (c + 1 < cend) G1_GLOAD(c + 1)
+    const float* ap = &Xs[(wm * 32 + l31) * LD + lhi];
+    const float* bp = &Ds[(wn * 32 + l31) * LD + lhi];
+#pragma unroll 8
+    for (int ks = 0; ks < BK / 2; ++ks)
+      acc = __builtin_amdgcn_mfma_f32_32x32x2f32(ap[2 * ks], bp[2 * ks], acc, 0, 0, 0);
+  }
+#undef G1_GLOAD
+#undef G1_LSTORE
+  const int co = co0 + wn * 32 + l31;
+  if (co < Cout && cbeg < cend) {
+#pragma unroll
+    for (int i = 0; i < 16; ++i) {
+      const int ci = ci0 + wm * 32 + 4 * lhi + (i & 3) + 8 * (i >> 2);
+      if (ci < Cin) df_acc(dwt, (long long)ci * Cout + co, acc[i], fx);
+    }
+  }
diff --git a/dfmir_amd/csrc/nce_head.hip b/dfmir_amd/csrc/nce_head.hip
--- a/dfmir_amd/csrc/nce_head.hip
+++ b/dfmir_amd/csrc/nce_head.hip
@@ -181,116 +181,7 @@
 };
 constexpr int NH_R = 32, NH_M = 256, NH_CMAX = 256, NH_KB = 8;
 __global__ __launch_bounds__(256, 2) void nce_head_fwd_k(NceHeadP k) {
-  __shared__ float Xs[NH_CMAX * NH_R];
-  __shared__ float Hs[NH_M * NH_R];
-  __shared__ float red[4][NH_R];
-  const int tid = threadIdx.x, lane = tid & 63, wid = tid >> 6;
-  const int l31 = lane & 31, hi = lane >> 5;
-  const long long r0 = (long long)blockIdx.x * NH_R;
-  {
-    const int r = tid & 31;
-    const long long rr = r0 + r;
-    const bool rok = rr < k.rows;
-    const long long gb = rok ? rr / k.P : 0;
-    const int pp = rok ? (int)(rr - gb * k.P) : 0;
-    const int g = (int)(gb / k.Bper), b = (int)(gb - (long long)g * k.Bper);
-    const long long id = rok ? k.ids[(long long)g * k.P + pp] : 0;
-    const float* src = k.srcs.p[g] + (long long)b * k.C * k.S + id;
-    const int Cp = (k.C + 2 * NH_KB - 1) / (2 * NH_KB) * (2 * NH_KB);
-    for (int cb = tid >> 5; cb < Cp; cb += 64) {
-      float v[8];
-#pragma unroll
-      for (int u = 0; u < 8; ++u) {
-        const int c = cb + 8 * u;
-        v[u] = (rok && c < k.C) ? src[(long long)c * k.S] : 0.f;
-      }
-#pragma unroll
-      for (int u = 0; u < 8; ++u) {
-        const int c = cb + 8 * u;
-        if (c < Cp) {
-          Xs[c * NH_R + r] = v[u];
-          if (k.xs && rok && c < k.C) k.xs[(long long)c * k.rows + rr] = v[u];
-        }
-      }
-    }
-  }
-  __syncthreads();
-  const int m0 = 64 * wid;
-  nh_f32x16 acc[2];
-#pragma unroll
-  for (int i = 0; i < 2; ++i)
-#pragma unroll
-    for (int e = 0; e < 16; ++e) acc[i][e] = 0.f;
-#define NH_GEMM(W_, KTOT_, SRC_)                                                                  \
-  {                                                                                               \
-    const float* wp = (W_) + m0 + l31;                                                            \
-    const int K2 = ((KTOT_) + 1) >> 1, nb = (K2 + NH_KB - 1) / NH_KB;                             \
-    float ca0[NH_KB], ca1[NH_KB], na0[NH_KB], na1[NH_KB];                                         \
-    _Pragma("unroll") for (int u = 0; u < NH_KB; ++u) {                                           \
-      const int kr = 2 * u + hi;                                                                  \
-      const bool ok = kr < (KTOT_);                                                               \
-      ca0[u] = ok ? wp[(long long)kr * NH_M] : 0.f;                                               \
-      ca1[u] = ok ? wp[(long long)kr * NH_M + 32] : 0.f;                                          \
-    }                                                                                             \
-    for (int j = 0; j < nb; ++j) {                                                                \
-      if (j + 1 < nb) {                                                                           \
-        _Pragma("unroll") for (int u = 0; u < NH_KB; ++u) {                                       \
-          const int kr = 2 * ((j + 1) * NH_KB + u) + hi;                                          \
-          const bool ok = kr < (KTOT_);                                                           \
-          na0[u] = ok ? wp[(long long)kr * NH_M] : 0.f;                                           \
-          na1[u] = ok ? wp[(long long)kr * NH_M + 32] : 0.f;                                      \
-        }                                                                                         \
-      }                                                                                           \
-      _Pragma("unroll") for (int u = 0; u < NH_KB; ++u) {                                         \
-        const int kr = 2 * (j * NH_KB + u) + hi;                                                  \
-        const float bv = (SRC_)[kr * NH_R + l31];                                                 \
-        acc[0] = __builtin_amdgcn_mfma_f32_32x32x2f32(ca0[u], bv, acc[0], 0, 0, 0);               \
-        acc[1] = __builtin_amdgcn_mfma_f32_32x32x2f32(ca1[u], bv, acc[1], 0, 0, 0);               \
-      }                                                                                           \
-      _Pragma("unroll") for (int u = 0; u < NH_KB; ++u) { ca0[u] = na0[u]; ca1[u] = na1[u]; }     \
-    }                                                                                             \
-  }
-  NH_GEMM(k.w1, k.C, Xs)
-#pragma unroll
-  for (int i = 0; i < 2; ++i)
-#pragma unroll
-    for (int e = 0; e < 16; ++e) {
-      const int m = m0 + 32 * i + (e >> 2) * 8 + hi * 4 + (e & 3);
-      float v = acc[i][e] + k.b1[m];
-      v = v > 0.f ? v : 0.f;
-      Hs[m * NH_R + l31] = v;
-      if (k.hs && r0 + l31 < k.rows) k.hs[(long long)m * k.rows + r0 + l31] = v;
-      acc[i][e] = 0.f;
-    }
-  __syncthreads();
-  NH_GEMM(k.w2, NH_M, Hs)
-#undef NH_GEMM
-  float ss = 0.f;
-#pragma unroll
-  for (int i = 0; i < 2; ++i)
-#pragma unroll
-    for (int e = 0; e < 16; ++e) {
-      const int m = m0 + 32 * i + (e >> 2) * 8 + hi * 4 + (e & 3);
-      acc[i][e] += k.b2[m];
-      ss += acc[i][e] * acc[i][e];
-    }
-  ss += __shfl_xor(ss, 32);
-  if (hi == 0) red[wid][l31] = ss;
-  __syncthreads();
-  const float nr = sqrtf((red[0][l31] + red[1][l31]) + (red[2][l31] + red[3][l31]));
-  const float inv = 1.f / (nr + k.eps);
-  const long long rr = r0 + l31;
-  if (rr < k.rows) {
-    if (k.nrm && wid == 0 && hi == 0) k.nrm[rr] = nr;
-#pragma unroll
-    for (int i = 0; i < 2; ++i)
-#pragma unroll
-      for (int e = 0; e < 16; ++e) {
-        const int m = m0 + 32 * i + (e >> 2) * 8 + hi * 4 + (e & 3);
-        k.out[(long long)m * k.rows + rr] = acc[i][e] * inv;
-        if (k.ypre) k.ypre[(long long)m * k.rows + rr] = acc[i][e];
-      }
-  }
+#include "nce_head_fwd_body.inc"
 }
 extern "C" int dfmir_nce_head_fwd(const float* const* srcs, int G, const long long* ids, const float* w1, const float* b1,
                                   const float* w2, const float* b2, float* out, float* nrm, float* xs, float* hs,
@@ -309,6 +200,37 @@
   return 0;
 }
 
+struct NceHeadTab {
+  NceHeadP job[DF_NCE_GROUP_MAX];
+};
+__global__ __launch_bounds__(256, 2) void nce_head_fwd_group_k(NceHeadTab t) {
+  const NceHeadP& k = t.job[blockIdx.y];
+#include "nce_head_fwd_body.inc"
+}
+extern "C" int dfmir_nce_head_fwd_group(const DfNceHeadJob* jobs, int njobs, float eps, void* stream) {
+  DF_ARG_CHECK(jobs && njobs > 0 && njobs <= DF_NCE_GROUP_MAX);
+  NceHeadTab t{};
+  long long rows = 0;
+  for (int j = 0; j < njobs; ++j) {
+    const DfNceHeadJob& a = jobs[j];
+    DF_ARG_CHECK(a.ids && a.w1 && a.b1 && a.w2 && a.b2 && a.out && a.G > 0 && a.G <= 8 && a.Bper > 0 && a.C > 0 &&
+                 a.C <= NH_CMAX && a.S > 0 && a.P > 0);
+    NceHeadP& k = t.job[j];
+    for (int g = 0; g < a.G; ++g) {
+      DF_ARG_CHECK(a.srcs[g] != nullptr);
+      k.srcs.p[g] = a.srcs[g];
+    }
+    k.ids = a.ids; k.w1 = a.w1; k.b1 = a.b1; k.w2 = a.w2; k.b2 = a.b2;
+    k.out = a.out; k.nrm = a.nrm; k.xs = a.xs; k.hs = a.hs; k.ypre = a.ypre;
+    k.G = a.G; k.Bper = a.Bper; k.C = a.C; k.P = a.P; k.S = a.S; k.rows = (long long)a.G * a.Bper * a.P; k.eps = eps;
+    DF_ARG_CHECK(j == 0 || k.rows == rows);
+    rows = k.rows;
+  }
+  nce_head_fwd_group_k<<<dim3((unsigned)((rows + NH_R - 1) / NH_R), (unsigned)njobs), 256, 0, (hipStream_t)stream>>>(t);
+  DF_LAUNCH_CHECK();
+  return 0;
+}
+
 __global__ __launch_bounds__(256) void segment_means_k(const float* __restrict__ rows, float* __restrict__ out, int L,
                                                        int T, long long seg, float scale) {
   __shared__ float sm[17];
diff --git a/dfmir_amd/csrc/nce_head_fwd_body.inc b/dfmir_amd/csrc/nce_head_fwd_body.inc
--- /dev/null
+++ b/dfmir_amd/csrc/nce_head_fwd_body.inc
@@ -0,0 +1,110 @@
+  __shared__ float Xs[NH_CMAX * NH_R];
+  __shared__ float Hs[NH_M * NH_R];
+  __shared__ float red[4][NH_R];
+  const int tid = threadIdx.x, lane = tid & 63, wid = tid >> 6;
+  const int l31 = lane & 31, hi = lane >> 5;
+  const long long r0 = (long long)blockIdx.x * NH_R;
+  {
+    const int r = tid & 31;
+    const long long rr = r0 + r;
+    const bool rok = rr < k.rows;
+    const long long gb = rok ? rr / k.P : 0;
+    const int pp = rok ? (int)(rr - gb * k.P) : 0;
+    const int g = (int)(gb / k.Bper), b = (int)(gb - (long long)g * k.Bper);
+    const long long id = rok ? k.ids[(long long)g * k.P + pp] : 0;
+    const float* src = k.srcs.p[g] + (long long)b * k.C * k.S + id;
+    const int Cp = (k.C + 2 * NH_KB - 1) / (2 * NH_KB) * (2 * NH_KB);
+    for (int cb = tid >> 5; cb < Cp; cb += 64) {
+      float v[8];
+#pragma unroll
+      for (int u = 0; u < 8; ++u) {
+        const int c = cb + 8 * u;
+        v[u] = (rok && c < k.C) ? src[(long long)c * k.S] : 0.f;
+      }
+#pragma unroll
+      for (int u = 0; u < 8; ++u) {
+        const int c = cb + 8 * u;
+        if (c < Cp) {
+          Xs[c * NH_R + r] = v[u];
+          if (k.xs && rok && c < k.C) k.xs[(long long)c * k.rows + rr] = v[u];
+        }
+      }
+    }
+  }
+  __syncthreads();
+  const int m0 = 64 * wid;
+  nh_f32x16 acc[2];
+#pragma unroll
+  for (int i = 0; i < 2; ++i)
+#pragma unroll
+    for (int e = 0; e < 16; ++e) acc[i][e] = 0.f;
+#define NH_GEMM(W_, KTOT_, SRC_)                                                                  \
+  {                                                                                               \
+    const float* wp = (W_) + m0 + l31;                                                            \
+    const int K2 = ((KTOT_) + 1) >> 1, nb = (K2 + NH_KB - 1) / NH_KB;                             \
+    float ca0[NH_KB], ca1[NH_KB], na0[NH_KB], na1[NH_KB];                                         \
+    _Pragma("unroll") for (int u = 0; u < NH_KB; ++u) {                                           \
+      const int kr = 2 * u + hi;                                                                  \
+      const bool ok = kr < (KTOT_);                                                               \
+      ca0[u] = ok ? wp[(long long)kr * NH_M] : 0.f;                                               \
+      ca1[u] = ok ? wp[(long long)kr * NH_M + 32] : 0.f;                                          \
+    }                                                                                             \
+    for (int j = 0; j < nb; ++j) {                                                                \
+      if (j + 1 < nb) {                                                                           \
+        _Pragma("unroll") for (int u = 0; u < NH_KB; ++u) {                                       \
+          const int kr = 2 * ((j + 1) * NH_KB + u) + hi;                                          \
+          const bool ok = kr < (KTOT_);                                                           \
+          na0[u] = ok ? wp[(long long)kr * NH_M] : 0.f;                                           \
+          na1[u] = ok ? wp[(long long)kr * NH_M + 32] : 0.f;                                      \
+        }                                                                                         \
+      }                                                                                           \
+      _Pragma("unroll") for (int u = 0; u < NH_KB; ++u) {                                         \
+        const int kr = 2 * (j * NH_KB + u) + hi;                                                  \
+        const float bv = (SRC_)[kr * NH_R + l31];                                                 \
+        acc[0] = __builtin_amdgcn_mfma_f32_32x32x2f32(ca0[u], bv, acc[0], 0, 0, 0);               \
+        acc[1] = __builtin_amdgcn_mfma_f32_32x32x2f32(ca1[u], bv, acc[1], 0, 0, 0);               \
+      }                                                                                           \
+      _Pragma("unroll") for (int u = 0; u < NH_KB; ++u) { ca0[u] = na0[u]; ca1[u] = na1[u]; }     \
+    }                                                                                             \
+  }
+  NH_GEMM(k.w1, k.C, Xs)
+#pragma unroll
+  for (int i = 0; i < 2; ++i)
+#pragma unroll
+    for (int e = 0; e < 16; ++e) {
+      const int m = m0 + 32 * i + (e >> 2) * 8 + hi * 4 + (e & 3);
+      float v = acc[i][e] + k.b1[m];
+      v = v > 0.f ? v : 0.f;
+      Hs[m * NH_R + l31] = v;
+      if (k.hs && r0 + l31 < k.rows) k.hs[(long long)m * k.rows + r0 + l31] = v;
+      acc[i][e] = 0.f;
+    }
+  __syncthreads();
+  NH_GEMM(k.w2, NH_M, Hs)
+#undef NH_GEMM
+  float ss = 0.f;
+#pragma unroll
+  for (int i = 0; i < 2; ++i)
+#pragma unroll
+    for (int e = 0; e < 16; ++e) {
+      const int m = m0 + 32 * i + (e >> 2) * 8 + hi * 4 + (e & 3);
+      acc[i][e] += k.b2[m];
+      ss += acc[i][e] * acc[i][e];
+    }
+  ss += __shfl_xor(ss, 32);
+  if (hi == 0) red[wid][l31] = ss;
+  __syncthreads();
+  const float nr = sqrtf((red[0][l31] + red[1][l31]) + (red[2][l31] + red[3][l31]));
+  const float inv = 1.f / (nr + k.eps);
+  const long long rr = r0 + l31;
+  if (rr < k.rows) {
+    if (k.nrm && wid == 0 && hi == 0) k.nrm[rr] = nr;
+#pragma unroll
+    for (int i = 0; i < 2; ++i)
+#pragma unroll
+      for (int e = 0; e < 16; ++e) {
+        const int m = m0 + 32 * i + (e >> 2) * 8 + hi * 4 + (e & 3);
+        k.out[(long long)m * k.rows + rr] = acc[i][e] * inv;
+        if (k.ypre) k.ypre[(long long)m * k.rows + rr] = acc[i][e];
+      }
+  }
diff --git a/dfmir_amd/networks.py b/dfmir_amd/networks.py
--- a/dfmir_amd/networks.py
+++ b/dfmir_amd/networks.py
@@ -415,6 +415,14 @@
             return ops.nce_head_multi(srcs, ids, mlp[0], mlp[2])
         return self.project(feat_id, ops.patch_gather_multi(srcs, ids))
 
+    def nce_losses_grouped(self, feats, key_srcs, ids, n_terms, groups, temp, scale, keep=None):
+        if not (self.use_mlp and self.mlp_init and 'forward' not in vars(self)
+                and all(ops.nce_head_ok(f.shape[1], self.nc, self.use_mlp) for f in feats)
+                and ops.nce_group_ok(feats, key_srcs, ids, n_terms, groups)):
+            return None
+        mlps = [(getattr(self, 'mlp_%d' % l)[0], getattr(self, 'mlp_%d' % l)[2]) for l in range(len(feats))]
+        return ops.nce_phase(feats, key_srcs, ids, mlps, n_terms, groups, temp, scale, keep=keep)
+
     def project(self, feat_id, x_cm):
         if self.use_mlp:
             mlp = getattr(self, 'mlp_%d' % feat_id)
diff --git a/dfmir_amd/ops.py b/dfmir_amd/ops.py
--- a/dfmir_amd/ops.py
+++ b/dfmir_amd/ops.py
@@ -1957,6 +1957,7 @@
 
 
 def nce_terms(qs, ks, groups, temp, scale, n_terms):
+    _LAST_NCE_GROUPED[0] = False
     return NCETermsFn.apply(int(groups), temp, scale, int(n_terms), *(list(qs) + [k.detach() for k in ks]))
 
 
@@ -2138,6 +2139,210 @@
     return NceHeadFn.apply(feat, ids2, mlp0.weight, mlp0.bias, mlp2.weight, mlp2.bias, mlp0, mlp2, eps, distinct)
 
 
+_NO_NCE_GROUP = _env_on("DFMIR_NO_NCE_GROUP")
+_NCE_GROUP_SKIP = frozenset(s for s in os.environ.get("DFMIR_NCE_GROUP_SKIP", "").replace(" ", "").split(",") if s)
+_LAST_NCE_GROUPED = [False]
+
+
+def last_nce_grouped():
+    return _LAST_NCE_GROUPED[0]
+
+
+def nce_group_ok(feats, key_srcs, ids, n_terms, groups):
+    from ._lib import NCE_GROUP_MAX
+    if _NO_NCE_GROUP or _CONV_PROFILER[0] is not None or _DET["on"] or _PROBE_AUDIT["on"]:
+        return False
+    L, T = len(feats), int(n_terms)
+    if not (1 <= L and 2 * L <= NCE_GROUP_MAX and 1 <= T <= 8 and len(key_srcs) == L and len(ids) == L):
+        return False
+    rows = None
+    for f, ks, i in zip(feats, key_srcs, ids):
+        if not (f.is_cuda and f.dtype == torch.float32 and f.is_contiguous() and f.dim() == 4 and f.shape[0] % T == 0
+                and 1 <= f.shape[1] <= 256 and i.dim() == 2 and i.shape[0] == T and i.dtype == torch.int64
+                and len(ks) == T and all(tuple(k.shape) == tuple(ks[0].shape) and k.is_contiguous() for k in ks)
+                and ks[0].shape[1] == f.shape[1] and ks[0].numel() // (ks[0].shape[0] * ks[0].shape[1]) == f.shape[2] * f.shape[3]):
+            return False
+        r = f.shape[0] * i.shape[1]
+        if T * ks[0].shape[0] * i.shape[1] != r or (rows is not None and r != rows):
+            return False
+        rows = r
+        if torch.is_grad_enabled() and f.requires_grad and not ids_distinct(i, T):
+            return False
+    return rows % groups == 0 and (rows // groups) % 16 == 0
+
+
+class NceGroupFn(Function):
+
+    @staticmethod
+    def forward(ctx, cfg, *ts):
+        from ._lib import DfNceHeadJob
+        L, T = cfg["L"], cfg["T"]
+        feats, params = ts[:L], ts[L:]
+        ids, mlps, keys, eps = cfg["ids"], cfg["mlps"], cfg["keys"], float(cfg["eps"])
+        _need(*feats)
+        dev = feats[0].device
+        Pn = ids[0].shape[1]
+        rows = feats[0].shape[0] * Pn
+        ctx.stashes = [getattr(f, "_df_tap_stash", None) for f in feats]
+        q, k, nrm, xs, hs, ypre, metas = [], [], [], [], [], [], []
+        jobs = (DfNceHeadJob * (2 * L))()
+        for l in range(L):
+            f = feats[l]
+            B, C = f.shape[0], f.shape[1]
+            S = f.numel() // (B * C)
+            Bper = B // T
+            metas.append((tuple(f.shape), B, C, S, Pn, T, True))
+            if "head" in _NCE_GROUP_SKIP:
+                k.append(_nce_head_launch([s_.data_ptr() for s_ in keys[l]], T, ids[l], mlps[l][0], mlps[l][1],
+                                          keys[l][0].shape[0], C, S, Pn, eps, dev, False)[0])
+                o = _nce_head_launch([f.data_ptr() + 4 * g * Bper * C * S for g in range(T)], T, ids[l], mlps[l][0],
+                                     mlps[l][1], Bper, C, S, Pn, eps, dev, True)
+                for lst, t in zip((q, nrm, xs, hs, ypre), o):
+                    lst.append(t)
+                continue
+            k.append(torch.empty((256, rows), device=dev, dtype=torch.float32))
+            q.append(torch.empty((256, rows), device=dev, dtype=torch.float32))
+            nrm.append(torch.empty(rows, device=dev, dtype=torch.float32))
+            xs.append(torch.empty((C, rows), device=dev, dtype=torch.float32))
+            hs.append(torch.empty((256, rows), device=dev, dtype=torch.float32))
+            ypre.append(torch.empty((256, rows), device=dev, dtype=torch.float32))
+            w1p, w2p = mlps[l][0].packed(0), mlps[l][1].packed(0)
+            for side in range(2):
+                j = jobs[2 * l + side]
+                for g in range(T):
+                    j.srcs[g] = keys[l][g].data_ptr() if side == 0 else f.data_ptr() + 4 * g * Bper * C * S
+                j.ids = ids[l].data_ptr()
+                j.w1, j.b1, j.w2, j.b2 = (w1p.data_ptr(), mlps[l][0].bias.data_ptr(), w2p.data_ptr(),
+                                          mlps[l][1].bias.data_ptr())
+                j.out = (k if side == 0 else q)[l].data_ptr()
+                if side == 1:
+                    j.nrm, j.xs, j.hs, j.ypre = nrm[l].data_ptr(), xs[l].data_ptr(), hs[l].data_ptr(), ypre[l].data_ptr()
+                j.G, j.Bper, j.C, j.P, j.S = T, (keys[l][0].shape[0] if side == 0 else Bper), C, Pn, S
+        if "head" not in _NCE_GROUP_SKIP:
+            check(lib().dfmir_nce_head_fwd_group(jobs, 2 * L, eps, _st()))
+        groups, temp, scale = cfg["groups"], float(cfg["temp"]), float(cfg["scale"])
+        R = rows // groups
+        buf = torch.empty((L, rows), device=dev, dtype=torch.float32)
+        probs = [torch.empty((rows, R + 1), device=dev, dtype=torch.float32) for _ in range(L)]
+        for l in range(L):
+            check(lib().dfmir_patchnce_fwd(_p(q[l]), _p(k[l]), _p(buf[l]), _p(probs[l]), rows, 256, groups, temp, _st()))
+        out = torch.empty(T, device=dev, dtype=torch.float32)
+        check(lib().dfmir_segment_means_fwd(_p(buf), _p(out), L, T, rows // T, scale, _st()))
+        ctx.save_for_backward(*(list(ids) + nrm + xs + hs + ypre + probs + k + list(params)))
+        ctx.meta = (L, T, rows, groups, temp, scale, eps, metas)
+        ctx.mlps = mlps
+        ctx.rows_buf = buf
+        keep = cfg.get("keep")
+        if keep is not None:
+            keep.update(q=q, k=k, nrm=nrm, xs=xs, hs=hs, ypre=ypre, rows=buf, probs=probs)
+        ctx.keep = keep
+        return out
+
+    @staticmethod
+    @once_differentiable
+    def backward(ctx, g):
+        from ._lib import DfWgradJob
+        L, T, rows, groups, temp, scale, eps, metas = ctx.meta
+        sv = ctx.saved_tensors
+        ids, nrm, xs, hs, ypre, probs, k = (sv[i * L:(i + 1) * L] for i in range(7))
+        params = sv[7 * L:]
+        g = _c(g)
+        dev = g.device
+        drows = torch.empty((L, rows), device=dev, dtype=torch.float32)
+        check(lib().dfmir_segment_means_bwd(_p(g), _p(drows), L, T, rows // T, scale, _st()))
+        dq = [torch.empty_like(k[l]) for l in range(L)]
+        dy = [torch.empty_like(ypre[l]) for l in range(L)]
+        for l in range(L):
+            check(lib().dfmir_patchnce_bwd(_p(drows[l]), _p(probs[l]), _p(k[l]), _p(dq[l]), rows, 256, groups, temp, _st()))
+        for l in range(L):
+            check(lib().dfmir_l2norm_bwd(_p(dq[l]), _p(ypre[l]), _p(nrm[l]), _p(dy[l]), 256, rows, eps, _st()))
+        grads = [None] * (L + 4 * L)
+        wjobs, late = [], []
+        dpres, dxs = [], []
+        for l in range(L):
+            shape, B, C, S, Pn, G, distinct = metas[l]
+            mlp0, mlp2 = ctx.mlps[l]
+            w1, b1, w2, b2 = params[4 * l:4 * l + 4]
+            need = ctx.needs_input_grad[1 + L + 4 * l:1 + L + 4 * l + 4]
+            c2 = _Ctx()
+            c2.cfg, c2.x_amax, c2.dead_tail, c2.in_act, c2.has_bias = (2, (1, 1, 1), 1, (0, 0, 0), 0, 0, 0.0, mlp2), None, 0, None, True
+            c2.needs_input_grad = (True, False, False)
+            dh, _, _ = _conv_backward_impl(c2, dy[l].view(1, 256, 1, rows), None, hs[l].view(1, 256, 1, 1, rows),
+                                           w2.view(256, 256, 1, 1), None)
+            dh = _c(dh)
+            dpre = torch.empty_like(dh)
+            check(lib().dfmir_act_bwd(_p(dh), _p(hs[l]), _p(dpre), dh.numel(), 1, 0.0, _st()))
+            dpres.append(dpre)
+            dx = None
+            if ctx.needs_input_grad[1 + l]:
+                c1 = _Ctx()
+                c1.cfg, c1.x_amax, c1.dead_tail, c1.in_act, c1.has_bias = (2, (1, 1, 1), 1, (0, 0, 0), 0, 0, 0.0, mlp0), None, 0, None, True
+                c1.needs_input_grad = (True, False, False)
+                dx, _, _ = _conv_backward_impl(c1, dpre.view(1, 256, 1, rows), None, xs[l].view(1, C, 1, 1, rows),
+                                               w1.view(256, C, 1, 1), None)
+            dxs.append(dx)
+            for which, (owner, w, x_, dy_, Cin, nw, nb) in enumerate(((mlp0, w1, xs[l], dpre, C, need[0], need[1]),
+                                                                      (mlp2, w2, hs[l], dy[l], 256, need[2], need[3]))):
+                gi = L + 4 * l + 2 * which
+                defer = (_DEFER["on"] and getattr(owner, "weight", None) is not None and owner.weight.grad is not None
+                         and owner.weight.grad.is_contiguous())
+                db_buf = None
+                if nb:
+                    bg = owner.bias.grad if defer and getattr(owner, "bias", None) is not None else None
+                    if bg is not None and bg.is_contiguous():
+                        db_buf = bg
+                    else:
+                        grads[gi + 1] = db_buf = zeros(256, dev)
+                x5, dy5 = x_.view(1, Cin, 1, 1, rows), dy_.view(1, 256, 1, 1, rows)
+                if not nw:
+                    if db_buf is not None:
+                        bias_grad(dy5, db_buf)
+                    continue
+                dwt = (_deferred_buffer(owner, 1, Cin, 256, (256, Cin, 1, 1), dev) if defer else zeros((1, Cin, 256), dev))
+                if not defer:
+                    late.append((gi, dwt, (256, Cin, 1, 1)))
+                if "wgrad" not in _NCE_GROUP_SKIP and lib().dfmir_conv1x1_wgrad_group_ok(Cin, 256, rows, _p(x_), _p(dy_)):
+                    wjobs.append((x_, dy_, dwt, db_buf, Cin))
+                else:
+                    conv_wgrad_raw(x5, dy5, (1, 1, 1), 1, (0, 0, 0), 0, out=dwt, db=db_buf)
+        if wjobs:
+            jobs = (DfWgradJob * len(wjobs))()
+            for j, (x_, dy_, dwt, db_buf, Cin) in zip(jobs, wjobs):
+                j.x, j.dy, j.dw_tcc, j.db = x_.data_ptr(), dy_.data_ptr(), dwt.data_ptr(), (db_buf.data_ptr() if db_buf is not None else None)
+                j.Cin, j.Cout = Cin, 256
+            check(lib().dfmir_conv1x1_wgrad_group(jobs, len(wjobs), rows, _st()))
+        for gi, dwt, shape in late:
+            grads[gi] = weight_unpack(dwt, shape).view(shape[0], shape[1])
+        for l in range(L):
+            dx = dxs[l]
+            if dx is None:
+                continue
+            shape, B, C, S, Pn, G, distinct = metas[l]
+            dxr = _c(dx).view(C, rows)
+            if ctx.stashes[l] is not None:
+                ctx.stashes[l].append((dxr, ids[l], metas[l]))
+            else:
+                dfeat = zeros(shape, dev)
+                check(lib().dfmir_patch_gather_bwd_g(_p(dxr), _p(ids[l]), _p(dfeat), B, C, S, Pn, G, None, _st()))
+                grads[l] = dfeat
+        if ctx.keep is not None:
+            ctx.keep.update(dq=dq, dy=dy, dh=dpres, dx=dxs)
+        return (None,) + tuple(grads)
+
+
+def nce_phase(feats, key_srcs, ids, mlps, n_terms, groups, temp, scale, eps=1e-7, keep=None):
+    L = len(feats)
+    cfg = {"L": L, "T": int(n_terms), "ids": [_c(i) for i in ids], "mlps": list(mlps),
+           "keys": [[k.detach() for k in ks] for ks in key_srcs], "groups": int(groups), "temp": temp, "scale": scale,
+           "eps": eps, "keep": keep}
+    params = []
+    for m0, m2 in mlps:
+        params += [m0.weight, m0.bias, m2.weight, m2.bias]
+    out = NceGroupFn.apply(cfg, *(list(feats) + params))
+    _LAST_NCE_GROUPED[0] = True
+    return out
+
+
 _LAST_L1_WS = [None]
 
 
diff --git a/dfmir_amd/registration_model.py b/dfmir_amd/registration_model.py
--- a/dfmir_amd/registration_model.py
+++ b/dfmir_amd/registration_model.py
@@ -644,8 +644,13 @@
                 for src, _ in terms:
                     if id(src) not in keys:
                         keys[id(src)] = self._encode_keys(src)
-                k_cm = [self.netF.sample_project_multi(l, [keys[id(src)][l] for src, _ in terms], ids[l])
-                        for l in range(n_layers)]
+            key_srcs = [[keys[id(src)][l] for src, _ in terms] for l in range(n_layers)]
+            losses = self.netF.nce_losses_grouped(feat_q, key_srcs, ids, T, T * per_term_groups, self.opt.nce_T,
+                                                  self.opt.lambda_NCE / n_layers)
+            if losses is not None:
+                return list(losses.unbind(0))
+            with torch.no_grad():
+                k_cm = [self.netF.sample_project_multi(l, key_srcs[l], ids[l]) for l in range(n_layers)]
             q_cm = [self.netF.sample_project(l, feat_q[l], ids[l], T) for l in range(n_layers)]
             losses = ops.nce_terms(q_cm, k_cm, T * per_term_groups, self.opt.nce_T,
                                    self.opt.lambda_NCE / n_layers, T)
diff --git a/include/dfmir_hip.h b/include/dfmir_hip.h
--- a/include/dfmir_hip.h
+++ b/include/dfmir_hip.h
@@ -246,6 +246,24 @@
                        int C, int G, float T, void* stream);
 int dfmir_patchnce_bwd(const float* dloss, const float* probs, const float* k, float* dq,
                        long long rows, int C, int G, float T, void* stream);
+
+#define DF_NCE_GROUP_MAX 16
+typedef struct DfNceHeadJob {
+  const float* srcs[8];
+  const long long* ids;
+  const float *w1, *b1, *w2, *b2;
+  float *out, *nrm, *xs, *hs, *ypre;
+  int G, Bper, C, P;
+  long long S;
+} DfNceHeadJob;
+int dfmir_nce_head_fwd_group(const DfNceHeadJob* jobs, int njobs, float eps, void* stream);
+typedef struct DfWgradJob {
+  const float *x, *dy;
+  float *dw_tcc, *db;
+  int Cin, Cout;
+} DfWgradJob;
+int dfmir_conv1x1_wgrad_group_ok(int Cin, int Cout, long long rows, const float* x, const float* dy);
+int dfmir_conv1x1_wgrad_group(const DfWgradJob* jobs, int njobs, long long rows, void* stream);
 
 int dfmir_masked_l1_fwd(const float* a, const float* b, const unsigned char* mask, float thr,
                         float* ws, float* out, long long n, void* stream);
```

After: 222.2, median of 6. No clear change (+0.7%).
